# gvanhorn38/multibox

Measured on AMD Instinct MI355X. Metric: images/sec (299x299, 5-AR priors) train, higher is better.
Workload: dtype bf16; 1 GPU; full train step: Inception-ResNet-v2 + multibox heads fwd, on-device matching+loss, bwd, RMSProp+EMA; 299x299, k=5 (P=646), BATCH_SIZE=64/GPU, MAX_NUM_BBOXES=13; global_batch=64, parallelism=dp1, hip_graph=True

## Files before the change

### include/mbx.h

```cpp
#ifndef MBX_H
#define MBX_H

#include <stddef.h>
#include <stdint.h>

#ifdef __cplusplus
extern "C" {
#endif

typedef void* mbx_stream_t;

typedef enum {
  MBX_OK = 0,
  MBX_ERR_INVALID_ARG = -1,
  MBX_ERR_UNSUPPORTED = -2,
  MBX_ERR_LAUNCH = -3,
  MBX_ERR_WORKSPACE = -4
} mbx_status;

int mbx_version(void);
const char* mbx_status_string(int status);

int mbx_priors_count(int k, const int* grids, int n_grids);

uint32_t mbx_crc32c(const void* data, uint64_t n, uint32_t crc);
int mbx_generate_priors(const double* aspect_ratios, int k, double min_scale, double max_scale,
                        int restrict_to_image_bounds, const int* grids, int n_grids,
                        double* out );

int mbx_decode_conf(const float* raw_locs , const float* logits ,
                    const float* priors , int B, int P, float eps_add,
                    float* decoded , float* conf , mbx_stream_t stream);

size_t mbx_match_workspace_bytes(int B, int P, int G);
int mbx_match(const float* decoded , const float* conf ,
              const float* gt , const int32_t* n_gt , float alpha,
              int B, int P, int G, int32_t* match , int32_t* status ,
              void* workspace, size_t workspace_bytes, mbx_stream_t stream);

int mbx_match_extend(const float* priors , const float* gt ,
                     const int32_t* n_gt , const int32_t* status ,
                     float iou_threshold, int B, int P, int G,
                     int32_t* match ,
                     int32_t* n_extra , mbx_stream_t stream);

size_t mbx_loss_workspace_bytes(int B);
int mbx_loss_fwd_bwd(const float* decoded , const float* conf_in ,
                     int conf_is_logit, const float* gt ,
                     const int32_t* match , float alpha, float grad_scale, int B, int P,
                     int G, float* loss2 ,
                     float* d_raw_locs , float* d_logits ,
                     void* workspace, size_t workspace_bytes, mbx_stream_t stream);

size_t mbx_loss_mined_workspace_bytes(int B, int P);
int mbx_loss_fwd_bwd_mined(const float* decoded , const float* conf_in ,
                           int conf_is_logit, const float* gt ,
                           const int32_t* match , float alpha, float grad_scale, int B, int P,
                           int G, float* loss2 ,
                           float* d_raw_locs , float* d_logits ,
                           int neg_per_pos, int min_neg, int32_t* n_neg ,
                           void* workspace, size_t workspace_bytes, mbx_stream_t stream);

size_t mbx_loss_focal_workspace_bytes(int B, int P);
int mbx_loss_fwd_bwd_focal(const float* decoded , const float* conf_in ,
                           int conf_is_logit, const float* gt ,
                           const int32_t* match , float alpha, float grad_scale, int B, int P,
                           int G, float* loss2 ,
                           float* d_raw_locs , float* d_logits ,
                           float gamma, float w_pos, float w_neg,
                           int neg_per_pos , int min_neg, int32_t* n_neg ,
                           void* workspace, size_t workspace_bytes, mbx_stream_t stream);

typedef struct {
  int32_t offset_y, offset_x;
  int32_t patch_h, patch_w;
  int32_t image_h, image_w;
  int32_t is_flipped;
  int32_t max_to_keep;
  float restrictions[4];
} mbx_patch_meta;

int mbx_decode_filter_topk(const float* raw_locs , const float* conf ,
                           const float* priors , const mbx_patch_meta* meta ,
                           int B, int P, int k_max, double* out_boxes ,
                           float* out_scores , int32_t* out_index ,
                           int32_t* out_count , mbx_stream_t stream);

int mbx_nms(double* boxes , float* scores , int32_t* index ,
            int32_t* count , int B, int k_max, double iou_threshold, mbx_stream_t stream);

#define MBX_MERGE_MAX_CANDIDATES 16384
int mbx_merge_detections(const double* boxes , const float* scores ,
                         const int32_t* count , const int32_t* image_rows , int I, int k_max,
                         int max_det, double iou_threshold, double* out_boxes ,
                         float* out_scores , int32_t* out_src ,
                         int32_t* out_count , int32_t* out_status , mbx_stream_t stream);

int mbx_merge_detections_voted(const double* boxes , const float* scores ,
                               const int32_t* count , const int32_t* image_rows , int I,
                               int k_max, int max_det, double iou_threshold, double vote_iou_threshold,
                               double* out_boxes , float* out_scores ,
                               int32_t* out_src , int32_t* out_count ,
                               int32_t* out_status , int32_t* out_votes , mbx_stream_t stream);

#define MBX_SOFT_LINEAR 1
#define MBX_SOFT_GAUSSIAN 2
int mbx_merge_detections_soft(const double* boxes , const float* scores ,
                              const int32_t* count , const int32_t* image_rows , int I, int k_max,
                              int max_det, int method, double iou_threshold , double sigma ,
                              double min_score, double vote_iou_threshold ,
                              double* out_boxes , float* out_scores ,
                              int32_t* out_src , int32_t* out_count , int32_t* out_status ,
                              int32_t* out_votes , mbx_stream_t stream);

#define MBX_COCO_MAX_DET 100
#define MBX_COCO_MAX_GT 128
int mbx_coco_match(const double* dt , const int32_t* dt_rows ,
                   const double* gt , const int32_t* gt_rows , int I,
                   const double* iou_thrs , int T, const double* area_rng ,
                   int A, int16_t* match , uint8_t* ignore ,
                   int32_t* n_gt_counted , int32_t* status , mbx_stream_t stream);

#define MBX_COCO_ACC_MAX_R 128
#define MBX_COCO_ACC_MAX_M 4
#define MBX_COCO_ACC_MAX_ND 4194304
#define MBX_COCO_ACC_CHUNK 256
#define MBX_COCO_ACC_SORT_TILE 1024
size_t mbx_coco_accumulate_workspace(long long ND, int T, int A, int M);
int mbx_coco_accumulate(const double* dt , const int32_t* dt_rows , int I,
                        const int16_t* match , const uint8_t* ignore ,
                        const int32_t* n_gt_counted , int T, int A, const double* rec_thrs , int R,
                        const int32_t* max_dets , int M, double* precision ,
                        double* recall , void* workspace, size_t workspace_bytes, mbx_stream_t stream);

typedef enum {
  MBX_EPI_STORE = 0,
  MBX_EPI_AFFINE = 1,
  MBX_EPI_RESIDUAL = 2,
  MBX_EPI_STORE_F32 = 3
} mbx_epilogue;

typedef struct {
  int32_t n, rows_mod;
  int32_t c_begin[4];
  const void* y[4]; int32_t ld_y[4];
  const float* relu_thr[4];
  float* stats[4]; int32_t stats_ld[4];
} mbx_bn_bwd_stats;

#define MBX_GRID_BARRIER_BYTES 6400
typedef struct {
  void* barrier;
  void* a; int32_t ld_a;
  const float* beta;
  float* mean; float* rstd;
  float* moving_mean; float* moving_var;
  float* relu_thr;
  int32_t relu; float eps, decay;
  float* step_poison;
} mbx_bn_apply_desc;

#define MBX_BN_BWD_SLOTS 8
typedef struct {
  void* barrier;
  int32_t n;
  int32_t c_begin[4];
  const void* y[4]; int32_t ld_y[4];
  void* dy[4]; int32_t ld_dy[4];
  const float* mean[4]; const float* rstd[4]; const float* beta[4];
  float* dbeta[4];
  float* acc[4]; int32_t acc_ld[4];
  int32_t relu[4];
  float* step_poison;
} mbx_bn_bwd_fused;

typedef struct {
  const void* x; int64_t x_img_stride; int32_t ldx;
  int32_t N, H_in, W_in, C_in;
  const void* w; int32_t C_out, R, S;
  int32_t stride, transposed, pad_t, pad_l, H_out, W_out;
  void* y; int64_t y_img_stride; int32_t ldy;
  int32_t epilogue, relu, accumulate;
  const float* scale; const float* shift;
  const void* skip; int64_t skip_img_stride; int32_t ld_skip; float rscale;
  float* stats_partial;
  int32_t tile_config;
  const void* acc_src; int64_t acc_img_stride; int32_t ld_acc;
  int32_t* work_counter;
  int32_t max_workgroups;
  void* splitk_ws; int64_t splitk_ws_bytes;
  int32_t stats_rows_mod, stats_ld;
  const mbx_bn_bwd_stats* bn_bwd_stats;
  void* relu_bits; int32_t ld_bits;
  const mbx_bn_apply_desc* bn_apply;
  const mbx_bn_bwd_fused* bn_bwd;
} mbx_conv_desc;
#define MBX_CONV_TILE_CONFIGS 14
#define MBX_TILE_I5_BASE 32
#define MBX_TILE_I7 65
#define MBX_TILE_DIRECT3 96
#define MBX_TILE_DIRECTW 97
#define MBX_TILE_RESIDENT 98
#define MBX_TILE_PWRES 99
#define MBX_TILE_SPLITK_BASE 128
#define MBX_TILE_SPLITK_MAX 32

int mbx_conv_stats_rows(const mbx_conv_desc* desc );
int mbx_conv(const mbx_conv_desc* desc , mbx_stream_t stream);
int mbx_conv_supported(const mbx_conv_desc* desc );
int mbx_conv_pair(const mbx_conv_desc* a , const mbx_conv_desc* b , mbx_stream_t stream);
size_t mbx_conv_splitk_workspace_bytes(const mbx_conv_desc* desc );

int mbx_conv_wgrad(const mbx_conv_desc* desc , const void* dy,
                   int64_t dy_img_stride, int32_t ld_dy, float* dw, float* db, mbx_stream_t stream);

typedef struct {
  mbx_conv_desc desc;
  const void* dy; int64_t dy_img_stride; int32_t ld_dy;
  float scale;
  float* dw; float* db;
} mbx_wgrad_job;
typedef struct {
  int32_t n_layers, n_items;
  int64_t layers_off, items_off;
  int64_t queues_off, heads_off;
  double flops;
  int64_t tally_off;
} mbx_wgrad_plan_info;
#define MBX_WGRAD_DETERMINISTIC 1
#define MBX_WGRAD_SCATTER 2
size_t mbx_wgrad_plan_bytes(const mbx_wgrad_job* jobs , int n_jobs, int flags);
int mbx_wgrad_plan(const mbx_wgrad_job* jobs , int n_jobs, int flags, void* host_image, size_t bytes,
                   mbx_wgrad_plan_info* info );
int mbx_conv_wgrad_grouped(void* device_image , const mbx_wgrad_plan_info* info ,
                           mbx_stream_t stream);
int mbx_conv_wgrad_grouped_capped(void* device_image, const mbx_wgrad_plan_info* info , int max_workgroups,
                                  mbx_stream_t stream);

int mbx_conv_wgrad_scaled(const mbx_conv_desc* desc, const void* dy, int64_t dy_img_stride,
                          int32_t ld_dy, float scale, float* dw, float* db, mbx_stream_t stream);

int mbx_bn_finalize(const float* stats_partial , int rows, int C, int64_t count,
                    float eps, float decay, float* mean , float* rstd ,
                    float* moving_mean , float* moving_var ,
                    mbx_stream_t stream);
int mbx_bn_apply(const void* y, int64_t M, int C, const float* mean, const float* rstd,
                 const float* beta, int relu, void* a, int ld_a, mbx_stream_t stream);
int mbx_bn_apply_fused(const float* stats_partial, int rows, int64_t count, float eps, float decay,
                       const void* y, int64_t M, int C, const float* beta, int relu, void* a, int ld_a,
                       float* mean, float* rstd, float* moving_mean, float* moving_var,
                       mbx_stream_t stream);
int mbx_bn_apply_fused_mapped(const void* stats_fixed, int rows, int64_t count, float eps, float decay,
                              const void* y, int64_t M, int C, const float* beta, int relu, void* a, int ld_a,
                              const struct mbx_chan_map_s* a_map , float* mean, float* rstd, float* moving_mean,
                              float* moving_var, float* relu_thr, mbx_stream_t stream);
int mbx_bn_moving_update(float* moving_mean, float* moving_var, const float* batch_mean, const float* batch_var,
                         int64_t n, float decay, const float* skip_ctl, uint64_t* skipped_steps,
                         float* ema_mean, float* ema_var, float ema_decay, mbx_stream_t stream);
typedef struct mbx_chan_map_s { int32_t n; int32_t c_begin[4]; int32_t offset[4]; } mbx_chan_map;
int mbx_bn_finalize_parts(const float* const* parts , const int32_t* rows ,
                          const int32_t* Cs , int n_parts, int64_t count, float eps, float decay, float* mean,
                          float* rstd, float* moving_mean, float* moving_var, mbx_stream_t stream);
int mbx_bn_apply_mapped(const void* y, int64_t M, int C, const float* mean, const float* rstd, const float* beta,
                        int relu, void* a, int ld_a, const mbx_chan_map* a_map , mbx_stream_t stream);
int mbx_bn_apply_maxpool(const void* y, int N, int H, int W, int C, const float* mean, const float* rstd, const float* beta,
                         int relu, void* p, int64_t p_img_stride, int ld_p, int Ho, int Wo, uint8_t* argmax,
                         mbx_stream_t stream);
int mbx_bn_fold(const float* moving_mean, const float* moving_var, const float* beta, float eps,
                int C, float* scale, float* shift, mbx_stream_t stream);
int mbx_bn_bwd_rows(int64_t M, int C);
int mbx_bn_bwd_reduce(const void* da, int ld_da, const void* a, int ld_a, int relu, const void* y,
                      int64_t M, int C, const float* mean, const float* rstd, const float* beta,
                      float* partial , mbx_stream_t stream);
int mbx_bn_bwd_finalize(const float* partial, int rows, int C, int64_t M, float* dbeta ,
                        float* m12 , mbx_stream_t stream);
int mbx_bn_bwd_apply(const void* da, int ld_da, const void* a, int ld_a, int relu, const void* y,
                     int64_t M, int C, const float* mean, const float* rstd, const float* beta,
                     const float* m12, void* dy , mbx_stream_t stream);

int mbx_bn_bwd_reduce_mapped(const void* da, int ld_da, const void* a, int ld_a, int relu, const void* y, int64_t M, int C,
                             const float* mean, const float* rstd, const float* beta, float* partial,
                             const mbx_chan_map* da_map , mbx_stream_t stream);
int mbx_bn_bwd_apply_mapped(const void* da, int ld_da, const void* a, int ld_a, int relu, const void* y, int64_t M, int C,
                            const float* mean, const float* rstd, const float* beta, const float* m12, void* dy,
                            const mbx_chan_map* da_map , mbx_stream_t stream);

int mbx_bn_bwd_apply_rows(const float* stats, int rows, const void* da, int ld_da, const void* y, int64_t M, int C,
                          const float* mean, const float* rstd, const float* relu_thr, float* dbeta, void* dy,
                          const mbx_chan_map* da_map , mbx_stream_t stream);

size_t mbx_bn_bwd_onepass_workspace_bytes(int C);
int mbx_bn_bwd_onepass_supported(int64_t M, int C, int max_workgroups);
int mbx_bn_bwd_onepass(const void* da, int ld_da, int relu, const void* y, int64_t M, int C,
                       const float* mean, const float* rstd, const float* beta, float* dbeta ,
                       void* dy , void* ws, int max_workgroups, float* step_poison ,
                       mbx_stream_t stream);

int mbx_bn_bwd_rows_pooled(int N, int H, int W, int C);
int mbx_bn_bwd_reduce_pooled(const void* gy, int64_t gy_img_stride, int ld_gy, const uint8_t* argmax, int N, int H, int W,
                             int Ho, int Wo, int relu, const void* y, int C, const float* mean, const float* rstd,
                             const float* beta, float* partial , mbx_stream_t stream);
int mbx_bn_bwd_apply_pooled(const void* gy, int64_t gy_img_stride, int ld_gy, const uint8_t* argmax, int N, int H, int W,
                            int Ho, int Wo, int relu, const void* y, int C, const float* mean, const float* rstd,
                            const float* beta, const float* m12, void* dy, mbx_stream_t stream);
int mbx_bn_bwd_onepass_mapped(const void* da, int ld_da, int relu, const void* y, int64_t M, int C, const float* mean,
                              const float* rstd, const float* beta, float* dbeta, void* dy, void* ws, int max_workgroups,
                              float* step_poison, const mbx_chan_map* da_map , mbx_stream_t stream);

int mbx_maxpool_fwd(const void* x, int64_t x_img_stride, int ldx, int N, int H, int W, int C,
                    int k, int stride, void* y, int64_t y_img_stride, int ldy, int Ho, int Wo,
                    uint8_t* argmax , mbx_stream_t stream);
int mbx_maxpool_bwd(const void* dy, int64_t dy_img_stride, int ld_dy, const uint8_t* argmax,
                    int N, int H, int W, int C, int k, int stride, int Ho, int Wo, void* dx,
                    int64_t dx_img_stride, int ld_dx, int accumulate, mbx_stream_t stream);
int mbx_avgpool_fwd(const void* x, int64_t x_img_stride, int ldx, int N, int H, int W, int C,
                    int k, int pad, void* y, int64_t y_img_stride, int ldy, int Ho, int Wo,
                    mbx_stream_t stream);
int mbx_avgpool_bwd(const void* dy, int64_t dy_img_stride, int ld_dy, int N, int H, int W, int C,
                    int k, int pad, int Ho, int Wo, void* dx, int64_t dx_img_stride, int ld_dx,
                    int accumulate, mbx_stream_t stream);

int mbx_relu_mask(void* g, int ld_g, const void* a, int ld_a, int64_t M, int C, mbx_stream_t stream);
int mbx_pack_input(const float* img, int64_t pixels, void* out, mbx_stream_t stream);
int mbx_head_gather(const float* h, int ld_h, int N, int cells, int k, int P, int off,
                    float* locs, float* logits, mbx_stream_t stream);
int mbx_head_scatter(const float* d_locs, const float* d_logits, int N, int cells, int k, int P,
                     int off, void* g, int ld_g, mbx_stream_t stream);

typedef struct {
  const float* h; int32_t ld_h;
  void* g; int32_t ld_g;
  int32_t cells, k, off;
} mbx_head;
int mbx_head_gather_all(const mbx_head* heads , int n_heads, int N, int P, float* locs, float* logits,
                        mbx_stream_t stream);
int mbx_head_scatter_all(const float* d_locs, const float* d_logits, const mbx_head* heads , int n_heads, int N,
                         int P, mbx_stream_t stream);

int mbx_step_begin(float* grads, int64_t n_grads, float* bn_ws, int64_t n_ws, int64_t ctl_index, uint64_t* timeouts_total,
                   float* zero_scalar, mbx_stream_t stream);

typedef struct {
  int64_t src_off;
  int64_t dst_off;
  int32_t K, R, S, C, Kpad;
  int32_t first_block;
} mbx_filter_entry;
int mbx_filter_prepare(const void* w_bf16, void* w_dgrad, const mbx_filter_entry* table ,
                       int n_entries, int total_blocks, mbx_stream_t stream);

int mbx_rmsprop_ema_step(float* w, const float* g, float* ms, float* mom ,
                         float* ema , void* w_bf16 , int64_t n, float lr,
                         float decay, float momentum, float eps, float wd, float ema_decay,
                         int trainable, float* reg_loss, const float* skip_ctl, mbx_stream_t stream);
int mbx_ema_update(float* ema, const float* value, int64_t n, float ema_decay, const float* skip_ctl ,
                   mbx_stream_t stream);

typedef struct {
  uint64_t src_offset;
  int32_t src_h, src_w;
  int32_t method;
  int32_t flip;
  int32_t n_ops;
  int32_t op[4];
  int32_t pad_;
  double arg[4];
} mbx_augment_item;
size_t mbx_augment_workspace_bytes(int B, int S);
int mbx_augment_batch(const uint8_t* src , const mbx_augment_item* items , int B, int S,
                      int any_contrast, float* out , void* workspace, mbx_stream_t stream);

typedef struct {
  uint64_t src_offset;
  int32_t img_h, img_w;
  int32_t win_y, win_x, win_h, win_w;
  int32_t flip_source;
  int32_t pad_;
} mbx_patch_item;
int mbx_extract_patches(const uint8_t* src , const mbx_patch_item* items , int n, int S,
                        float* out , mbx_stream_t stream);

#ifdef __cplusplus
}
#endif
#endif
```

### multibox_amd/_lib.py

```python
from __future__ import annotations

import ctypes as C
import os

_HERE = os.path.dirname(os.path.abspath(__file__))
LIB_PATH = os.path.join(_HERE, "libmbx.so")

P = C.c_void_p
I = C.c_int
F = C.c_float
D = C.c_double
SZ = C.c_size_t


class PatchMeta(C.Structure):
    _fields_ = [("offset_y", C.c_int32), ("offset_x", C.c_int32), ("patch_h", C.c_int32), ("patch_w", C.c_int32),
                ("image_h", C.c_int32), ("image_w", C.c_int32), ("is_flipped", C.c_int32),
                ("max_to_keep", C.c_int32), ("restrictions", C.c_float * 4)]


_SIGS = {
    "mbx_version": (I, []),
    "mbx_status_string": (C.c_char_p, [I]),
    "mbx_priors_count": (I, [I, P, I]),
    "mbx_crc32c": (C.c_uint32, [P, C.c_uint64, C.c_uint32]),
    "mbx_generate_priors": (I, [P, I, D, D, I, P, I, P]),
    "mbx_decode_conf": (I, [P, P, P, I, I, F, P, P, P]),
    "mbx_match_workspace_bytes": (SZ, [I, I, I]),
    "mbx_match": (I, [P, P, P, P, F, I, I, I, P, P, P, SZ, P]),
    "mbx_match_extend": (I, [P, P, P, P, F, I, I, I, P, P, P]),
    "mbx_loss_workspace_bytes": (SZ, [I]),
    "mbx_loss_fwd_bwd": (I, [P, P, I, P, P, F, F, I, I, I, P, P, P, P, SZ, P]),
    "mbx_loss_mined_workspace_bytes": (SZ, [I, I]),
    "mbx_loss_fwd_bwd_mined": (I, [P, P, I, P, P, F, F, I, I, I, P, P, P, I, I, P, P, SZ, P]),
    "mbx_loss_focal_workspace_bytes": (SZ, [I, I]),
    "mbx_loss_fwd_bwd_focal": (I, [P, P, I, P, P, F, F, I, I, I, P, P, P, F, F, F, I, I, P, P, SZ, P]),
    "mbx_decode_filter_topk": (I, [P, P, P, P, I, I, I, P, P, P, P, P]),
    "mbx_nms": (I, [P, P, P, P, I, I, C.c_double, P]),
    "mbx_merge_detections": (I, [P, P, P, P, I, I, I, C.c_double, P, P, P, P, P, P]),
    "mbx_merge_detections_voted": (I, [P, P, P, P, I, I, I, C.c_double, C.c_double, P, P, P, P, P, P, P]),
    "mbx_merge_detections_soft": (I, [P, P, P, P, I, I, I, I, C.c_double, C.c_double, C.c_double, C.c_double, P, P, P, P, P, P, P]),
    "mbx_coco_match": (I, [P, P, P, P, I, P, I, P, I, P, P, P, P, P]),
    "mbx_coco_accumulate_workspace": (SZ, [C.c_longlong, I, I, I]),
    "mbx_coco_accumulate": (I, [P, P, I, P, P, P, I, I, P, I, P, I, P, P, P, SZ, P]),
    "mbx_augment_workspace_bytes": (SZ, [I, I]),
    "mbx_augment_batch": (I, [P, P, I, I, I, P, P, P]),
    "mbx_extract_patches": (I, [P, P, I, I, P, P]),
    "mbx_conv_stats_rows": (I, [P]),
    "mbx_conv": (I, [P, P]),
    "mbx_conv_supported": (I, [P]),
    "mbx_conv_pair": (I, [P, P, P]),
    "mbx_conv_splitk_workspace_bytes": (SZ, [P]),
    "mbx_conv_wgrad": (I, [P, P, C.c_int64, I, P, P, P]),
    "mbx_conv_wgrad_scaled": (I, [P, P, C.c_int64, I, F, P, P, P]),
    "mbx_wgrad_plan_bytes": (SZ, [P, I, I]),
    "mbx_wgrad_plan": (I, [P, I, I, P, SZ, P]),
    "mbx_conv_wgrad_grouped": (I, [P, P, P]),
    "mbx_conv_wgrad_grouped_capped": (I, [P, P, I, P]),
    "mbx_bn_finalize": (I, [P, I, I, C.c_int64, F, F, P, P, P, P, P]),
    "mbx_bn_apply": (I, [P, C.c_int64, I, P, P, P, I, P, I, P]),
    "mbx_bn_moving_update": (I, [P, P, P, P, C.c_int64, F, P, P, P, P, F, P]),
    "mbx_bn_finalize_parts": (I, [P, P, P, I, C.c_int64, F, F, P, P, P, P, P]),
    "mbx_bn_apply_mapped": (I, [P, C.c_int64, I, P, P, P, I, P, I, P, P]),
    "mbx_bn_bwd_reduce_mapped": (I, [P, I, P, I, I, P, C.c_int64, I, P, P, P, P, P, P]),
    "mbx_bn_bwd_apply_mapped": (I, [P, I, P, I, I, P, C.c_int64, I, P, P, P, P, P, P, P]),
    "mbx_bn_apply_maxpool": (I, [P, I, I, I, I, P, P, P, I, P, C.c_int64, I, I, I, P, P]),
    "mbx_bn_bwd_rows_pooled": (I, [I, I, I, I]),
    "mbx_bn_bwd_reduce_pooled": (I, [P, C.c_int64, I, P, I, I, I, I, I, I, P, I, P, P, P, P, P]),
    "mbx_bn_bwd_apply_pooled": (I, [P, C.c_int64, I, P, I, I, I, I, I, I, P, I, P, P, P, P, P, P]),
    "mbx_bn_bwd_onepass_mapped": (I, [P, I, I, P, C.c_int64, I, P, P, P, P, P, P, I, P, P, P]),
    "mbx_bn_fold": (I, [P, P, P, F, I, P, P, P]),
    "mbx_bn_apply_fused": (I, [P, I, C.c_int64, F, F, P, C.c_int64, I, P, I, P, I, P, P, P, P, P]),
    "mbx_bn_apply_fused_mapped": (I, [P, I, C.c_int64, F, F, P, C.c_int64, I, P, I, P, I, P, P, P, P, P, P, P]),
    "mbx_bn_bwd_apply_rows": (I, [P, I, P, I, P, C.c_int64, I, P, P, P, P, P, P, P]),
    "mbx_bn_bwd_rows": (I, [C.c_int64, I]),
    "mbx_bn_bwd_onepass_workspace_bytes": (C.c_size_t, [I]),
    "mbx_bn_bwd_onepass_supported": (I, [C.c_int64, I, I]),
    "mbx_bn_bwd_onepass": (I, [P, I, I, P, C.c_int64, I, P, P, P, P, P, P, I, P, P]),
    "mbx_bn_bwd_reduce": (I, [P, I, P, I, I, P, C.c_int64, I, P, P, P, P, P]),
    "mbx_bn_bwd_finalize": (I, [P, I, I, C.c_int64, P, P, P]),
    "mbx_bn_bwd_apply": (I, [P, I, P, I, I, P, C.c_int64, I, P, P, P, P, P, P]),
    "mbx_maxpool_fwd": (I, [P, C.c_int64, I, I, I, I, I, I, I, P, C.c_int64, I, I, I, P, P]),
    "mbx_maxpool_bwd": (I, [P, C.c_int64, I, P, I, I, I, I, I, I, I, I, P, C.c_int64, I, I, P]),
    "mbx_avgpool_fwd": (I, [P, C.c_int64, I, I, I, I, I, I, I, P, C.c_int64, I, I, I, P]),
    "mbx_avgpool_bwd": (I, [P, C.c_int64, I, I, I, I, I, I, I, I, I, P, C.c_int64, I, I, P]),
    "mbx_relu_mask": (I, [P, I, P, I, C.c_int64, I, P]),
    "mbx_pack_input": (I, [P, C.c_int64, P, P]),
    "mbx_head_gather": (I, [P, I, I, I, I, I, I, P, P, P]),
    "mbx_head_scatter": (I, [P, P, I, I, I, I, I, P, I, P]),
    "mbx_head_gather_all": (I, [P, I, I, I, P, P, P]),
    "mbx_head_scatter_all": (I, [P, P, P, I, I, I, P]),
    "mbx_step_begin": (I, [P, C.c_int64, P, C.c_int64, C.c_int64, P, P, P]),
    "mbx_filter_prepare": (I, [P, P, P, I, I, P]),
    "mbx_rmsprop_ema_step": (I, [P, P, P, P, P, P, C.c_int64, F, F, F, F, F, F, I, P, P, P]),
    "mbx_ema_update": (I, [P, P, C.c_int64, F, P, P]),
}

_lib = None


class MbxError(RuntimeError):
    pass


class ChanMap(C.Structure):
    _fields_ = [("n", C.c_int32), ("c_begin", C.c_int32 * 4), ("offset", C.c_int32 * 4)]


class BnBwdStats(C.Structure):
    _fields_ = [("n", C.c_int32), ("rows_mod", C.c_int32), ("c_begin", C.c_int32 * 4), ("y", C.c_void_p * 4), ("ld_y", C.c_int32 * 4),
                ("relu_thr", C.c_void_p * 4), ("stats", C.c_void_p * 4), ("stats_ld", C.c_int32 * 4)]


class Head(C.Structure):
    _fields_ = [("h", C.c_void_p), ("ld_h", C.c_int32), ("g", C.c_void_p), ("ld_g", C.c_int32), ("cells", C.c_int32),
                ("k", C.c_int32), ("off", C.c_int32)]


class FilterEntry(C.Structure):
    _fields_ = [("src_off", C.c_int64), ("dst_off", C.c_int64), ("K", C.c_int32), ("R", C.c_int32), ("S", C.c_int32),
                ("C", C.c_int32), ("Kpad", C.c_int32), ("first_block", C.c_int32)]


def lib():
    global _lib
    if _lib is None:
        if not os.path.exists(LIB_PATH):
            raise MbxError("libmbx.so not built at %s -- run `python -c 'import __graft_entry__ as g; g.build()'` "
                           "(needs hipcc); there is no CPU fallback" % LIB_PATH)
        import torch
        l = C.CDLL(LIB_PATH)
        for name, (res, args) in _SIGS.items():
            fn = getattr(l, name)
            fn.restype = res
            fn.argtypes = args
        _lib = l
    return _lib


def check(status, what=""):
    if status != 0:
        msg = lib().mbx_status_string(int(status))
        raise MbxError("%s failed: %s (%d)" % (what or "libmbx call", msg.decode() if msg else "?", status))


def declared_symbols():
    return sorted(_SIGS)
```

### multibox_amd/csrc/loss.hip

```cpp
#include "boxes.h"

namespace {

constexpr int kThreads = 256;
constexpr int kWaves = kThreads / 64;

__global__ void __launch_bounds__(kThreads)
decode_conf_kernel(const float4* __restrict__ raw, const float* __restrict__ logits,
                   const float4* __restrict__ priors, int total, int P, float eps_add,
                   float4* __restrict__ decoded, float* __restrict__ conf) {
  for (int i = blockIdx.x * blockDim.x + threadIdx.x; i < total; i += gridDim.x * blockDim.x) {
    if (decoded) {
      const float4 r = raw[i], p = priors[i % P];
      decoded[i] = make_float4(__fadd_rn(r.x, p.x), __fadd_rn(r.y, p.y), __fadd_rn(r.z, p.z), __fadd_rn(r.w, p.w));
    }
    if (conf) {
      const float s = 1.0f / (1.0f + expf(-logits[i]));
      conf[i] = __fadd_rn(s, eps_add);
    }
  }
}

__device__ __forceinline__ double match_cost(const float4 l, const float4 g, float half_alpha,
                                             float lc, float l1c) {
  const float d0 = __fsub_rn(l.x, g.x), d1 = __fsub_rn(l.y, g.y), d2 = __fsub_rn(l.z, g.z), d3 = __fsub_rn(l.w, g.w);
  const float ss = __fadd_rn(__fadd_rn(__fadd_rn(__fmul_rn(d0, d0), __fmul_rn(d1, d1)), __fmul_rn(d2, d2)), __fmul_rn(d3, d3));
  const float nrm = __fsqrt_rn(ss);
  float t = __fmul_rn(half_alpha, __fmul_rn(nrm, nrm));
  t = __fsub_rn(t, lc);
  t = __fadd_rn(t, l1c);
  return (double)t;
}

struct Cand {
  double val;
  int j;
  int free_;
};

__device__ __forceinline__ bool cand_better(const Cand& a, const Cand& b) {
  if (a.j < 0) return false;
  if (b.j < 0) return true;
  if (a.val < b.val) return true;
  if (a.val > b.val) return false;
  if (a.free_ != b.free_) return a.free_ > b.free_;
  return a.j < b.j;
}

__device__ __forceinline__ Cand cand_shfl_xor(const Cand& c, int o) {
  Cand r;
  r.val = __shfl_xor(c.val, o, 64);
  r.j = __shfl_xor(c.j, o, 64);
  r.free_ = __shfl_xor(c.free_, o, 64);
  return r;
}

__global__ void __launch_bounds__(1024)
match_kernel(const float4* __restrict__ decoded, const float* __restrict__ conf,
             const float4* __restrict__ gt, const int* __restrict__ n_gt, float alpha, int P, int G,
             int* __restrict__ match, int* __restrict__ status) {
  extern __shared__ __attribute__((aligned(16))) unsigned char smem[];
  double* v = reinterpret_cast<double*>(smem);
  double* spc = v + P;
  double* u = spc + P;
  float2* lcl = reinterpret_cast<float2*>(u + G);
  int* path = reinterpret_cast<int*>(lcl + P);
  int* row4col = path + P;
  int* SC = row4col + P;
  int* col4row = SC + P;
  int* SR = col4row + G;
  __shared__ Cand wave_best[16];
  __shared__ int sh_i, sh_sink, sh_bad;
  __shared__ double sh_min;

  const int b = blockIdx.x, tid = threadIdx.x;
  const int nt = (int)blockDim.x, nwaves = nt >> 6;
  const float4* loc = decoded + (size_t)b * P;
  const float* cf = conf + (size_t)b * P;
  const float4* g = gt + (size_t)b * G;
  int* mt = match + (size_t)b * P;
  const int n = n_gt[b];
  const float half_alpha = alpha / 2.0f;

  if (tid == 0) sh_bad = 0;
  __syncthreads();
  int bad = 0;
  for (int j = tid; j < P; j += nt) {
    mt[j] = -1;
    const float c = cf[j];
    const float lc = logf(c);
    float w = __fsub_rn(1.0f, c);
    if (w > 1.0f) w = 1.0f;
    if (w <= 0.0f) w = 1e-10f;
    const float l1c = logf(w);
    lcl[j] = make_float2(lc, l1c);
    v[j] = 0.0;
    row4col[j] = -1;
    const float4 l = loc[j];
    if (!(isfinite(lc) && isfinite(l1c) && isfinite(l.x) && isfinite(l.y) && isfinite(l.z) && isfinite(l.w))) bad = 1;
  }
  for (int i = tid; i < G; i += nt) {
    u[i] = 0.0;
    col4row[i] = -1;
    if (i < n) {
      const float4 q = g[i];
      if (!(isfinite(q.x) && isfinite(q.y) && isfinite(q.z) && isfinite(q.w))) bad = 1;
    }
  }
  if (bad) sh_bad = 1;
  __syncthreads();
  if (n <= 0) { if (tid == 0) status[b] = 0; return; }
  if (n > P || n > G) { if (tid == 0) status[b] = 1; return; }
  if (sh_bad) { if (tid == 0) status[b] = 2; return; }

  for (int cur = 0; cur < n; ++cur) {
    for (int j = tid; j < P; j += nt) { spc[j] = INFINITY; SC[j] = 0; }
    for (int i = tid; i < n; i += nt) SR[i] = 0;
    if (tid == 0) { sh_i = cur; sh_sink = -1; sh_min = 0.0; }
    __syncthreads();
    while (true) {
      const int i = sh_i;
      const double min_val = sh_min;
      const float4 gi = g[i];
      const double ui = u[i];
      Cand best; best.val = INFINITY; best.j = -1; best.free_ = 0;
      for (int j = tid; j < P; j += nt) {
        if (SC[j]) continue;
        const float2 ll = lcl[j];
        const double r = ((min_val + match_cost(loc[j], gi, half_alpha, ll.x, ll.y)) - ui) - v[j];
        double s = spc[j];
        if (r < s) { path[j] = i; spc[j] = r; s = r; }
        Cand c; c.val = s; c.j = j; c.free_ = row4col[j] < 0;
        if (cand_better(c, best)) best = c;
      }
#pragma unroll
      for (int o = 32; o > 0; o >>= 1) {
        const Cand other = cand_shfl_xor(best, o);
        if (cand_better(other, best)) best = other;
      }
      if ((tid & 63) == 0) wave_best[tid >> 6] = best;
      __syncthreads();
      if (tid == 0) {
        Cand bb = wave_best[0];
        for (int w = 1; w < nwaves; ++w) if (cand_better(wave_best[w], bb)) bb = wave_best[w];
        if (bb.j < 0 || !(bb.val < INFINITY)) {
          sh_sink = -2;
        } else {
          sh_min = bb.val;
          SC[bb.j] = 1;
          SR[i] = 1;
          const int r4c = row4col[bb.j];
          if (r4c < 0) sh_sink = bb.j; else sh_i = r4c;
        }
      }
      __syncthreads();
      if (sh_sink != -1) break;
    }
    const int sink = sh_sink;
    if (sink == -2) { if (tid == 0) status[b] = 2; return; }
    const double min_val = sh_min;
    for (int i = tid; i < n; i += nt) {
      if (i == cur) u[i] += min_val;
      else if (SR[i]) u[i] += min_val - spc[col4row[i]];
    }
    for (int j = tid; j < P; j += nt)
      if (SC[j]) v[j] -= min_val - spc[j];
    __syncthreads();
    if (tid == 0) {
      int j = sink;
      while (true) {
        const int i = path[j];
        row4col[j] = i;
        const int t = col4row[i];
        col4row[i] = j;
        j = t;
        if (i == cur) break;
      }
    }
    __syncthreads();
  }
  for (int i = tid; i < n; i += nt) mt[col4row[i]] = i;
  if (tid == 0) status[b] = 0;
}

struct StagedBox { Box box; double area; };

__global__ void __launch_bounds__(1024)
match_extend_kernel(const float4* __restrict__ priors, const float4* __restrict__ gt, const int* __restrict__ n_gt,
                    const int* __restrict__ status, double thr, int P, int G, int* __restrict__ match,
                    int* __restrict__ n_extra) {
  extern __shared__ __attribute__((aligned(16))) unsigned char smem[];
  StagedBox* boxes = reinterpret_cast<StagedBox*>(smem);
  __shared__ int added_waves[16];
  const int b = blockIdx.x, tid = threadIdx.x, nt = (int)blockDim.x;
  const int n = n_gt[b];
  if (status[b] != 0 || n <= 0 || n > G) {
    if (tid == 0 && n_extra) n_extra[b] = 0;
    return;
  }
  for (int j = tid; j < n; j += nt) {
    const float4 q = gt[(size_t)b * G + j];
    StagedBox s;
    s.box = {(double)q.x, (double)q.y, (double)q.z, (double)q.w};
    s.area = box_area(s.box);
    boxes[j] = s;
  }
  __syncthreads();
  int* mt = match + (size_t)b * P;
  int added = 0;
  for (int p = tid; p < P; p += nt) {
    if (mt[p] >= 0) continue;
    const float4 q = priors[p];
    const Box e = {(double)q.x, (double)q.y, (double)q.z, (double)q.w};
    const double area_e = box_area(e);
    double best = thr;
    int best_j = -1;
    for (int j = 0; j < n; ++j) {
      const Box g = boxes[j].box;
      const double iw = fmin(e.x2, g.x2) - fmax(e.x1, g.x1), ih = fmin(e.y2, g.y2) - fmax(e.y1, g.y1);
      if (iw > 0.0 && ih > 0.0) {
        const double inter = iw * ih;
        const double uni = area_e + boxes[j].area - inter;
        const double iou = uni > 0.0 ? inter / uni : 0.0;
        if (iou > best) { best = iou; best_j = j; }
      }
    }
    if (best_j >= 0) { mt[p] = best_j; ++added; }
  }
  if (!n_extra) return;
  added = wave_sum(added);
  if ((tid & 63) == 0) added_waves[tid >> 6] = added;
  __syncthreads();
  if (tid == 0) {
    int total = 0;
    for (int w = 0; w < (nt >> 6); ++w) total += added_waves[w];
    n_extra[b] = total;
  }
}

__global__ void loss_final_kernel(const double* __restrict__ partial, int B, float alpha, float* __restrict__ loss2) {
  if (threadIdx.x == 0 && blockIdx.x == 0) {
    double a = 0.0, c = 0.0;
    for (int b = 0; b < B; ++b) { a += partial[2 * b]; c += partial[2 * b + 1]; }
    loss2[0] = alpha * (float)(a * 0.5);
    loss2[1] = (float)c;
  }
}

__device__ __forceinline__ unsigned long long mined_key(float conf_in, int P, int p) {
  return ((unsigned long long)score_order_key(conf_in) << 32) | (unsigned)(P - 1 - p);
}

__device__ __forceinline__ unsigned long long mined_select_cut(const int* __restrict__ mt, const float* __restrict__ cf,
                                                               int P, int neg_per_pos, int min_neg, int b,
                                                               int* __restrict__ n_neg) {
  static_assert(kThreads == 256, "one thread per histogram bin, four bins per lane of the walking wave");
  __shared__ unsigned hist[256];
  __shared__ unsigned long long sh_cut;
  __shared__ int sh_need, sh_done;
  const int tid = threadIdx.x;
  unsigned long long cut = 0ull;
  int need = 0;
  for (int shift = 56; shift >= 0; shift -= 8) {
    if (shift < 32 && ((unsigned)(P - 1) >> shift) == 0) continue;
    const unsigned long long fixed = shift == 56 ? 0ull : ~0ull << (shift + 8);
    hist[tid] = 0u;
    __syncthreads();
    for (int p = tid; p < P; p += kThreads) {
      if (mt[p] >= 0) continue;
      const unsigned long long key = mined_key(cf[p], P, p);
      if (((key ^ cut) & fixed) == 0ull) atomicAdd(&hist[(unsigned)(key >> shift) & 255u], 1u);
    }
    __syncthreads();
    if (tid < 64) {
      const unsigned h0 = hist[4 * tid], h1 = hist[4 * tid + 1], h2 = hist[4 * tid + 2], h3 = hist[4 * tid + 3];
      const unsigned own = h0 + h1 + h2 + h3;
      unsigned incl = own;
#pragma unroll
      for (int o = 1; o < 64; o <<= 1) {
        const unsigned t = __shfl_down(incl, o, 64);
        if (tid + o < 64) incl += t;
      }
      bool whole = false;
      if (shift == 56) {
        const int n_negatives = (int)__shfl(incl, 0, 64), n_pos = P - n_negatives;
        long long K = (long long)neg_per_pos * (long long)n_pos;
        if (K < (long long)min_neg) K = min_neg;
        if (K > (long long)n_negatives) K = n_negatives;
        need = (int)K;
        whole = need == 0 || need == n_negatives;
        if (tid == 0) {
          if (n_neg) n_neg[b] = need;
          if (whole) { sh_cut = need == 0 ? ~0ull : 0ull; sh_need = 0; sh_done = 1; }
        }
      }
      const unsigned above = incl - own, k = (unsigned)need;
      if (!whole && above < k && k <= incl) {
        unsigned a = above, cnt = h3;
        int d = 3;
        if (k > a + h3) { a += h3; cnt = h2; d = 2;
          if (k > a + h2) { a += h2; cnt = h1; d = 1;
            if (k > a + h1) { a += h1; cnt = h0; d = 0; } } }
        sh_cut = cut | ((unsigned long long)(4 * tid + d) << shift);
        sh_need = (int)(k - a);
        sh_done = cnt == k - a;
      }
    }
    __syncthreads();
    cut = sh_cut;
    need = sh_need;
    if (sh_done) break;
  }
  return cut;
}

template <bool MINED, bool FOCAL>
__device__ __forceinline__ void loss_body(const float4* __restrict__ decoded, const float* __restrict__ logits, int is_logit,
                                          const float4* __restrict__ gt, const int* __restrict__ match, float alpha,
                                          float grad_scale, int P, int G, float gamma, float w_pos, float w_neg,
                                          int neg_per_pos, int min_neg, double* __restrict__ partial ,
                                          float4* __restrict__ d_locs, float* __restrict__ d_logits, int* __restrict__ n_neg) {
  constexpr bool kCountPositives = FOCAL && !MINED;
  const int b = blockIdx.x, tid = threadIdx.x;
  unsigned long long cut = 0ull;
  if (MINED) cut = mined_select_cut(match + (size_t)b * P, logits + (size_t)b * P, P, neg_per_pos, min_neg, b, n_neg);
  const bool modulated = FOCAL && gamma != 0.0f;

  double loc_acc = 0.0, conf_acc = 0.0;
  int n_pos = 0;
  for (int p = tid; p < P; p += kThreads) {
    const size_t i = (size_t)b * P + p;
    const int m = match[i];
    const float z = logits[i];
    float4 dl = make_float4(0.f, 0.f, 0.f, 0.f);
    float g;
    if (MINED && m < 0 && mined_key(z, P, p) < cut) {
      g = 0.f;
    } else {
      const float s = is_logit ? 1.0f / (1.0f + expf(-z)) : z;
      const float c = __fadd_rn(s, 1e-10f);
      const float w = __fadd_rn(__fsub_rn(1.0f, c), 1e-10f);
      const float ds = is_logit ? s * (1.0f - s) : 1.0f;
      const bool pos = m >= 0;
      if (pos) {
        const float4 l = decoded[i], q = gt[(size_t)b * G + m];
        const float d0 = __fsub_rn(l.x, q.x), d1 = __fsub_rn(l.y, q.y), d2 = __fsub_rn(l.z, q.z), d3 = __fsub_rn(l.w, q.w);
        loc_acc += (double)d0 * d0 + (double)d1 * d1 + (double)d2 * d2 + (double)d3 * d3;
        const float a = alpha * grad_scale;
        dl = make_float4(a * d0, a * d1, a * d2, a * d3);
        if (kCountPositives) ++n_pos;
      }
      const float arg = pos ? c : w, base = pos ? w : c, wt = FOCAL ? (pos ? w_pos : w_neg) : 1.0f;
      const float lg = logf(arg);
      const float pw = modulated ? powf(base, gamma) : 1.0f;
      conf_acc -= (double)wt * ((double)pw * (double)lg);
      float d = (ds * pw) / arg;
      if (modulated) d = d - gamma * (pw / base) * lg * ds;
      d = wt * d;
      g = (pos ? -d : d) * grad_scale;
    }
    if (d_locs) d_locs[i] = dl;
    if (d_logits) d_logits[i] = g;
  }
  loc_acc = wave_sum(loc_acc);
  conf_acc = wave_sum(conf_acc);
  __shared__ double red[kWaves][2];
  __shared__ int pos_waves[kWaves];
  if (kCountPositives) n_pos = wave_sum(n_pos);
  if ((tid & 63) == 0) {
    red[tid >> 6][0] = loc_acc; red[tid >> 6][1] = conf_acc;
    if (kCountPositives) pos_waves[tid >> 6] = n_pos;
  }
  __syncthreads();
  if (tid == 0) {
    double a = 0.0, c = 0.0;
    for (int w = 0; w < kWaves; ++w) { a += red[w][0]; c += red[w][1]; }
    partial[2 * b] = a;
    partial[2 * b + 1] = c;
    if (kCountPositives && n_neg) {
      int total = 0;
      for (int w = 0; w < kWaves; ++w) total += pos_waves[w];
      n_neg[b] = P - total;
    }
  }
}

__global__ void __launch_bounds__(kThreads)
loss_kernel(const float4* __restrict__ decoded, const float* __restrict__ logits, int is_logit,
            const float4* __restrict__ gt, const int* __restrict__ match, float alpha, float grad_scale,
            int P, int G, double* __restrict__ partial , float4* __restrict__ d_locs,
            float* __restrict__ d_logits) {
  loss_body<false, false>(decoded, logits, is_logit, gt, match, alpha, grad_scale, P, G, 0.0f, 1.0f, 1.0f, 0, 0, partial,
                          d_locs, d_logits, nullptr);
}

__global__ void __launch_bounds__(kThreads)
loss_mined_kernel(const float4* __restrict__ decoded, const float* __restrict__ logits, int is_logit,
                  const float4* __restrict__ gt, const int* __restrict__ match, float alpha, float grad_scale,
                  int P, int G, int neg_per_pos, int min_neg, double* __restrict__ partial ,
                  float4* __restrict__ d_locs, float* __restrict__ d_logits, int* __restrict__ n_neg) {
  loss_body<true, false>(decoded, logits, is_logit, gt, match, alpha, grad_scale, P, G, 0.0f, 1.0f, 1.0f, neg_per_pos,
                         min_neg, partial, d_locs, d_logits, n_neg);
}

template <bool MINED>
__global__ void __launch_bounds__(kThreads)
loss_focal_kernel(const float4* __restrict__ decoded, const float* __restrict__ logits, int is_logit,
                  const float4* __restrict__ gt, const int* __restrict__ match, float alpha, float grad_scale,
                  int P, int G, float gamma, float w_pos, float w_neg, int neg_per_pos, int min_neg,
                  double* __restrict__ partial , float4* __restrict__ d_locs, float* __restrict__ d_logits,
                  int* __restrict__ n_neg) {
  loss_body<MINED, true>(decoded, logits, is_logit, gt, match, alpha, grad_scale, P, G, gamma, w_pos, w_neg, neg_per_pos,
                         min_neg, partial, d_locs, d_logits, n_neg);
}

}

extern "C" int mbx_decode_conf(const float* raw_locs, const float* logits, const float* priors, int B,
                               int P, float eps_add, float* decoded, float* conf, mbx_stream_t stream) {
  if (B < 0 || P <= 0) return MBX_ERR_INVALID_ARG;
  if ((decoded && (!raw_locs || !priors)) || (conf && !logits)) return MBX_ERR_INVALID_ARG;
  if (B == 0 || (!decoded && !conf)) return MBX_OK;
  const int total = B * P;
  int blocks = (total + kThreads - 1) / kThreads;
  if (blocks > 2048) blocks = 2048;
  MBX_ENTER();
  hipLaunchKernelGGL(decode_conf_kernel, dim3(blocks), dim3(kThreads), 0, mbx_s(stream),
                     reinterpret_cast<const float4*>(raw_locs), logits, reinterpret_cast<const float4*>(priors),
                     total, P, eps_add, reinterpret_cast<float4*>(decoded), conf);
  MBX_LAUNCH_CHECK();
  return MBX_OK;
}

static size_t match_lds_bytes(int P, int G) { return (size_t)P * 36 + (size_t)G * 16 + 16; }

extern "C" size_t mbx_match_workspace_bytes(int, int, int) { return 0; }

extern "C" int mbx_match(const float* decoded, const float* conf, const float* gt, const int32_t* n_gt,
                         float alpha, int B, int P, int G, int32_t* match, int32_t* status, void*, size_t,
                         mbx_stream_t stream) {
  if (!decoded || !conf || !gt || !n_gt || !match || !status || B < 0 || P <= 0 || G <= 0) return MBX_ERR_INVALID_ARG;
  if (B == 0) return MBX_OK;
  const size_t lds = match_lds_bytes(P, G);
  if (lds > 150 * 1024) return MBX_ERR_UNSUPPORTED;
  static const int force_nt = mbx_env_int("MBX_MATCH_THREADS", 0);
  const int nthreads = force_nt ? force_nt : (P > 1536 ? 512 : kThreads);
  MBX_ENTER();
  if (lds > 64 * 1024) {
    if (hipFuncSetAttribute(reinterpret_cast<const void*>(match_kernel), hipFuncAttributeMaxDynamicSharedMemorySize,
                            (int)lds) != hipSuccess) return MBX_ERR_LAUNCH;
  }
  hipLaunchKernelGGL(match_kernel, dim3(B), dim3(nthreads), lds, mbx_s(stream),
                     reinterpret_cast<const float4*>(decoded), conf, reinterpret_cast<const float4*>(gt), n_gt,
                     alpha, P, G, match, status);
  MBX_LAUNCH_CHECK();
  return MBX_OK;
}

extern "C" int mbx_match_extend(const float* priors, const float* gt, const int32_t* n_gt, const int32_t* status,
                                float iou_threshold, int B, int P, int G, int32_t* match, int32_t* n_extra,
                                mbx_stream_t stream) {
  if (!priors || !gt || !n_gt || !status || !match || B < 0 || P <= 0 || G <= 0) return MBX_ERR_INVALID_ARG;
  if (!(iou_threshold > 0.0f && iou_threshold <= 1.0f)) return MBX_ERR_INVALID_ARG;
  const size_t lds = (size_t)G * sizeof(StagedBox);
  if (lds > 60 * 1024) return MBX_ERR_UNSUPPORTED;
  if (B == 0) return MBX_OK;
  const int nthreads = P >= 1024 ? 1024 : (P + 63) / 64 * 64;
  MBX_ENTER();
  hipLaunchKernelGGL(match_extend_kernel, dim3(B), dim3(nthreads), lds, mbx_s(stream),
                     reinterpret_cast<const float4*>(priors), reinterpret_cast<const float4*>(gt), n_gt, status,
                     (double)iou_threshold, P, G, match, n_extra);
  MBX_LAUNCH_CHECK();
  return MBX_OK;
}

extern "C" size_t mbx_loss_workspace_bytes(int B) { return (size_t)(B > 0 ? B : 1) * 2 * sizeof(double); }
extern "C" size_t mbx_loss_mined_workspace_bytes(int B, int) { return mbx_loss_workspace_bytes(B); }
extern "C" size_t mbx_loss_focal_workspace_bytes(int B, int) { return mbx_loss_workspace_bytes(B); }

enum class LossKind { kPlain, kMined, kFocal };

static int launch_loss(LossKind kind, const float* decoded, const float* logits, int conf_is_logit, const float* gt,
                       const int32_t* match, float alpha, float grad_scale, int B, int P, int G, float* loss2,
                       float* d_raw_locs, float* d_logits, float gamma, float w_pos, float w_neg, int neg_per_pos,
                       int min_neg, int32_t* n_neg, void* workspace, size_t workspace_bytes, mbx_stream_t stream) {
  if (!decoded || !logits || !gt || !match || !loss2 || B <= 0 || P <= 0 || G <= 0) return MBX_ERR_INVALID_ARG;
  if (!workspace || workspace_bytes < mbx_loss_workspace_bytes(B)) return MBX_ERR_WORKSPACE;
  double* partial = reinterpret_cast<double*>(workspace);
  const float4* dec4 = reinterpret_cast<const float4*>(decoded);
  const float4* gt4 = reinterpret_cast<const float4*>(gt);
  float4* dl4 = reinterpret_cast<float4*>(d_raw_locs);
  MBX_ENTER();
  switch (kind) {
    case LossKind::kPlain:
      hipLaunchKernelGGL(loss_kernel, dim3(B), dim3(kThreads), 0, mbx_s(stream), dec4, logits, conf_is_logit, gt4, match,
                         alpha, grad_scale, P, G, partial, dl4, d_logits);
      break;
    case LossKind::kMined:
      hipLaunchKernelGGL(loss_mined_kernel, dim3(B), dim3(kThreads), 0, mbx_s(stream), dec4, logits, conf_is_logit, gt4,
                         match, alpha, grad_scale, P, G, neg_per_pos, min_neg, partial, dl4, d_logits, n_neg);
      break;
    case LossKind::kFocal:
      hipLaunchKernelGGL(neg_per_pos ? loss_focal_kernel<true> : loss_focal_kernel<false>, dim3(B), dim3(kThreads), 0,
                         mbx_s(stream), dec4, logits, conf_is_logit, gt4, match, alpha, grad_scale, P, G, gamma, w_pos,
                         w_neg, neg_per_pos, min_neg, partial, dl4, d_logits, n_neg);
      break;
  }
  MBX_LAUNCH_CHECK();
  hipLaunchKernelGGL(loss_final_kernel, dim3(1), dim3(64), 0, mbx_s(stream), partial, B, alpha, loss2);
  MBX_LAUNCH_CHECK();
  return MBX_OK;
}

extern "C" int mbx_loss_fwd_bwd(const float* decoded, const float* logits, int conf_is_logit, const float* gt,
                                const int32_t* match, float alpha, float grad_scale, int B, int P, int G, float* loss2,
                                float* d_raw_locs, float* d_logits, void* workspace, size_t workspace_bytes,
                                mbx_stream_t stream) {
  return launch_loss(LossKind::kPlain, decoded, logits, conf_is_logit, gt, match, alpha, grad_scale, B, P, G, loss2,
                     d_raw_locs, d_logits, 0.0f, 1.0f, 1.0f, 0, 0, nullptr, workspace, workspace_bytes, stream);
}

extern "C" int mbx_loss_fwd_bwd_mined(const float* decoded, const float* logits, int conf_is_logit, const float* gt,
                                      const int32_t* match, float alpha, float grad_scale, int B, int P, int G, float* loss2,
                                      float* d_raw_locs, float* d_logits, int neg_per_pos, int min_neg, int32_t* n_neg,
                                      void* workspace, size_t workspace_bytes, mbx_stream_t stream) {
  if (neg_per_pos < 1 || min_neg < 0) return MBX_ERR_INVALID_ARG;
  return launch_loss(LossKind::kMined, decoded, logits, conf_is_logit, gt, match, alpha, grad_scale, B, P, G, loss2,
                     d_raw_locs, d_logits, 0.0f, 1.0f, 1.0f, neg_per_pos, min_neg, n_neg, workspace, workspace_bytes, stream);
}

extern "C" int mbx_loss_fwd_bwd_focal(const float* decoded, const float* logits, int conf_is_logit, const float* gt,
                                      const int32_t* match, float alpha, float grad_scale, int B, int P, int G, float* loss2,
                                      float* d_raw_locs, float* d_logits, float gamma, float w_pos, float w_neg,
                                      int neg_per_pos, int min_neg, int32_t* n_neg, void* workspace, size_t workspace_bytes,
                                      mbx_stream_t stream) {
  if (!(gamma >= 0.0f && gamma <= 10.0f)) return MBX_ERR_INVALID_ARG;
  if (!(w_pos >= 0.0f && w_neg >= 0.0f) || isinf(w_pos) || isinf(w_neg)) return MBX_ERR_INVALID_ARG;
  if (neg_per_pos < 0 || min_neg < 0 || (neg_per_pos == 0 && min_neg > 0)) return MBX_ERR_INVALID_ARG;
  return launch_loss(LossKind::kFocal, decoded, logits, conf_is_logit, gt, match, alpha, grad_scale, B, P, G, loss2,
                     d_raw_locs, d_logits, gamma, w_pos, w_neg, neg_per_pos, min_neg, n_neg, workspace, workspace_bytes, stream);
}
```

### multibox_amd/csrc/nnops.hip

```cpp
#include "vec8.h"

namespace {

template <int KK, int SS>
__global__ void __launch_bounds__(kT)
maxpool_fwd_kernel(const unsigned short* __restrict__ x, long long xs, int ldx, int N, int H, int W, int C, int k_,
                   int stride_, unsigned short* __restrict__ y, long long ys, int ldy, int Ho, int Wo,
                   unsigned char* __restrict__ argmax) {
  const int k = KK ? KK : k_, stride = SS ? SS : stride_;
  const int C8 = C >> 3;
  const unsigned total = (unsigned)N * Ho * Wo * C8;
  for (unsigned i = blockIdx.x * kT + threadIdx.x; i < total; i += gridDim.x * kT) {
    unsigned t = i / (unsigned)C8;
    const int c = (int)(i - t * C8) << 3;
    const unsigned t2 = t / (unsigned)Wo;
    const int ow = (int)(t - t2 * Wo);
    const int n = (int)(t2 / (unsigned)Ho);
    const int oh = (int)(t2 - (unsigned)n * Ho);
    float best[8];
    unsigned arg[8];
#pragma unroll
    for (int j = 0; j < 8; ++j) { best[j] = -INFINITY; arg[j] = 0; }
    if constexpr (KK > 0) {
      u32x4 v[KK * KK];
#pragma unroll
      for (int r = 0; r < KK; ++r)
#pragma unroll
        for (int s = 0; s < KK; ++s) {
          const int h = oh * stride + r, w = ow * stride + s;
          v[r * KK + s] = (h < H && w < W) ? ld8(x + n * xs + ((long long)h * W + w) * ldx + c) : u32x4{0u, 0u, 0u, 0u};
        }
#pragma unroll
      for (int r = 0; r < KK; ++r)
#pragma unroll
        for (int s = 0; s < KK; ++s) {
          const int h = oh * stride + r, w = ow * stride + s;
          if (h >= H || w >= W) continue;
          float f[8];
          unpack8(v[r * KK + s], f);
#pragma unroll
          for (int j = 0; j < 8; ++j)
            if (f[j] > best[j]) { best[j] = f[j]; arg[j] = r * KK + s; }
        }
    } else {
      for (int r = 0; r < k; ++r)
        for (int s = 0; s < k; ++s) {
          const int h = oh * stride + r, w = ow * stride + s;
          if (h >= H || w >= W) continue;
          float f[8];
          unpack8(ld8(x + n * xs + ((long long)h * W + w) * ldx + c), f);
#pragma unroll
          for (int j = 0; j < 8; ++j)
            if (f[j] > best[j]) { best[j] = f[j]; arg[j] = r * k + s; }
        }
    }
    st8(y + n * ys + ((long long)oh * Wo + ow) * ldy + c, pack8(best));
    if (argmax) {
      u32x2 av;
      av.x = arg[0] | (arg[1] << 8) | (arg[2] << 16) | (arg[3] << 24);
      av.y = arg[4] | (arg[5] << 8) | (arg[6] << 16) | (arg[7] << 24);
      *reinterpret_cast<u32x2*>(argmax + (((long long)n * Ho + oh) * Wo + ow) * C + c) = av;
    }
  }
}

template <int KK, int SS>
__global__ void __launch_bounds__(kT)
maxpool_bwd_kernel(const unsigned short* __restrict__ dy, long long dys, int ld_dy,
                   const unsigned char* __restrict__ argmax, int N, int H, int W, int C, int k_, int stride_, int Ho,
                   int Wo, unsigned short* __restrict__ dx, long long dxs, int ld_dx, int accumulate) {
  const int k = KK ? KK : k_, stride = SS ? SS : stride_;
  const int C8 = C >> 3;
  const unsigned total = (unsigned)N * H * W * C8;
  for (unsigned i = blockIdx.x * kT + threadIdx.x; i < total; i += gridDim.x * kT) {
    unsigned t = i / (unsigned)C8;
    const int c = (int)(i - t * C8) << 3;
    const unsigned t2 = t / (unsigned)W;
    const int w = (int)(t - t2 * W);
    const int n = (int)(t2 / (unsigned)H);
    const int h = (int)(t2 - (unsigned)n * H);
    float acc[8];
    unsigned short* dst = dx + n * dxs + ((long long)h * W + w) * ld_dx + c;
    if (accumulate) unpack8(ld8(dst), acc);
    else {
#pragma unroll
      for (int j = 0; j < 8; ++j) acc[j] = 0.f;
    }
    if constexpr (KK > 0) {
      constexpr int NW = (KK + SS - 1) / SS;
      const int ohb = h / SS, owb = w / SS;
      u32x4 gv[NW * NW];
      u32x2 av[NW * NW];
      bool ok[NW * NW];
#pragma unroll
      for (int a = 0; a < NW; ++a)
#pragma unroll
        for (int b = 0; b < NW; ++b) {
          const int oh = ohb - (NW - 1 - a), ow = owb - (NW - 1 - b);
          const bool v = oh >= 0 && oh < Ho && ow >= 0 && ow < Wo && h - oh * SS < KK && w - ow * SS < KK;
          ok[a * NW + b] = v;
          const long long o = ((long long)n * Ho + (v ? oh : 0)) * Wo + (v ? ow : 0);
          av[a * NW + b] = v ? *reinterpret_cast<const u32x2*>(argmax + o * C + c) : u32x2{0u, 0u};
          gv[a * NW + b] = v ? ld8(dy + n * dys + ((long long)oh * Wo + ow) * ld_dy + c) : u32x4{0u, 0u, 0u, 0u};
        }
#pragma unroll
      for (int a = 0; a < NW; ++a)
#pragma unroll
        for (int b = 0; b < NW; ++b) {
          if (!ok[a * NW + b]) continue;
          const int oh = ohb - (NW - 1 - a), ow = owb - (NW - 1 - b);
          const unsigned tap = (h - oh * SS) * KK + (w - ow * SS);
          float g[8];
          unpack8(gv[a * NW + b], g);
#pragma unroll
          for (int j = 0; j < 8; ++j) {
            const unsigned aj = ((j < 4 ? av[a * NW + b].x : av[a * NW + b].y) >> (8 * (j & 3))) & 0xffu;
            if (aj == tap) acc[j] += g[j];
          }
        }
    } else {
      int oh0 = (h - k + stride) / stride;
      if (h - k + 1 <= 0) oh0 = 0;
      int ow0 = (w - k + stride) / stride;
      if (w - k + 1 <= 0) ow0 = 0;
      const int oh1 = min(h / stride, Ho - 1), ow1 = min(w / stride, Wo - 1);
      for (int oh = oh0; oh <= oh1; ++oh)
        for (int ow = ow0; ow <= ow1; ++ow) {
          const unsigned tap = (h - oh * stride) * k + (w - ow * stride);
          const long long o = ((long long)n * Ho + oh) * Wo + ow;
          const u32x2 av = *reinterpret_cast<const u32x2*>(argmax + o * C + c);
          float g[8];
          unpack8(ld8(dy + n * dys + ((long long)oh * Wo + ow) * ld_dy + c), g);
#pragma unroll
          for (int j = 0; j < 8; ++j) {
            const unsigned aj = ((j < 4 ? av.x : av.y) >> (8 * (j & 3))) & 0xffu;
            if (aj == tap) acc[j] += g[j];
          }
        }
    }
    st8(dst, pack8(acc));
  }
}

__global__ void __launch_bounds__(kT)
avgpool_fwd_kernel(const unsigned short* __restrict__ x, long long xs, int ldx, int N, int H, int W, int C, int k,
                   int pad, unsigned short* __restrict__ y, long long ys, int ldy, int Ho, int Wo) {
  const int C8 = C >> 3;
  const unsigned total = (unsigned)N * Ho * Wo * C8;
  for (unsigned i = blockIdx.x * kT + threadIdx.x; i < total; i += gridDim.x * kT) {
    unsigned t = i / (unsigned)C8;
    const int c = (int)(i - t * C8) << 3;
    const unsigned t2 = t / (unsigned)Wo;
    const int ow = (int)(t - t2 * Wo);
    const int n = (int)(t2 / (unsigned)Ho);
    const int oh = (int)(t2 - (unsigned)n * Ho);
    float acc[8];
#pragma unroll
    for (int j = 0; j < 8; ++j) acc[j] = 0.f;
    int cnt = 0;
    if (k == 3) {
      u32x4 v[9];
      bool ok[9];
#pragma unroll
      for (int r = 0; r < 3; ++r)
#pragma unroll
        for (int q = 0; q < 3; ++q) {
          const int h = oh - pad + r, w = ow - pad + q;
          ok[r * 3 + q] = (unsigned)h < (unsigned)H && (unsigned)w < (unsigned)W;
          v[r * 3 + q] = ok[r * 3 + q] ? ld8(x + n * xs + ((long long)h * W + w) * ldx + c) : u32x4{0u, 0u, 0u, 0u};
        }
#pragma unroll
      for (int tq = 0; tq < 9; ++tq) {
        if (!ok[tq]) continue;
        float f[8];
        unpack8(v[tq], f);
#pragma unroll
        for (int j = 0; j < 8; ++j) acc[j] += f[j];
        ++cnt;
      }
    } else
    for (int r = 0; r < k; ++r) {
      const int h = oh - pad + r;
      if ((unsigned)h >= (unsigned)H) continue;
      const unsigned short* row = x + n * xs + (long long)h * W * ldx + c;
      for (int s0 = 0; s0 < k; s0 += 8) {
        u32x4 v[8];
        bool ok[8];
#pragma unroll
        for (int q = 0; q < 8; ++q) {
          const int w = ow - pad + s0 + q;
          ok[q] = s0 + q < k && (unsigned)w < (unsigned)W;
          v[q] = ok[q] ? ld8(row + (long long)w * ldx) : u32x4{0u, 0u, 0u, 0u};
        }
#pragma unroll
        for (int q = 0; q < 8; ++q) {
          if (!ok[q]) continue;
          float f[8];
          unpack8(v[q], f);
#pragma unroll
          for (int j = 0; j < 8; ++j) acc[j] += f[j];
          ++cnt;
        }
      }
    }
    const float inv = 1.0f / (float)cnt;
#pragma unroll
    for (int j = 0; j < 8; ++j) acc[j] *= inv;
    st8(y + n * ys + ((long long)oh * Wo + ow) * ldy + c, pack8(acc));
  }
}

__global__ void __launch_bounds__(kT)
avgpool_bwd_kernel(const unsigned short* __restrict__ dy, long long dys, int ld_dy, int N, int H, int W, int C, int k,
                   int pad, int Ho, int Wo, unsigned short* __restrict__ dx, long long dxs, int ld_dx,
                   int accumulate) {
  const int C8 = C >> 3;
  const unsigned total = (unsigned)N * H * W * C8;
  for (unsigned i = blockIdx.x * kT + threadIdx.x; i < total; i += gridDim.x * kT) {
    unsigned t = i / (unsigned)C8;
    const int c = (int)(i - t * C8) << 3;
    const unsigned t2 = t / (unsigned)W;
    const int w = (int)(t - t2 * W);
    const int n = (int)(t2 / (unsigned)H);
    const int h = (int)(t2 - (unsigned)n * H);
    float acc[8];
    unsigned short* dst = dx + n * dxs + ((long long)h * W + w) * ld_dx + c;
    if (accumulate) unpack8(ld8(dst), acc);
    else {
#pragma unroll
      for (int j = 0; j < 8; ++j) acc[j] = 0.f;
    }
    const int oh0 = max(h + pad - k + 1, 0), oh1 = min(h + pad, Ho - 1);
    const int ow0 = max(w + pad - k + 1, 0), ow1 = min(w + pad, Wo - 1);
    if (k == 3) {
      u32x4 v[9];
      float inv[9];
#pragma unroll
      for (int a = 0; a < 3; ++a)
#pragma unroll
        for (int b = 0; b < 3; ++b) {
          const int oh = oh0 + a, ow = ow0 + b;
          const bool ok = oh <= oh1 && ow <= ow1;
          const int nh = min(oh - pad + 3, H) - max(oh - pad, 0), nw = min(ow - pad + 3, W) - max(ow - pad, 0);
          inv[a * 3 + b] = ok ? 1.0f / (float)(nh * nw) : 0.f;
          v[a * 3 + b] = ok ? ld8(dy + n * dys + ((long long)oh * Wo + ow) * ld_dy + c) : u32x4{0u, 0u, 0u, 0u};
        }
#pragma unroll
      for (int tq = 0; tq < 9; ++tq) {
        if (inv[tq] == 0.f) continue;
        float g[8];
        unpack8(v[tq], g);
#pragma unroll
        for (int j = 0; j < 8; ++j) acc[j] += g[j] * inv[tq];
      }
    } else
    for (int oh = oh0; oh <= oh1; ++oh) {
      const int nh = min(oh - pad + k, H) - max(oh - pad, 0);
      for (int ow = ow0; ow <= ow1; ++ow) {
        const int nw = min(ow - pad + k, W) - max(ow - pad, 0);
        const float inv = 1.0f / (float)(nh * nw);
        float g[8];
        unpack8(ld8(dy + n * dys + ((long long)oh * Wo + ow) * ld_dy + c), g);
#pragma unroll
        for (int j = 0; j < 8; ++j) acc[j] += g[j] * inv;
      }
    }
    st8(dst, pack8(acc));
  }
}

__global__ void __launch_bounds__(kT)
relu_mask_kernel(unsigned short* __restrict__ g, int ld_g, const unsigned short* __restrict__ a, int ld_a,
                 long long M, int C) {
  const int C8 = C >> 3;
  const long long total = M * C8;
  for (long long i = (long long)blockIdx.x * kT + threadIdx.x; i < total; i += (long long)gridDim.x * kT) {
    const long long m = i / C8;
    const int c = (int)(i - m * C8) << 3;
    float gg[8], aa[8];
    unpack8(ld8(g + m * ld_g + c), gg);
    unpack8(ld8(a + m * ld_a + c), aa);
#pragma unroll
    for (int j = 0; j < 8; ++j)
      if (!(aa[j] > 0.f)) gg[j] = 0.f;
    st8(g + m * ld_g + c, pack8(gg));
  }
}

__global__ void __launch_bounds__(kT)
pack_input_kernel(const float* __restrict__ img, long long pixels, unsigned short* __restrict__ out) {
  for (long long i = (long long)blockIdx.x * kT + threadIdx.x; i < pixels; i += (long long)gridDim.x * kT) {
    float f[8] = {img[3 * i], img[3 * i + 1], img[3 * i + 2], 0.f, 0.f, 0.f, 0.f, 0.f};
    st8(out + 8 * i, pack8(f));
  }
}

__global__ void __launch_bounds__(kT)
head_gather_kernel(const float* __restrict__ h, int ld_h, int N, int cells, int k, int P, int off,
                   float* __restrict__ locs, float* __restrict__ logits) {
  const int total = N * cells * k;
  for (int i = blockIdx.x * kT + threadIdx.x; i < total; i += gridDim.x * kT) {
    const int a = i % k, t = i / k, cell = t % cells, n = t / cells;
    const float* row = h + (size_t)(n * cells + cell) * ld_h;
    const size_t p = (size_t)n * P + off + cell * k + a;
    *reinterpret_cast<float4*>(locs + p * 4) = make_float4(row[a * 4], row[a * 4 + 1], row[a * 4 + 2], row[a * 4 + 3]);
    logits[p] = row[4 * k + a];
  }
}

__global__ void __launch_bounds__(kT)
head_scatter_kernel(const float* __restrict__ d_locs, const float* __restrict__ d_logits, int N, int cells, int k,
                    int P, int off, unsigned short* __restrict__ g, int ld_g) {
  const int total = N * cells * ld_g;
  for (int i = blockIdx.x * kT + threadIdx.x; i < total; i += gridDim.x * kT) {
    const int ch = i % ld_g, t = i / ld_g, cell = t % cells, n = t / cells;
    const size_t p = (size_t)n * P + off + cell * k;
    float v = 0.f;
    if (ch < 4 * k) v = d_locs[(p + ch / 4) * 4 + (ch & 3)];
    else if (ch < 5 * k) v = d_logits[p + (ch - 4 * k)];
    g[i] = (unsigned short)f2bf(v);
  }
}

constexpr int kMaxHeads = 8;
struct HeadTable {
  const float* h[kMaxHeads]; unsigned short* g[kMaxHeads];
  int ld_h[kMaxHeads], ld_g[kMaxHeads], cells[kMaxHeads], k[kMaxHeads], off[kMaxHeads];
  int start[kMaxHeads + 1];
  int n;
};

__global__ void __launch_bounds__(kT)
head_gather_all_kernel(const HeadTable t, int P, float* __restrict__ locs, float* __restrict__ logits) {
  const int total = t.start[t.n];
  for (int i = blockIdx.x * kT + threadIdx.x; i < total; i += gridDim.x * kT) {
    int j = 0;
    while (j + 1 < t.n && i >= t.start[j + 1]) ++j;
    const int e = i - t.start[j], k = t.k[j], cells = t.cells[j];
    const int a = e % k, q = e / k, cell = q % cells, n = q / cells;
    const float* row = t.h[j] + (size_t)(n * cells + cell) * t.ld_h[j];
    const size_t p = (size_t)n * P + t.off[j] + cell * k + a;
    *reinterpret_cast<float4*>(locs + p * 4) = make_float4(row[a * 4], row[a * 4 + 1], row[a * 4 + 2], row[a * 4 + 3]);
    logits[p] = row[4 * k + a];
  }
}

__global__ void __launch_bounds__(kT)
head_scatter_all_kernel(const HeadTable t, int P, const float* __restrict__ d_locs, const float* __restrict__ d_logits) {
  const int total = t.start[t.n];
  for (int i = blockIdx.x * kT + threadIdx.x; i < total; i += gridDim.x * kT) {
    int j = 0;
    while (j + 1 < t.n && i >= t.start[j + 1]) ++j;
    const int e = i - t.start[j], k = t.k[j], cells = t.cells[j], ld = t.ld_g[j];
    const int ch = e % ld, q = e / ld, cell = q % cells, n = q / cells;
    const size_t p = (size_t)n * P + t.off[j] + cell * k;
    float v = 0.f;
    if (ch < 4 * k) v = d_locs[(p + ch / 4) * 4 + (ch & 3)];
    else if (ch < 5 * k) v = d_logits[p + (ch - 4 * k)];
    t.g[j][e] = (unsigned short)f2bf(v);
  }
}

__global__ void __launch_bounds__(kT)
step_begin_kernel(float* __restrict__ G, long long nG, float* __restrict__ ws, long long nws, long long ctl,
                  unsigned long long* __restrict__ timeouts_total, float* __restrict__ scalar) {
  if (scalar && blockIdx.x == 0 && threadIdx.x == 0) *scalar = 0.f;
  const long long n4 = nG >> 2, w4 = nws >> 2;
  const float4 z = make_float4(0.f, 0.f, 0.f, 0.f);
  for (long long i = (long long)blockIdx.x * kT + threadIdx.x; i < n4 + w4; i += (long long)gridDim.x * kT) {
    if (i < n4) {
      if (timeouts_total && i == (ctl >> 2)) {
        const float t = G[ctl];
        if (t > 0.f) *timeouts_total += (unsigned long long)t;
      }
      reinterpret_cast<float4*>(G)[i] = z;
    } else {
      reinterpret_cast<float4*>(ws)[i - n4] = z;
    }
  }
}

__global__ void __launch_bounds__(kT)
filter_prepare_kernel(const unsigned short* __restrict__ w, unsigned short* __restrict__ wd,
                      const mbx_filter_entry* __restrict__ table, int n_entries) {
  __shared__ __attribute__((aligned(16))) unsigned short tile[64][40];
  int lo = 0, hi = n_entries - 1;
  while (lo < hi) {
    const int mid = (lo + hi + 1) >> 1;
    if (table[mid].first_block <= (int)blockIdx.x) lo = mid; else hi = mid - 1;
  }
  const mbx_filter_entry e = table[lo];
  const int kt = (e.Kpad + 63) / 64, ct = (e.C + 31) / 32;
  int b = blockIdx.x - e.first_block;
  const int ck = b % kt; b /= kt;
  const int cc = b % ct; b /= ct;
  const int s = b % e.S, r = b / e.S;
  const unsigned short* src = w + e.src_off;
  unsigned short* dst = wd + e.dst_off;
  const int k0 = ck * 64, c0 = cc * 32;
  const long long tap_src = ((long long)(e.R - 1 - r) * e.S + (e.S - 1 - s)) * e.C;
  if (((e.C | e.Kpad) & 7) == 0 && ((e.src_off | e.dst_off) & 7) == 0) {
    static_assert(kT == 256, "one 16-byte chunk per thread");
    {
      const int kk = threadIdx.x >> 2, c = (threadIdx.x & 3) << 3;
      uint4 v = make_uint4(0u, 0u, 0u, 0u);
      if (k0 + kk < e.K && c0 + c < e.C)
        v = *reinterpret_cast<const uint4*>(src + (long long)(k0 + kk) * e.R * e.S * e.C + tap_src + c0 + c);
      *reinterpret_cast<uint4*>(&tile[kk][c]) = v;
    }
    __syncthreads();
    {
      const int c = threadIdx.x >> 3, kk = (threadIdx.x & 7) << 3;
      if (k0 + kk < e.Kpad && c0 + c < e.C) {
        unsigned q[4];
#pragma unroll
        for (int j = 0; j < 4; ++j) q[j] = (unsigned)tile[kk + 2 * j][c] | ((unsigned)tile[kk + 2 * j + 1][c] << 16);
        *reinterpret_cast<uint4*>(dst + (((long long)(c0 + c) * e.R + r) * e.S + s) * e.Kpad + k0 + kk) =
            make_uint4(q[0], q[1], q[2], q[3]);
      }
    }
    return;
  }
  for (int i = threadIdx.x; i < 64 * 32; i += kT) {
    const int kk = i >> 5, c = i & 31;
    unsigned short v = 0;
    if (k0 + kk < e.K && c0 + c < e.C) v = src[(long long)(k0 + kk) * e.R * e.S * e.C + tap_src + c0 + c];
    tile[kk][c] = v;
  }
  __syncthreads();
  for (int i = threadIdx.x; i < 64 * 32; i += kT) {
    const int c = i >> 6, kk = i & 63;
    if (k0 + kk < e.Kpad && c0 + c < e.C)
      dst[(((long long)(c0 + c) * e.R + r) * e.S + s) * e.Kpad + k0 + kk] = tile[kk][c];
  }
}

__global__ void __launch_bounds__(kT)
rmsprop_ema_kernel(float* __restrict__ w, const float* __restrict__ g, float* __restrict__ ms, float* __restrict__ mom,
                   float* __restrict__ ema, unsigned short* __restrict__ wb, long long n, float lr, float decay,
                   float momentum, float eps, float wd, float ema_decay, int trainable, float* __restrict__ reg_loss,
                   const float* __restrict__ skip_ctl) {
  if (skip_ctl && (skip_ctl[0] != 0.f || skip_ctl[1] != 0.f)) return;
  float sq = 0.f;
  auto one = [&](float wi, const float gi_, float& msi, float& momi, float& emai) -> float {
    sq += wi * wi;
    if (ema) emai = emai - (1.0f - ema_decay) * (emai - wi);
    if (trainable) {
      const float gi = gi_ + wd * wi;
      const float m = decay * msi + (1.0f - decay) * gi * gi;
      msi = m;
      float step = lr * gi / sqrtf(m + eps);
      if (mom) { step = momentum * momi + step; momi = step; }
      wi -= step;
    }
    return wi;
  };
  const bool vec = ((reinterpret_cast<uintptr_t>(w) | reinterpret_cast<uintptr_t>(g) | reinterpret_cast<uintptr_t>(ms) |
                     reinterpret_cast<uintptr_t>(mom) | reinterpret_cast<uintptr_t>(ema)) & 15) == 0 && (reinterpret_cast<uintptr_t>(wb) & 7) == 0;
  const long long n4 = vec ? n / 4 : 0;
  for (long long i = (long long)blockIdx.x * kT + threadIdx.x; i < n4; i += (long long)gridDim.x * kT) {
    float4 wv = reinterpret_cast<const float4*>(w)[i];
    float4 ev = ema ? reinterpret_cast<const float4*>(ema)[i] : make_float4(0.f, 0.f, 0.f, 0.f);
    float4 gv = make_float4(0.f, 0.f, 0.f, 0.f), mv = gv, ov = gv;
    if (trainable) { gv = reinterpret_cast<const float4*>(g)[i]; mv = reinterpret_cast<const float4*>(ms)[i]; if (mom) ov = reinterpret_cast<const float4*>(mom)[i]; }
    wv.x = one(wv.x, gv.x, mv.x, ov.x, ev.x); wv.y = one(wv.y, gv.y, mv.y, ov.y, ev.y);
    wv.z = one(wv.z, gv.z, mv.z, ov.z, ev.z); wv.w = one(wv.w, gv.w, mv.w, ov.w, ev.w);
    if (ema) reinterpret_cast<float4*>(ema)[i] = ev;
    if (trainable) { reinterpret_cast<float4*>(ms)[i] = mv; if (mom) reinterpret_cast<float4*>(mom)[i] = ov; reinterpret_cast<float4*>(w)[i] = wv; }
    if (wb) reinterpret_cast<uint2*>(wb)[i] = make_uint2(pack2bf(wv.x, wv.y), pack2bf(wv.z, wv.w));
  }
  for (long long i = 4 * n4 + (long long)blockIdx.x * kT + threadIdx.x; i < n; i += (long long)gridDim.x * kT) {
    float msi = trainable ? ms[i] : 0.f, momi = (trainable && mom) ? mom[i] : 0.f, emai = ema ? ema[i] : 0.f;
    const float wi = one(w[i], trainable ? g[i] : 0.f, msi, momi, emai);
    if (ema) ema[i] = emai;
    if (trainable) { ms[i] = msi; if (mom) mom[i] = momi; w[i] = wi; }
    if (wb) wb[i] = (unsigned short)f2bf(wi);
  }
  if (reg_loss && wd != 0.f) {
    sq = wave_sum(sq);
    __shared__ float red[kT / 64];
    if ((threadIdx.x & 63) == 0) red[threadIdx.x >> 6] = sq;
    __syncthreads();
    if (threadIdx.x == 0) {
      float t = 0.f;
      for (int i = 0; i < kT / 64; ++i) t += red[i];
      atomicAdd(reg_loss, 0.5f * wd * t);
    }
  }
}

__global__ void __launch_bounds__(kT)
ema_update_kernel(float* __restrict__ ema, const float* __restrict__ v, long long n, float d,
                  const float* __restrict__ skip_ctl) {
  if (skip_ctl && (skip_ctl[0] != 0.f || skip_ctl[1] != 0.f)) return;
  for (long long i = (long long)blockIdx.x * kT + threadIdx.x; i < n; i += (long long)gridDim.x * kT) {
    const float e = ema[i];
    ema[i] = e - (1.0f - d) * (e - v[i]);
  }
}

}

static int pool_args_ok(const void* x, int ldx, const void* y, int ldy, int N, int H, int W, int C, int k, int Ho, int Wo) {
  return x && y && N > 0 && H > 0 && W > 0 && C > 0 && C % 8 == 0 && ldx % 8 == 0 && ldy % 8 == 0 && k > 0 && k < 16 &&
         Ho > 0 && Wo > 0 && al16(x) && al16(y) && (long long)N * H * W * (C / 8) < (1LL << 31) &&
         (long long)N * Ho * Wo * (C / 8) < (1LL << 31);
}

extern "C" int mbx_maxpool_fwd(const void* x, int64_t xs, int ldx, int N, int H, int W, int C, int k, int stride, void* y,
                               int64_t ys, int ldy, int Ho, int Wo, uint8_t* argmax, mbx_stream_t stream) {
  if (!pool_args_ok(x, ldx, y, ldy, N, H, W, C, k, Ho, Wo) || stride < 1) return MBX_ERR_INVALID_ARG;
  if ((Ho - 1) * stride + k > H || (Wo - 1) * stride + k > W) return MBX_ERR_INVALID_ARG;
  MBX_ENTER();
  if (k == 3 && stride == 2)
    hipLaunchKernelGGL((maxpool_fwd_kernel<3, 2>), dim3(grid_for((long long)N * Ho * Wo * (C / 8))), dim3(kT), 0, mbx_s(stream),
                       (cus)x, (long long)xs, ldx, N, H, W, C, k, stride, (us)y, (long long)ys, ldy, Ho, Wo, argmax);
  else
    hipLaunchKernelGGL((maxpool_fwd_kernel<0, 0>), dim3(grid_for((long long)N * Ho * Wo * (C / 8))), dim3(kT), 0, mbx_s(stream),
                       (cus)x, (long long)xs, ldx, N, H, W, C, k, stride, (us)y, (long long)ys, ldy, Ho, Wo, argmax);
  MBX_LAUNCH_CHECK();
  return MBX_OK;
}

extern "C" int mbx_maxpool_bwd(const void* dy, int64_t dys, int ld_dy, const uint8_t* argmax, int N, int H, int W, int C,
                               int k, int stride, int Ho, int Wo, void* dx, int64_t dxs, int ld_dx, int accumulate,
                               mbx_stream_t stream) {
  if (!pool_args_ok(dy, ld_dy, dx, ld_dx, N, H, W, C, k, Ho, Wo) || !argmax || stride < 1) return MBX_ERR_INVALID_ARG;
  MBX_ENTER();
  if (k == 3 && stride == 2)
    hipLaunchKernelGGL((maxpool_bwd_kernel<3, 2>), dim3(grid_for((long long)N * H * W * (C / 8))), dim3(kT), 0, mbx_s(stream),
                       (cus)dy, (long long)dys, ld_dy, argmax, N, H, W, C, k, stride, Ho, Wo, (us)dx, (long long)dxs, ld_dx,
                       accumulate);
  else
    hipLaunchKernelGGL((maxpool_bwd_kernel<0, 0>), dim3(grid_for((long long)N * H * W * (C / 8))), dim3(kT), 0, mbx_s(stream),
                       (cus)dy, (long long)dys, ld_dy, argmax, N, H, W, C, k, stride, Ho, Wo, (us)dx, (long long)dxs, ld_dx,
                       accumulate);
  MBX_LAUNCH_CHECK();
  return MBX_OK;
}

extern "C" int mbx_avgpool_fwd(const void* x, int64_t xs, int ldx, int N, int H, int W, int C, int k, int pad, void* y,
                               int64_t ys, int ldy, int Ho, int Wo, mbx_stream_t stream) {
  if (!pool_args_ok(x, ldx, y, ldy, N, H, W, C, k, Ho, Wo) || pad < 0 || pad >= k) return MBX_ERR_INVALID_ARG;
  if (Ho != H + 2 * pad - k + 1 || Wo != W + 2 * pad - k + 1) return MBX_ERR_INVALID_ARG;
  MBX_ENTER();
  hipLaunchKernelGGL(avgpool_fwd_kernel, dim3(grid_for((long long)N * Ho * Wo * (C / 8))), dim3(kT), 0, mbx_s(stream),
                     (cus)x, (long long)xs, ldx, N, H, W, C, k, pad, (us)y, (long long)ys, ldy, Ho, Wo);
  MBX_LAUNCH_CHECK();
  return MBX_OK;
}

extern "C" int mbx_avgpool_bwd(const void* dy, int64_t dys, int ld_dy, int N, int H, int W, int C, int k, int pad, int Ho,
                               int Wo, void* dx, int64_t dxs, int ld_dx, int accumulate, mbx_stream_t stream) {
  if (!pool_args_ok(dy, ld_dy, dx, ld_dx, N, H, W, C, k, Ho, Wo) || pad < 0 || pad >= k) return MBX_ERR_INVALID_ARG;
  MBX_ENTER();
  hipLaunchKernelGGL(avgpool_bwd_kernel, dim3(grid_for((long long)N * H * W * (C / 8))), dim3(kT), 0, mbx_s(stream),
                     (cus)dy, (long long)dys, ld_dy, N, H, W, C, k, pad, Ho, Wo, (us)dx, (long long)dxs, ld_dx, accumulate);
  MBX_LAUNCH_CHECK();
  return MBX_OK;
}

extern "C" int mbx_relu_mask(void* g, int ld_g, const void* a, int ld_a, int64_t M, int C, mbx_stream_t stream) {
  if (!g || !a || M <= 0 || C <= 0 || C % 8 || ld_g % 8 || ld_a % 8 || !al16(g) || !al16(a)) return MBX_ERR_INVALID_ARG;
  MBX_ENTER();
  hipLaunchKernelGGL(relu_mask_kernel, dim3(grid_for(M * (C / 8))), dim3(kT), 0, mbx_s(stream), (us)g, ld_g, (cus)a, ld_a,
                     (long long)M, C);
  MBX_LAUNCH_CHECK();
  return MBX_OK;
}

extern "C" int mbx_pack_input(const float* img, int64_t pixels, void* out, mbx_stream_t stream) {
  if (!img || !out || pixels <= 0 || !al16(out)) return MBX_ERR_INVALID_ARG;
  MBX_ENTER();
  hipLaunchKernelGGL(pack_input_kernel, dim3(grid_for(pixels)), dim3(kT), 0, mbx_s(stream), img, (long long)pixels, (us)out);
  MBX_LAUNCH_CHECK();
  return MBX_OK;
}

extern "C" int mbx_head_gather(const float* h, int ld_h, int N, int cells, int k, int P, int off, float* locs,
                               float* logits, mbx_stream_t stream) {
  if (!h || !locs || !logits || N <= 0 || cells <= 0 || k <= 0 || ld_h < 5 * k || off < 0 || off + cells * k > P)
    return MBX_ERR_INVALID_ARG;
  MBX_ENTER();
  hipLaunchKernelGGL(head_gather_kernel, dim3(grid_for((long long)N * cells * k)), dim3(kT), 0, mbx_s(stream), h, ld_h, N,
                     cells, k, P, off, locs, logits);
  MBX_LAUNCH_CHECK();
  return MBX_OK;
}

extern "C" int mbx_head_scatter(const float* d_locs, const float* d_logits, int N, int cells, int k, int P, int off, void* g,
                                int ld_g, mbx_stream_t stream) {
  if (!d_locs || !d_logits || !g || N <= 0 || cells <= 0 || k <= 0 || ld_g < 5 * k || off < 0 || off + cells * k > P)
    return MBX_ERR_INVALID_ARG;
  MBX_ENTER();
  hipLaunchKernelGGL(head_scatter_kernel, dim3(grid_for((long long)N * cells * ld_g)), dim3(kT), 0, mbx_s(stream), d_locs,
                     d_logits, N, cells, k, P, off, (us)g, ld_g);
  MBX_LAUNCH_CHECK();
  return MBX_OK;
}

static int fill_head_table(const mbx_head* heads, int n_heads, int N, int P, bool scatter, HeadTable& t) {
  if (!heads || n_heads <= 0 || n_heads > kMaxHeads || N <= 0 || P <= 0) return MBX_ERR_INVALID_ARG;
  long long acc = 0;
  t.n = n_heads;
  for (int j = 0; j < n_heads; ++j) {
    const mbx_head& H = heads[j];
    if (H.cells <= 0 || H.k <= 0 || H.off < 0 || H.off + H.cells * H.k > P) return MBX_ERR_INVALID_ARG;
    if (scatter ? (!H.g || H.ld_g < 5 * H.k) : (!H.h || H.ld_h < 5 * H.k)) return MBX_ERR_INVALID_ARG;
    t.h[j] = H.h; t.g[j] = reinterpret_cast<unsigned short*>(H.g);
    t.ld_h[j] = H.ld_h; t.ld_g[j] = H.ld_g; t.cells[j] = H.cells; t.k[j] = H.k; t.off[j] = H.off;
    t.start[j] = (int)acc;
    acc += (long long)N * H.cells * (scatter ? H.ld_g : H.k);
    if (acc >= (1LL << 31)) return MBX_ERR_UNSUPPORTED;
  }
  for (int j = n_heads; j <= kMaxHeads; ++j) t.start[j] = (int)acc;
  return MBX_OK;
}

extern "C" int mbx_head_gather_all(const mbx_head* heads, int n_heads, int N, int P, float* locs, float* logits,
                                   mbx_stream_t stream) {
  if (!locs || !logits) return MBX_ERR_INVALID_ARG;
  HeadTable t;
  const int st = fill_head_table(heads, n_heads, N, P, false, t);
  if (st != MBX_OK) return st;
  MBX_ENTER();
  hipLaunchKernelGGL(head_gather_all_kernel, dim3(grid_for(t.start[t.n])), dim3(kT), 0, mbx_s(stream), t, P, locs, logits);
  MBX_LAUNCH_CHECK();
  return MBX_OK;
}

extern "C" int mbx_head_scatter_all(const float* d_locs, const float* d_logits, const mbx_head* heads, int n_heads, int N,
                                    int P, mbx_stream_t stream) {
  if (!d_locs || !d_logits) return MBX_ERR_INVALID_ARG;
  HeadTable t;
  const int st = fill_head_table(heads, n_heads, N, P, true, t);
  if (st != MBX_OK) return st;
  MBX_ENTER();
  hipLaunchKernelGGL(head_scatter_all_kernel, dim3(grid_for(t.start[t.n])), dim3(kT), 0, mbx_s(stream), t, P, d_locs, d_logits);
  MBX_LAUNCH_CHECK();
  return MBX_OK;
}

extern "C" int mbx_step_begin(float* grads, int64_t n_grads, float* bn_ws, int64_t n_ws, int64_t ctl_index,
                              uint64_t* timeouts_total, float* zero_scalar, mbx_stream_t stream) {
  if (!grads || n_grads <= 0 || n_grads % 4 || n_ws < 0 || n_ws % 4 || (n_ws && !bn_ws) || !al16(grads) || (bn_ws && !al16(bn_ws)) ||
      (timeouts_total && (ctl_index < 0 || ctl_index >= n_grads)))
    return MBX_ERR_INVALID_ARG;
  MBX_ENTER();
  hipLaunchKernelGGL(step_begin_kernel, dim3(grid_for((n_grads + n_ws) / 4)), dim3(kT), 0, mbx_s(stream), grads,
                     (long long)n_grads, bn_ws, (long long)n_ws, (long long)ctl_index,
                     reinterpret_cast<unsigned long long*>(timeouts_total), zero_scalar);
  MBX_LAUNCH_CHECK();
  return MBX_OK;
}

extern "C" int mbx_filter_prepare(const void* w_bf16, void* w_dgrad, const mbx_filter_entry* table, int n_entries,
                                  int total_blocks, mbx_stream_t stream) {
  if (!w_bf16 || !w_dgrad || !table || n_entries <= 0 || total_blocks <= 0) return MBX_ERR_INVALID_ARG;
  MBX_ENTER();
  hipLaunchKernelGGL(filter_prepare_kernel, dim3(total_blocks), dim3(kT), 0, mbx_s(stream), (cus)w_bf16, (us)w_dgrad, table,
                     n_entries);
  MBX_LAUNCH_CHECK();
  return MBX_OK;
}

extern "C" int mbx_rmsprop_ema_step(float* w, const float* g, float* ms, float* mom, float* ema, void* w_bf16, int64_t n,
                                    float lr, float decay, float momentum, float eps, float wd, float ema_decay,
                                    int trainable, float* reg_loss, const float* skip_ctl, mbx_stream_t stream) {
  if (!w || n <= 0 || (trainable && (!g || !ms))) return MBX_ERR_INVALID_ARG;
  if (trainable && momentum != 0.f && !mom) return MBX_ERR_INVALID_ARG;
  MBX_ENTER();
  hipLaunchKernelGGL(rmsprop_ema_kernel, dim3(grid_for(n)), dim3(kT), 0, mbx_s(stream), w, g, ms, momentum != 0.f ? mom : nullptr,
                     ema, (us)w_bf16, (long long)n, lr, decay, momentum, eps, wd, ema_decay, trainable, reg_loss, skip_ctl);
  MBX_LAUNCH_CHECK();
  return MBX_OK;
}

extern "C" int mbx_ema_update(float* ema, const float* value, int64_t n, float ema_decay, const float* skip_ctl,
                              mbx_stream_t stream) {
  if (!ema || !value || n <= 0) return MBX_ERR_INVALID_ARG;
  MBX_ENTER();
  hipLaunchKernelGGL(ema_update_kernel, dim3(grid_for(n)), dim3(kT), 0, mbx_s(stream), ema, value, (long long)n, ema_decay, skip_ctl);
  MBX_LAUNCH_CHECK();
  return MBX_OK;
}
```

### multibox_amd/engine.py

```python
from __future__ import annotations

import ctypes as C
import math
import os
import re

import numpy as np
import torch

from . import _lib, ops
from .ops import View

BN_EPS = 0.001
STATS_ROWS = int(os.environ.get("MBX_STATS_ROWS", "8"))
WEIGHT_DECAY = 0.00004


def _same_pad(n, k, s):
    out = -(-n // s)
    total = max((out - 1) * s + k - n, 0)
    return out, total // 2


def _valid(n, k, s):
# ... 549 lines not shown
        self._plan_fused_bwd()
        for op in self.convs:
            op.fb_acc_off = op.fb_bar_off = -1
        for op in self.convs:
            u = op.fb_unit
            if u is not None and op is u.lead:
                ws_floats = (ws_floats + 31) // 32 * 32
                op.fb_acc_off = ws_floats
                ws_floats += ops.BN_BWD_SLOTS * 2 * u.K
            if op.fb_segments is not None:
                ws_floats = (ws_floats + 31) // 32 * 32
                op.fb_bar_off = ws_floats
                ws_floats += ops.GRID_BARRIER_BYTES // 4
        ws_floats = (ws_floats + 31) // 32 * 32
        self.bn_ws = torch.zeros(max(ws_floats, 8), dtype=torch.float32, device=dev)
        assert self.bn_ws.data_ptr() % 128 == 0 or torch.device(dev).type != "cuda"
        n_ctr = self.i5_counters.numel()
        n_stats16 = (max(n_stats16, 4) + 31) // 32 * 32
        self._n_fwd_barriers = sum(1 for op in self.convs if op.kind == "bn") if self.fuse_apply else 0
        self._fwd_barriers_used = 0
        bar_words = ops.GRID_BARRIER_BYTES // 4
        self._fwd_clear = torch.zeros(n_ctr + n_stats16 + self._n_fwd_barriers * bar_words + 32, dtype=torch.int32, device=dev)
        self.i5_counters = self._fwd_clear[:n_ctr]
        self.stats16 = self._fwd_clear[n_ctr:n_ctr + n_stats16].view(torch.float32)
        b0 = n_ctr + n_stats16
        b0 += (-(self._fwd_clear.data_ptr() // 4 + b0)) % 32
        self._fwd_barrier_base = self._fwd_clear.data_ptr() + 4 * b0
        self.bn_thr = torch.zeros(max(self.nBt, 8), dtype=torch.float32, device=dev)
        self.bn_timeouts_total = torch.zeros((), dtype=torch.int64, device=dev)
        self.stats_scratch = torch.zeros(max(max_stats, 2), dtype=torch.float32, device=dev)
        self.bwd_scratch = torch.zeros(max(max_bwd, 2), dtype=torch.float32, device=dev)
        self.m12 = torch.zeros(2 * 2048, dtype=torch.float32, device=dev)
        self.reg_loss = torch.zeros(1, dtype=torch.float32, device=dev)

    def _plan_bw_stats(self):
        for op in self.convs:
            op.bw_unit, op.bw_segments = None, None
        if not self.bw_stats or torch.device(self.dev).type != "cuda":
            return

        def consumer_ok(X):
            dd = dgrad_probe(X)
            return not (ops.direct3_applies(dd) or ops.directw_applies(dd) or ops.resident_applies(dd))

        units, segs = plan_consumer_fusion(self.convs, self.fwd, lambda u: True, consumer_ok, align=32)
        for u in units:
            for m in u.members:
                m.bw_unit = u
        for X, sg in segs.items():
            X.bw_segments = sg

    def _plan_fused_bwd(self):
        for op in self.convs:
            op.fb_unit, op.fb_segments = None, None
        if not self.fuse_bwd:
            return
        pairs_ok = os.environ.get("MBX_FUSE_BWD_PAIRS", "1") != "0"
        only = re.compile(os.environ["MBX_FUSE_BWD_ONLY"]) if os.environ.get("MBX_FUSE_BWD_ONLY") else None
        max_rounds = int(os.environ.get("MBX_FUSE_BWD_MAX_ROUNDS", "1"))

        def consumer_ok(X):
            if X.x.img_stride != X.x.H * X.x.W * X.x.ld or X.Cin % 8 or (only is not None and not only.search(X.name)):
                return False
            if not pairs_ok and X.kind == "bn" and len(X.unit.members) == 2:
                return False
            dd = dgrad_probe(X)
            if ops.direct3_applies(dd):
                return False
            return ops.fused_tail_rounds(dd, self.n_cus) <= max_rounds

        units, segs = plan_consumer_fusion(self.convs, self.fwd, lambda u: all(m.fused_pool is None for m in u.members),
                                           consumer_ok, align=8)
        for u in units:
            for m in u.members:
                m.fb_unit = u
        for X, sg in segs.items():
            X.fb_segments = sg

    def _fb_table(self, X):
        t = ops.BnBwdFused()
        t.barrier = self.bn_ws.data_ptr() + 4 * X.fb_bar_off
        t.n = len(X.fb_segments)
        t.step_poison = self.step_ctl.data_ptr()
        for i, (c_rel, m, c_in, n) in enumerate(X.fb_segments):
            u = m.unit
            ko = m.y_view.ch_off
            assert m.y_view.ld == u.K and m.dy_view.ld == u.K and u.lead.fb_acc_off >= 0
            t.c_begin[i] = c_rel
            t.y[i], t.ld_y[i] = m.y_view.buf.data_ptr() + 2 * (ko + c_in), u.K
            t.dy[i], t.ld_dy[i] = m.dy_view.buf.data_ptr() + 2 * (ko + c_in), u.K
            t.mean[i] = self.bn_mean.data_ptr() + 4 * (m.beta_off + c_in)
            t.rstd[i] = self.bn_rstd.data_ptr() + 4 * (m.beta_off + c_in)
            t.beta[i] = self.Bt.data_ptr() + 4 * (m.beta_off + c_in)
            t.dbeta[i] = self.Btg.data_ptr() + 4 * (m.beta_off + c_in)
            t.acc[i], t.acc_ld[i] = self.bn_ws.data_ptr() + 4 * (u.lead.fb_acc_off + ko + c_in), u.K
            t.relu[i] = int(m.relu)
        self._keep.append(t)
        return t

    def _bw_table(self, X):
        t = _lib.BnBwdStats()
        t.n, t.rows_mod = len(X.bw_segments), STATS_ROWS
        for i, (c_rel, m, c_in, n) in enumerate(X.bw_segments):
            u = m.unit
            ko = m.y_view.ch_off
            t.c_begin[i] = c_rel
            t.y[i], t.ld_y[i] = m.y_view.buf.data_ptr() + 2 * (ko + c_in), u.K
            t.relu_thr[i] = self.bn_thr.data_ptr() + 4 * (m.beta_off + c_in)
            t.stats[i], t.stats_ld[i] = self.bn_ws.data_ptr() + 4 * (u.lead.bw_rows_off + 2 * (ko + c_in)), u.K
        self._keep.append(t)
        return t

    def _w(self, op):
        return self.Wb[op.w_off:]

    def _desc(self, op, y: View, **kw):
        return ops.make_desc(op.x, self._w(op), op.K, op.R, op.S, op.stride, op.pad_t, op.pad_l, y, **kw)

    def _sl(self, t, off, n):
        return t[off:off + n]

    def _tune(self, op, d, what):
        key = (what, op.x.N, op.x.H, op.x.W, op.x.C, op.K, op.R, op.S, op.stride, op.pad_t, op.pad_l, d.C_out, d.C_in,
               d.epilogue, bool(d.stats_partial), d.accumulate, bool(d.skip) or (bool(d.relu_bits) and d.epilogue == ops.EPI_STORE), d.relu)
        if d.relu_bits and d.epilogue == ops.EPI_RESIDUAL:
            key = key + ("bits",)
        self.tune_registry.append((repr(key), d, what))
        if self.autotune:
            ops.autotune(d, key)
            over = ops._TUNED.get(repr(key) + "#norule") if os.environ.get("MBX_NO_RULE_EXCEPTIONS") != "1" else None
            if over is not None:
                keep = d.tile_config
                d.tile_config = int(over)
                if _lib.lib().mbx_conv_supported(C.byref(d)) != 0:
                    d.tile_config, over = keep, None
            if os.environ.get("MBX_NO_I5") == "1" and d.tile_config > ops.I5_FLAG:
                d.tile_config = ops._TUNED.get(repr(key) + "#i3", 0)
            if d.tile_config > ops.I5_FLAG and os.environ.get("MBX_I5_STATIC") != "1":
                n = ops.I7_COUNTERS if d.tile_config == ops.I7_TILE_CONFIG else 1
                assert self._i5_used + n <= self.i5_counters.numel()
                d.work_counter = self.i5_counters.data_ptr() + 4 * self._i5_used
                self._i5_used += n
            if os.environ.get("MBX_NO_2STAGE") == "1":
                d.tile_config = {9: 7, 10: 2, 11: 5, 12: 2, 13: 8, 14: 1}.get(d.tile_config, d.tile_config)
            pair = (what == "fwd" and bool(d.stats_partial) and op.group is not None and len(op.group.members) == 2
                    and os.environ.get("MBX_CONV_PAIR", "1") != "0")
            rule = ops.launch_rule(d, pair) if over is None else None
            if rule is not None:
                d.tile_config, d.work_counter = rule[0], None
                _lib.check(_lib.lib().mbx_conv_supported(C.byref(d)), rule[1] + " " + op.name)
        return d

    def _build_forward_launches(self):
        L = []
        l = _lib.lib()
        st = lambda: torch.cuda.current_stream().cuda_stream
        for op in self.fwd:
            if isinstance(op, PoolOp):
                if not op.fused_fwd:
                    L.append(op.forward)
                continue
            if op.kind == "bn":
                L.append(self._bn_forward(op))
            elif op.kind == "frozen":
                d = self._tune(op, self._desc(op, op.out, epilogue=ops.EPI_AFFINE, relu=op.relu,
                                              scale=self._sl(self.bn_scale, op.beta_off, op.K),
                                              shift=self._sl(self.bn_shift, op.beta_off, op.K)), "fwd")
                L.append(lambda d=d, op=op: _lib.check(l.mbx_conv(C.byref(d), st()), op.name))
            elif op.kind == "residual":
                d = self._tune(op, self._desc(op, op.out, epilogue=ops.EPI_RESIDUAL, relu=op.relu,
                                              shift=self._sl(self.W, op.b_off, op.K), skip=op.skip, rscale=op.rscale,
                                              relu_bits=op.relu_bits), "fwd")
                L.append(lambda d=d, op=op: _lib.check(l.mbx_conv(C.byref(d), st()), op.name))
            elif op.kind == "head":
                d = self._desc(op, op.out, epilogue=ops.EPI_STORE_F32)
                L.append(lambda d=d, op=op: _lib.check(l.mbx_conv(C.byref(d), st()), op.name))
                if op is self.heads[-1]:
                    L.append(lambda: _lib.check(l.mbx_head_gather_all(self.head_table, len(self.heads), self.B, self.P,
                                                                      self.locs.data_ptr(), self.logits.data_ptr(), st()), "head_gather_all"))
        return L

    def _bn_forward(self, op):
        l = _lib.lib()
        st = lambda: torch.cuda.current_stream().cuda_stream
        cuda = torch.device(self.dev).type == "cuda"
        u = op.unit
        i, n, single = u.members.index(op), len(u.members), len(u.members) == 1
        fpool = op.fused_pool
        use16 = self.atomic_stats and fpool is None
        if use16:
            d = self._desc(op, op.y_view, stats=self.stats16[op.stats16_off:], stats_rows_mod=STATS_ROWS, stats_ld=0 if single else u.K)
        else:
            d = self._desc(op, op.y_view, stats=self.stats_scratch[op.stats_off:])
        d = self._tune(op, d, "fwd")
        S_ = ops.splitk_slices(d, self.n_cus) if single and cuda else 0
        if S_:
            d.tile_config = ops.SPLITK_FLAG + S_
            need = int(l.mbx_conv_splitk_workspace_bytes(C.byref(d)))
            ws = torch.empty(need // 4, dtype=torch.float32, device=self.dev)
            self._keep.append(ws)
            d.splitk_ws, d.splitk_ws_bytes = ws.data_ptr(), ws.numel() * 4
            _lib.check(l.mbx_conv_supported(C.byref(d)), "split-K " + op.name)
        rows = u.rows[i] = ops.conv_stats_rows(d)
        assert use16 or i + 1 == n or rows * op.K * 2 <= u.stats_off[i + 1] - u.stats_off[i]
        u.fwd_desc[i] = d
        if i + 1 < n:
            return lambda: None if u.pair_fwd else _lib.check(l.mbx_conv(C.byref(d), st()), op.name)
        if n == 2 and cuda and os.environ.get("MBX_CONV_PAIR", "1") != "0":
            u.pair_fwd = l.mbx_conv_pair(C.byref(u.fwd_desc[0]), C.byref(d), st()) == 0
        K, M, out = u.K, op.M, op.out
        mean, rstd, mm, mv, var, beta, thr = (self._sl(t, u.lead.beta_off, K) for t in
                                              (self.bn_mean, self.bn_rstd, self.MM, self.MV, self.bn_var, self.Bt, self.bn_thr))
        s16 = self.stats16[u.stats16_base:]
        a_ptr, a_ld, amap = u.target([m.out for m in u.members])
        amap = None if amap is None else C.byref(amap)
        parts = (C.c_void_p * n)(*[self.stats_scratch.data_ptr() + 4 * o for o in u.stats_off])
        rows_a, cs_a = (C.c_int32 * n)(*u.rows), (C.c_int32 * n)(*[m.K for m in u.members])
        if fpool is not None:
            fpool.fused_fwd = True
        fd = ba = None
        if single and use16 and self.fuse_apply and not S_ and cuda and out.img_stride == out.H * out.W * out.ld \
                and (not os.environ.get("MBX_FUSE_APPLY_ONLY") or re.search(os.environ["MBX_FUSE_APPLY_ONLY"], op.name)):
            ba = ops.BnApplyDesc()
            ba.barrier = self._fwd_barrier_base + ops.GRID_BARRIER_BYTES * self._fwd_barriers_used
            ba.a, ba.ld_a, ba.beta, ba.mean, ba.rstd = out.ptr, out.ld, beta.data_ptr(), mean.data_ptr(), rstd.data_ptr()
            ba.relu_thr, ba.relu, ba.eps, ba.step_poison = thr.data_ptr(), int(op.relu), BN_EPS, self.step_ctl.data_ptr()
            fd = ops.ConvDesc.from_buffer_copy(d)
            fd.bn_apply = C.addressof(ba)
            fd.work_counter = None
            if l.mbx_conv_supported(C.byref(fd)) == 0:
                assert self._fwd_barriers_used < self._n_fwd_barriers
                self._fwd_barriers_used += 1
                self.fused_apply_launches += 1
            else:
                fd = ba = None

        def run():
            s = st()
            mm_, mv_, decay = (None, var, -1.0) if self.defer_moving else (mm, mv, self.bn_decay)
            if fd is not None and not self.no_onepass:
                ba.moving_mean, ba.moving_var, ba.decay = ops._p(mm_), ops._p(mv_), decay
                fd.max_workgroups = self.cu_cap or self.bn_max_wg
                _lib.check(l.mbx_conv(C.byref(fd), s), op.name + " + bn apply")
                return
            if u.pair_fwd:
                _lib.check(l.mbx_conv_pair(C.byref(u.fwd_desc[0]), C.byref(d), s), "pair " + op.name)
            else:
                _lib.check(l.mbx_conv(C.byref(d), s), op.name)
            totals = (mean.data_ptr(), rstd.data_ptr(), ops._p(mm_), ops._p(mv_))
            if use16:
                _lib.check(l.mbx_bn_apply_fused_mapped(s16.data_ptr(), STATS_ROWS, M, BN_EPS, decay, u.y.data_ptr(), M, K,
                                                       beta.data_ptr(), int(op.relu), a_ptr, a_ld, amap, *totals,
                                                       thr.data_ptr(), s), "bn_apply_fused_mapped")
            elif not single:
                _lib.check(l.mbx_bn_finalize_parts(parts, rows_a, cs_a, n, M, BN_EPS, decay, *totals, s), "bn_finalize_parts")
                _lib.check(l.mbx_bn_apply_mapped(u.y.data_ptr(), M, K, mean.data_ptr(), rstd.data_ptr(), beta.data_ptr(),
                                                 int(op.relu), a_ptr, a_ld, amap, s), "bn_apply_mapped")
            elif fpool is not None:
                po = fpool.out
                _lib.check(l.mbx_bn_finalize(self.stats_scratch.data_ptr(), rows, K, M, BN_EPS, decay, *totals, s), "bn_finalize")
                _lib.check(l.mbx_bn_apply_maxpool(u.y.data_ptr(), out.N, out.H, out.W, K, mean.data_ptr(), rstd.data_ptr(),
                                                  beta.data_ptr(), int(op.relu), po.ptr, po.img_stride, po.ld, po.H, po.W,
                                                  fpool.argmax.data_ptr(), s), "bn_apply_maxpool")
            elif self._probe_skip_apply and ("/block" in op.name or "/Block8" in op.name):
                _lib.check(l.mbx_bn_finalize(self.stats_scratch.data_ptr(), rows, K, M, BN_EPS, decay, *totals, s), "fin")
            else:
                _lib.check(l.mbx_bn_apply_fused(self.stats_scratch.data_ptr(), rows, M, BN_EPS, decay, u.y.data_ptr(), M, K,
                                                beta.data_ptr(), int(op.relu), a_ptr, a_ld, *totals, s), "bn_apply_fused")
        return run

    def _gview(self, v: View) -> View:
        return self.grad_of(v)

    def _claim(self, g: View):
        key = (id(g.buf), g.ch_off, g.C)
        if key in self.written:
            return 1, None
        self.written.add(key)
        src = self.pending_acc.pop(key, None)
        return (1, src) if src is not None else (0, None)

    def _make_head_table(self):
        arr = (_lib.Head * len(self.heads))()
        for j, op in enumerate(self.heads):
            cells, kk, off = op.head
            if self.mode == "train":
                op.head_grad = View(torch.zeros((op.M, self.head_ld), dtype=torch.bfloat16, device=self.dev),
                                    op.out.N, op.out.H, op.out.W, self.head_ld)
                self._bufs.append(op.head_grad.buf)
            arr[j].h, arr[j].ld_h = op.out.buf.data_ptr(), self.head_ld
            arr[j].g, arr[j].ld_g = (op.head_grad.buf.data_ptr() if op.head_grad is not None else None), self.head_ld
            arr[j].cells, arr[j].k, arr[j].off = cells, kk, off
        self.head_table = arr

    def _build_backward(self):
        self._make_head_table()
        if self.mode != "train":
            self.fwd_launches = self._build_forward_launches()
            self.bwd_launches = []
            self.bwd_jobs = []
            return
        l = _lib.lib()
        st = lambda: torch.cuda.current_stream().cuda_stream
        entries, d_off, blocks = [], 0, 0
        for op in self.convs:
            if op.need_dx:
                kpad = (op.K + 7) // 8 * 8
                e = _lib.FilterEntry(op.w_off, d_off, op.K, op.R, op.S, op.Cin, kpad, blocks)
                op.dgrad_off, op.kpad = d_off, kpad
                n = op.Cin * op.R * op.S * kpad
                d_off += (n + 7) // 8 * 8
                blocks += op.R * op.S * ((op.Cin + 31) // 32) * ((kpad + 63) // 64)
                entries.append(e)
        self.Wd = torch.zeros(max(d_off, 8), dtype=torch.bfloat16, device=self.dev)
        arr = (_lib.FilterEntry * len(entries))(*entries)
        raw = np.frombuffer(C.string_at(C.addressof(arr), C.sizeof(arr)), dtype=np.uint8).copy()
        self.filter_table = torch.from_numpy(raw).to(self.dev)
        self.filter_blocks, self.filter_entries = blocks, len(entries)

        mask_of = {}
        fused_mask = set()
        for r in self.convs:
            if r.kind == "residual" and r.relu and r.trainable:
                for c in self.fwd:
                    if isinstance(c, ConvOp) and c.x.buf is r.out.buf:
                        if c.need_dx and c.x.ch_off == r.out.ch_off and c.x.C == r.out.C:
                            mask_of[id(c)] = r
                            fused_mask.add(id(r))
                        break
                    if isinstance(c, PoolOp) and c.x.buf is r.out.buf:
                        break
        self.pending_acc = {}
        L = []
        self.bwd_ops = []
        self.bwd_jobs = []
        for op in reversed(self.fwd):
            if isinstance(op, PoolOp):
                if op.needs_backward():
                    prod = self._pool_producer(op)
                    if prod is not None:
                        prod.fused_pool = op
                        continue
                    gx = self._gview(op.x)
                    acc, src = self._claim(gx)
                    assert src is None, "a pooling layer cannot be the first writer of a residual block's input gradient"
                    L.append(op.make_backward(self._gview(op.out), gx, acc))
                    self.bwd_ops.append(op)
                    self.bwd_jobs.append(None)
                continue
            if not op.trainable:
                continue
            K, M = op.K, op.M
            dw = self._sl(self.Wg, op.w_off, K * op.R * op.S * op.Cin)
            if op.kind == "head":
                cells, kk, off = op.head
                g = op.head_grad
                dyv, scale, db = g, 1.0, None
                pre = None
                if op is self.heads[-1]:
                    pre = lambda s: _lib.check(l.mbx_head_scatter_all(self.d_locs.data_ptr(), self.d_logits.data_ptr(), self.head_table,
                                                                      len(self.heads), self.B, self.P, s), "head_scatter_all")
            elif op.kind == "residual":
                gout = self._gview(op.out)
                gs = self._gview(op.skip)
                self.pending_acc[(id(gs.buf), gs.ch_off, gs.C)] = gout
                zb = id(self.grad_of(op.x).buf)
                self.written = {k for k in self.written if k[0] != zb}
                dyv, scale, db = gout, op.rscale, self._sl(self.Wg, op.b_off, K)
                if op.relu and id(op) not in fused_mask:
                    pre = lambda s, gout=gout, op=op: _lib.check(
                        l.mbx_relu_mask(gout.ptr, gout.ld, op.out.ptr, op.out.ld, op.M, op.K, s), "relu_mask")
                else:
                    pre = None
            else:
                dyv, scale, db = op.dy_view, 1.0, None
                pre = self._bn_backward(op)
            ddesc = fdesc = None
            if op.need_dx:
                gx = self._gview(op.x)
                acc, acc_src = self._claim(gx)
                dyin = View(dyv.buf, dyv.N, dyv.H, dyv.W, op.kpad, dyv.ld, dyv.ch_off, 2)
                mr = mask_of.get(id(op))
                ddesc = ops.make_desc(dyin, self.Wd[op.dgrad_off:], op.Cin, op.R, op.S, op.stride,
                                      op.R - 1 - op.pad_t, op.S - 1 - op.pad_l, gx, transposed=1, accumulate=acc,
                                      rscale=(scale if scale != 1.0 else 0.0), skip=(mr.out if mr is not None else None),
                                      acc_src=acc_src)
                if mr is not None and self.relu_bits and op.Cin % 8 == 0:
                    bits = torch.zeros((op.x.N * op.x.H * op.x.W, (op.Cin + 31) // 32 * 4), dtype=torch.uint8, device=self.dev)
                    alt = ops.make_desc(dyin, self.Wd[op.dgrad_off:], op.Cin, op.R, op.S, op.stride,
                                        op.R - 1 - op.pad_t, op.S - 1 - op.pad_l, gx, transposed=1, accumulate=acc,
                                        rscale=(scale if scale != 1.0 else 0.0), acc_src=acc_src, relu_bits=bits)
                    if torch.device(self.dev).type != "cuda" or l.mbx_conv_supported(C.byref(alt)) == 0:
                        ddesc, mr.relu_bits = alt, bits
                self._tune(op, ddesc, "dgrad")
                if op.fb_segments is not None:
                    assert acc == 0 and acc_src is None and mr is None, op.name
                    fdesc = ops.ConvDesc.from_buffer_copy(ddesc)
                    fdesc.bn_bwd = C.addressof(self._fb_table(op))
                    fdesc.work_counter = None
                    if not (ops.I5_FLAG < fdesc.tile_config <= ops.I5_FLAG + 7 or fdesc.tile_config in (ops.DIRECTW_TILE_CONFIG, ops.RESIDENT_TILE_CONFIG)):
                        fdesc.tile_config = ops.i5_tile_for(op.x.M, op.Cin, self.n_cus)
                    if l.mbx_conv_supported(C.byref(fdesc)) != 0:
                        fdesc.tile_config = ops.i5_tile_for(op.x.M, op.Cin, self.n_cus)
                    _lib.check(l.mbx_conv_supported(C.byref(fdesc)), "data gradient + BN backward " + op.name)
                    self.fused_bwd_launches += 1
                if op.bw_segments is not None:
                    assert acc == 0 and acc_src is None and mr is None, op.name
                    ddesc.bn_bwd_stats = C.addressof(self._bw_table(op))
                    if l.mbx_conv_supported(C.byref(ddesc)) != 0:
                        for alt in (ops.I5_TILE_CONFIGS[2], ops.I5_TILE_CONFIGS[1], 0):
                            ddesc.tile_config = alt
                            if alt == 0:
                                ddesc.work_counter = None
                            if l.mbx_conv_supported(C.byref(ddesc)) == 0:
                                break
                        _lib.check(l.mbx_conv_supported(C.byref(ddesc)), "statistics epilogue " + op.name)

            job = ops.WgradJob()
            job.desc = ops.make_desc(op.x, None, K, op.R, op.S, op.stride, op.pad_t, op.pad_l,
                                     View(dyv.buf, op.out.N, op.out.H, op.out.W, 8, dyv.ld, dyv.ch_off, 2))
            job.desc.C_out = K
            job.dy, job.dy_img_stride, job.ld_dy = dyv.ptr, dyv.img_stride, dyv.ld
            job.scale = float(scale)
            job.dw, job.db = dw.data_ptr(), (None if db is None else db.data_ptr())

            grp = op.group
            if grp is not None and ddesc is not None:
                grp.dgrad_desc[grp.members.index(op)] = ddesc

            op.fdesc = fdesc

            def run(op=op, pre=pre, ddesc=ddesc, grp=grp, fdesc=fdesc):
                s = st()
                if pre is not None and not (op.kind == "bn" and self._probe_skip_bn_bwd):
                    pre(s)
                if fdesc is not None and not self.no_onepass:
                    fdesc.max_workgroups = self.cu_cap or self.bn_max_wg
                    _lib.check(l.mbx_conv(C.byref(fdesc), s), "dgrad + bn backward " + op.name)
                    return
                if ddesc is not None:
                    if grp is not None and grp.pair_bwd:
                        if op is grp.members[-1]:
                            _lib.check(l.mbx_conv_pair(C.byref(ddesc), C.byref(grp.dgrad_desc[0]), s), "dgrad pair " + op.name)
                        return
                    ddesc.max_workgroups = self.cu_cap
                    _lib.check(l.mbx_conv(C.byref(ddesc), s), "dgrad " + op.name)
            L.append(run)
            self.bwd_ops.append(op)
            self.bwd_jobs.append(job)
        if torch.device(self.dev).type == "cuda" and os.environ.get("MBX_CONV_PAIR", "1") != "0":
            for grp in self.bn_groups:
                if len(grp.members) == 2 and len(grp.dgrad_desc) == 2 and not any(m.fdesc is not None for m in grp.members):
                    grp.pair_bwd = l.mbx_conv_pair(C.byref(grp.dgrad_desc[1]), C.byref(grp.dgrad_desc[0]), st()) == 0
        assert not self.pending_acc, "a residual block's input gradient was never written"
        self.bwd_launches = L
        self.fwd_launches = self._build_forward_launches()
        self._default_groups = None

    def _bn_backward(self, op):
        l = _lib.lib()
        u = op.unit
        if op is not u.members[-1]:
            return None
        K, M, relu, fpool = u.K, op.M, int(op.relu), op.fused_pool
        rows3 = l.mbx_bn_bwd_rows(M, K)
        y_ptr, dy_ptr, scratch, m12 = u.y.data_ptr(), u.dy.data_ptr(), self.bwd_scratch.data_ptr(), self.m12.data_ptr()
        mean, rstd, beta, dbeta, thr = (self._sl(t, u.lead.beta_off, K).data_ptr() for t in
                                        (self.bn_mean, self.bn_rstd, self.Bt, self.Btg, self.bn_thr))
        da_ptr = da_ld = dmap = None
        if fpool is None:
            da_ptr, da_ld, dmap = u.target([self._gview(m.out) for m in u.members])
            dmap = None if dmap is None else C.byref(dmap)

        def three(s):
            _lib.check(l.mbx_bn_bwd_reduce_mapped(da_ptr, da_ld, None, 0, relu, y_ptr, M, K, mean, rstd, beta, scratch, dmap, s),
                       "bn_bwd_reduce")
            _lib.check(l.mbx_bn_bwd_finalize(scratch, rows3, K, M, dbeta, m12, s), "bn_bwd_finalize")
            apply_only(s)

        def apply_only(s):
            _lib.check(l.mbx_bn_bwd_apply_mapped(da_ptr, da_ld, None, 0, relu, y_ptr, M, K, mean, rstd, beta, m12, dy_ptr, dmap, s),
                       "bn_bwd_apply")

        if fpool is not None:
            gy = self._gview(fpool.out)
            rows = l.mbx_bn_bwd_rows_pooled(fpool.x.N, fpool.x.H, fpool.x.W, K)
            assert 0 < rows * K * 2 <= self.bwd_scratch.numel()

            def form(s):
                geo = (gy.ptr, gy.img_stride, gy.ld, fpool.argmax.data_ptr(), fpool.x.N, fpool.x.H, fpool.x.W, fpool.out.H,
                       fpool.out.W, relu, y_ptr, K, mean, rstd, beta)
                _lib.check(l.mbx_bn_bwd_reduce_pooled(*geo, scratch, s), "bn_bwd_reduce_pooled")
                _lib.check(l.mbx_bn_bwd_finalize(scratch, rows, K, M, dbeta, m12, s), "bn_bwd_finalize")
                _lib.check(l.mbx_bn_bwd_apply_pooled(*geo, m12, dy_ptr, s), "bn_bwd_apply_pooled")
        elif op.bw_unit is not None:
            rows_ptr = self.bn_ws.data_ptr() + 4 * u.lead.bw_rows_off

            def form(s):
                _lib.check(l.mbx_bn_bwd_apply_rows(rows_ptr, STATS_ROWS, da_ptr, da_ld, y_ptr, M, K, mean, rstd, thr, dbeta,
                                                   dy_ptr, dmap, s), "bn_bwd_apply_rows")
        elif u.lead.bn_ws_off >= 0:
            ws_ptr = self.bn_ws.data_ptr() + 4 * u.lead.bn_ws_off

            def one(s):
                _lib.check(l.mbx_bn_bwd_onepass_mapped(da_ptr, da_ld, relu, y_ptr, M, K, mean, rstd, beta, dbeta, dy_ptr, ws_ptr,
                                                       self.cu_cap or self.bn_max_wg, self.step_ctl.data_ptr(), dmap, s),
                           "bn_bwd_onepass")

            def form(s):
                (three if self.no_onepass else one)(s)
            if os.environ.get("MBX_PROBE_BN_APPLY_ONLY") == "1":
                form = apply_only
        else:
            form = three
        if op.fb_unit is None:
            return form
        self.fused_bwd_layers += 1

        def unless_fused(s):
            if self.no_onepass:
                form(s)
        return unless_fused

    def _pool_producer(self, pool):
        if os.environ.get("MBX_POOL_FUSE", "1") == "0" or pool.kind != "max" or pool.k != 3 or pool.stride != 2 or pool.pad != 0 \
                or pool.argmax is None:
            return None
        readers = [o for o in self.fwd if o is not pool and o.x.buf is pool.x.buf]
        if readers:
            return None
        for c in self.convs:
            if c.out.buf is pool.x.buf and c.out.ch_off == pool.x.ch_off and c.out.C == pool.x.C and c.out.ld == pool.x.ld == pool.x.C:
                ok = c.kind == "bn" and c.trainable and c.group is None and (c.bn_ws_off < 0 or self.deterministic)
                return c if ok else None
        return None

    def make_wgrad_groups(self, job_lists):
        return [ops.WgradGroup(jobs, deterministic=self.deterministic, device=self.dev) for jobs in job_lists if jobs]

    def prepare_filters(self):
        if self.mode == "train" and self.filter_entries:
            _lib.check(_lib.lib().mbx_filter_prepare(self.Wb.data_ptr(), self.Wd.data_ptr(), self.filter_table.data_ptr(),
                                                     self.filter_entries, self.filter_blocks,
                                                     torch.cuda.current_stream().cuda_stream), "filter_prepare")

    def apply_moving_update(self, skip_ctl=None, skipped_steps=None, ema_mean=None, ema_var=None, ema_decay=0.0):
        lo = self.head_bt_start if self.fine_tune else 0
        n = self.nBt - lo
        if n > 0 and self.mode == "train":
            _lib.check(_lib.lib().mbx_bn_moving_update(self.MM.data_ptr() + 4 * lo, self.MV.data_ptr() + 4 * lo,
                                                       self.bn_mean.data_ptr() + 4 * lo, self.bn_var.data_ptr() + 4 * lo, n,
                                                       self.bn_decay, ops._p(skip_ctl), ops._p(skipped_steps),
                                                       None if ema_mean is None else ema_mean.data_ptr() + 4 * lo,
                                                       None if ema_var is None else ema_var.data_ptr() + 4 * lo, float(ema_decay),
                                                       torch.cuda.current_stream().cuda_stream), "bn_moving_update")

    def fold_bn(self):
        _lib.check(_lib.lib().mbx_bn_fold(self.MM.data_ptr(), self.MV.data_ptr(), self.Bt.data_ptr(), BN_EPS, self.nBt,
                                          self.bn_scale.data_ptr(), self.bn_shift.data_ptr(),
                                          torch.cuda.current_stream().cuda_stream), "bn_fold")

    def set_input(self, images_f32):
        assert images_f32.shape == (self.B, self.S, self.S, 3) and images_f32.dtype == torch.float32
        _lib.check(_lib.lib().mbx_pack_input(images_f32.contiguous().data_ptr(), self.B * self.S * self.S,
                                             self.images.buf.data_ptr(), torch.cuda.current_stream().cuda_stream), "pack_input")

    def forward(self):
        if self._i5_used or self.atomic_stats:
            self._fwd_clear.zero_()
        for f in self.fwd_launches:
            f()
        return self.locs, self.logits

    def layer_table(self):
        writers = {}

        def record(v: View, scope):
            lst = [w for w in writers.get(id(v.buf), []) if w[1] <= v.ch_off or w[0] >= v.ch_off + v.C]
            lst.append((v.ch_off, v.ch_off + v.C, scope))
            writers[id(v.buf)] = lst

        def producers(v: View):
            if v.buf is self.images.buf:
                return ["inputs"]
            inside = sorted(w for w in writers.get(id(v.buf), []) if w[0] >= v.ch_off and w[1] <= v.ch_off + v.C)
            assert inside and inside[0][0] == v.ch_off and inside[-1][1] == v.ch_off + v.C and \
                all(a[1] == b[0] for a, b in zip(inside, inside[1:])), "input view is not tiled by earlier outputs"
            return [w[2] for w in inside]

        table = []
        for op in self.fwd:
            if isinstance(op, PoolOp):
                table.append({"scope": op.scope, "op": op.kind + "_pool2d", "in_channels": op.x.C, "out_channels": op.out.C,
                              "kernel": [op.k, op.k], "stride": op.stride, "pad": [op.pad, op.pad],
                              "out_hw": [op.out.H, op.out.W], "inputs": producers(op.x)})
                record(op.out, op.scope)
                continue
            ins = producers(op.x)
            off = 0
            for m in op.members:
                e = {"scope": m.scope, "op": "conv2d", "in_channels": 3 if op.x.buf is self.images.buf else op.Cin,
                     "out_channels": m.K, "kernel": [op.R, op.S], "stride": op.stride, "pad": [op.pad_t, op.pad_l],
                     "out_hw": [op.out.H, op.out.W], "inputs": ins, "bn": op.kind in ("bn", "frozen"),
                     "bias": op.kind == "residual", "activation": "relu" if (op.relu and op.kind != "residual") else None}
                if op.kind == "residual":
                    e["residual"] = {"scale": op.rscale, "skip": producers(op.skip), "activation": "relu" if op.relu else None}
                table.append(e)
                if op.kind != "head":
                    record(op.out.slice(off, m.K), m.scope)
                off += m.K
        return table

    def flops_per_image(self, train=True):
        total = 0.0
        for op in self.convs:
            f = 2.0 * (op.M // self.B) * op.K * op.Cin * op.R * op.S
            total += f * (3.0 if (train and op.trainable) else 1.0)
        return total

    def barrier_timeouts(self):
        if self.mode != "train":
            return 0
        return int(self.bn_timeouts_total) + int(float(self.step_ctl[0]))

    def zero_grads(self):
        n_clear = self.G_off if self.fine_tune else self.G.numel()
        _lib.check(_lib.lib().mbx_step_begin(self.G.data_ptr(), n_clear, self.bn_ws.data_ptr(), self.bn_ws.numel(),
                                             self.nBt, self.bn_timeouts_total.data_ptr(), self.reg_loss.data_ptr(),
                                             torch.cuda.current_stream().cuda_stream), "step_begin")
        if self.fine_tune:
            self.Wg[self.head_w_start:].zero_()

    def backward(self):
        if self._i5_used:
            self.i5_counters.zero_()
        for f in self.bwd_launches:
            f()
        self.run_deferred_wgrad()

    def run_deferred_wgrad(self):
        if self._default_groups is None:
            jobs = [j for j in self.bwd_jobs if j is not None]
            n = max(1, (len(jobs) + 3) // 4)
            self._default_groups = self.make_wgrad_groups([jobs[i:i + n] for i in range(0, len(jobs), n)])
        for g in self._default_groups:
            g.launch()


class PoolOp:
    def __init__(self, net, kind, x: View, out: View, k, stride, pad):
        self.net, self.kind, self.x, self.out, self.k, self.stride, self.pad = net, kind, x, out, k, stride, pad
        self.argmax = None
        self.fused_fwd = False
        if kind == "max" and net.mode == "train" and not net.fine_tune:
            self.argmax = torch.zeros((out.N, out.H, out.W, out.C), dtype=torch.uint8, device=net.dev)

    def needs_backward(self):
        return self.net.mode == "train" and not self.net.fine_tune

    def forward(self):
        l, x, y = _lib.lib(), self.x, self.out
        s = torch.cuda.current_stream().cuda_stream
        if self.kind == "max":
            _lib.check(l.mbx_maxpool_fwd(x.ptr, x.img_stride, x.ld, x.N, x.H, x.W, x.C, self.k, self.stride, y.ptr,
                                         y.img_stride, y.ld, y.H, y.W, None if self.argmax is None else self.argmax.data_ptr(), s),
                       "maxpool_fwd")
        else:
            _lib.check(l.mbx_avgpool_fwd(x.ptr, x.img_stride, x.ld, x.N, x.H, x.W, x.C, self.k, self.pad, y.ptr,
                                         y.img_stride, y.ld, y.H, y.W, s), "avgpool_fwd")

    def make_backward(self, gy: View, gx: View, acc):
        l, x, y = _lib.lib(), self.x, self.out

        def run():
            s = torch.cuda.current_stream().cuda_stream
            if self.kind == "max":
                _lib.check(l.mbx_maxpool_bwd(gy.ptr, gy.img_stride, gy.ld, self.argmax.data_ptr(), x.N, x.H, x.W, x.C, self.k,
                                             self.stride, y.H, y.W, gx.ptr, gx.img_stride, gx.ld, acc, s), "maxpool_bwd")
            else:
                _lib.check(l.mbx_avgpool_bwd(gy.ptr, gy.img_stride, gy.ld, x.N, x.H, x.W, x.C, self.k, self.pad, y.H, y.W,
                                             gx.ptr, gx.img_stride, gx.ld, acc, s), "avgpool_bwd")
        return run
```

### multibox_amd/loss.py

```python
from __future__ import annotations

import torch

from . import _lib

SMALL_EPSILON = 1e-10


def _stream():
    return torch.cuda.current_stream().cuda_stream


def _f32(t):
    assert t.is_cuda and t.dtype == torch.float32 and t.is_contiguous(), "expected contiguous float32 CUDA tensor"
    return t


def _i32(t):
    assert t.is_cuda and t.dtype == torch.int32 and t.is_contiguous(), "expected contiguous int32 CUDA tensor"
    return t


def match_boxes(decoded, conf, gt_bboxes, num_gt_bboxes, alpha, match=None, status=None):
    B, P = decoded.shape[0], decoded.shape[1]
    G = gt_bboxes.shape[1]
    if match is None:
        match = torch.empty((B, P), dtype=torch.int32, device=decoded.device)
    if status is None:
        status = torch.empty((B,), dtype=torch.int32, device=decoded.device)
    _lib.check(_lib.lib().mbx_match(_f32(decoded).data_ptr(), _f32(conf).data_ptr(), _f32(gt_bboxes).data_ptr(),
                                    _i32(num_gt_bboxes).data_ptr(), float(alpha), B, P, G, match.data_ptr(),
                                    status.data_ptr(), None, 0, _stream()), "mbx_match")
    return match, status


def extend_matches(priors, gt_bboxes, num_gt_bboxes, status, match, iou_threshold, n_extra=None):
    B, P = match.shape
    G = gt_bboxes.shape[1]
    assert priors.shape == (P, 4) and gt_bboxes.shape == (B, G, 4)
    _lib.check(_lib.lib().mbx_match_extend(_f32(priors).data_ptr(), _f32(gt_bboxes).data_ptr(),
                                           _i32(num_gt_bboxes).data_ptr(), _i32(status).data_ptr(), float(iou_threshold),
                                           B, P, G, _i32(match).data_ptr(),
                                           None if n_extra is None else _i32(n_extra).data_ptr(), _stream()),
               "mbx_match_extend")
    return match, n_extra


def compute_assignments(locations, confidences, gt_bboxes, num_gt_bboxes, batch_size, alpha):
    B = int(batch_size)
    loc = locations.reshape(B, -1, 4).contiguous()
    P = loc.shape[1]
    conf = confidences.reshape(B, P).contiguous()
    match, status = match_boxes(loc, conf, gt_bboxes.contiguous(), num_gt_bboxes.to(torch.int32).contiguous(), alpha)
    st = status.cpu()
    if int(st.max()) != 0:
        raise ValueError("compute_assignments: infeasible or non-finite cost matrix (status %s)" % st.tolist())
    part = (match >= 0).to(torch.int32).reshape(-1)
    b_idx, p_idx = torch.nonzero(match >= 0, as_tuple=True)
    stacked = gt_bboxes[b_idx, match[b_idx, p_idx].long()].to(torch.float32)
    return [part, stacked]


def _focal_arguments(focal_gamma, focal_alpha):
    number = lambda v: isinstance(v, (int, float)) and not isinstance(v, bool)
    if focal_gamma is None:
        if focal_alpha is not None:
            raise ValueError("focal_alpha is given without focal_gamma")
        return None
    if not (number(focal_gamma) and 0.0 <= focal_gamma <= 10.0):
        raise ValueError("focal_gamma must be a number in [0, 10], got %r" % (focal_gamma,))
    if focal_alpha is None:
        return float(focal_gamma), 1.0, 1.0
    if not (number(focal_alpha) and 0.0 < focal_alpha < 1.0):
        raise ValueError("focal_alpha must be a number inside (0, 1), got %r" % (focal_alpha,))
    return float(focal_gamma), float(focal_alpha), 1.0 - float(focal_alpha)


class MultiboxLoss:

    def __init__(self, bbox_priors, batch_size, max_num_bboxes, location_loss_alpha, device="cuda", neg_per_pos=None,
                 min_neg=0, match_iou_threshold=None, focal_gamma=None, focal_alpha=None):
        self.focal = _focal_arguments(focal_gamma, focal_alpha)
        self.priors = torch.as_tensor(bbox_priors, dtype=torch.float32).to(device).contiguous()
        self.P = self.priors.shape[0]
        self.B, self.G, self.alpha = int(batch_size), int(max_num_bboxes), float(location_loss_alpha)
        f = dict(dtype=torch.float32, device=device)
        self.decoded = torch.empty((self.B, self.P, 4), **f)
        self.conf = torch.empty((self.B, self.P), **f)
        self.match = torch.empty((self.B, self.P), dtype=torch.int32, device=device)
        self.status = torch.zeros((self.B,), dtype=torch.int32, device=device)
        self.loss2 = torch.zeros((2,), **f)
        self.d_locs = torch.empty((self.B, self.P, 4), **f)
        self.d_logits = torch.empty((self.B, self.P), **f)
        self.neg_per_pos, self.min_neg, self.n_neg = neg_per_pos, min_neg, None
        mining = (0, 0, None)
        if neg_per_pos is not None:
            self.n_neg = torch.zeros((self.B,), dtype=torch.int32, device=device)
            mining = (neg_per_pos, min_neg, self.n_neg.data_ptr())
        l = _lib.lib()
        if self.focal is not None:
            self.entry, self.entry_args = "mbx_loss_fwd_bwd_focal", self.focal + mining
            ws_bytes = l.mbx_loss_focal_workspace_bytes(self.B, self.P)
        elif neg_per_pos is not None:
            self.entry, self.entry_args = "mbx_loss_fwd_bwd_mined", mining
            ws_bytes = l.mbx_loss_mined_workspace_bytes(self.B, self.P)
        else:
            self.entry, self.entry_args = "mbx_loss_fwd_bwd", ()
            ws_bytes = l.mbx_loss_workspace_bytes(self.B)
        self.ws = torch.empty((ws_bytes,), dtype=torch.uint8, device=device)
        self.match_iou_threshold, self.n_extra = match_iou_threshold, None
        if match_iou_threshold is not None:
            if not 0.0 < float(match_iou_threshold) <= 1.0:
                raise ValueError("match_iou_threshold must be in (0, 1], got %r" % (match_iou_threshold,))
            self.match_iou_threshold = float(match_iou_threshold)
            self.n_extra = torch.zeros((self.B,), dtype=torch.int32, device=device)

    def forward_backward(self, raw_locs, logits, gt_bboxes, num_gt_bboxes, grad_scale=1.0, conf_is_logit=True):
        l, s = _lib.lib(), _stream()
        B, P, G = self.B, self.P, self.G
        assert raw_locs.shape == (B, P, 4) and logits.numel() == B * P and gt_bboxes.shape == (B, G, 4)
        if conf_is_logit:
            _lib.check(l.mbx_decode_conf(_f32(raw_locs).data_ptr(), _f32(logits).data_ptr(), self.priors.data_ptr(),
                                         B, P, SMALL_EPSILON, self.decoded.data_ptr(), self.conf.data_ptr(), s),
                       "mbx_decode_conf")
        else:
            _lib.check(l.mbx_decode_conf(_f32(raw_locs).data_ptr(), None, self.priors.data_ptr(), B, P, 0.0,
                                         self.decoded.data_ptr(), None, s), "mbx_decode_conf")
            torch.add(logits.reshape(B, P), SMALL_EPSILON, out=self.conf)
        _lib.check(l.mbx_match(self.decoded.data_ptr(), self.conf.data_ptr(), _f32(gt_bboxes).data_ptr(),
                               _i32(num_gt_bboxes).data_ptr(), self.alpha, B, P, G, self.match.data_ptr(),
                               self.status.data_ptr(), None, 0, s), "mbx_match")
        if self.match_iou_threshold is not None:
            _lib.check(l.mbx_match_extend(self.priors.data_ptr(), gt_bboxes.data_ptr(), num_gt_bboxes.data_ptr(),
                                          self.status.data_ptr(), self.match_iou_threshold, B, P, G,
                                          self.match.data_ptr(), self.n_extra.data_ptr(), s), "mbx_match_extend")
        common = (self.decoded.data_ptr(), _f32(logits).data_ptr(), int(bool(conf_is_logit)), gt_bboxes.data_ptr(),
                  self.match.data_ptr(), self.alpha, float(grad_scale), B, P, G, self.loss2.data_ptr(), self.d_locs.data_ptr(),
                  self.d_logits.data_ptr())
        _lib.check(getattr(l, self.entry)(*common, *self.entry_args, self.ws.data_ptr(), self.ws.numel(), s), self.entry)
        return self.loss2, self.d_locs, self.d_logits


def add_loss(locations, confidences, batched_bboxes, batched_num_bboxes, bbox_priors, location_loss_alpha):
    B = locations.shape[0]
    m = MultiboxLoss(bbox_priors, B, batched_bboxes.shape[1], location_loss_alpha, device=locations.device)
    loss2, _, _ = m.forward_backward(locations.contiguous(), confidences.reshape(B, -1).contiguous(),
                                     batched_bboxes.to(torch.float32).contiguous(),
                                     batched_num_bboxes.to(torch.int32).contiguous(), conf_is_logit=False)
    st = m.status.cpu()
    if int(st.max()) != 0:
        raise ValueError("add_loss: matching failed (status %s)" % st.tolist())
    return loss2[0].clone(), loss2[1].clone()
```

### multibox_amd/trainer.py

```python
from __future__ import annotations

import math
import os
import re

import torch

from . import _lib
from .engine import Net, WEIGHT_DECAY
from .loss import MultiboxLoss
from .dist import BucketReducer


def decay_steps(num_train_examples, batch_size, num_epochs_per_decay):
    return int((int(num_train_examples) // int(batch_size)) * num_epochs_per_decay)


def learning_rate(step, lr0, dsteps, factor, staircase=True):
    p = step / float(dsteps)
    if staircase:
        p = math.floor(p)
    return float(lr0) * float(factor) ** p


class Trainer:
    def __init__(self, net: Net, bbox_priors, max_num_bboxes=13, location_loss_alpha=1000.0, initial_learning_rate=0.01,
                 decay_steps_=7116, learning_rate_decay_factor=0.94, staircase=True, rmsprop_decay=0.9,
                 rmsprop_momentum=0.0, rmsprop_epsilon=1.0, moving_average_decay=0.9999, use_graph=True,
                 n_segments=None, process_group=None, trainable_scopes=None, neg_per_pos=None, min_neg=0,
                 match_iou_threshold=None, focal_gamma=None, focal_alpha=None):
        assert net.mode == "train"
        self.net = net
        self.pg = process_group
        self.loss = MultiboxLoss(bbox_priors, net.B, max_num_bboxes, location_loss_alpha, device=net.dev,
                                 neg_per_pos=neg_per_pos, min_neg=min_neg, match_iou_threshold=match_iou_threshold,
                                 focal_gamma=focal_gamma, focal_alpha=focal_alpha)
        assert self.loss.P == net.P, "priors (%d) do not match the network's predictions (%d)" % (self.loss.P, net.P)
        self.loss.d_locs, self.loss.d_logits = net.d_locs, net.d_logits
        self.lr0, self.dsteps, self.lr_factor, self.staircase = initial_learning_rate, decay_steps_, learning_rate_decay_factor, staircase
        self.rms_decay, self.momentum, self.eps, self.ema_decay = rmsprop_decay, rmsprop_momentum, rmsprop_epsilon, moving_average_decay
        self.global_step = 0
        self.reducer = BucketReducer(process_group)
        f32 = dict(dtype=torch.float32, device=net.dev)
        self.w_lo = net.head_w_start if net.fine_tune else 0
        self.bt_lo = net.head_bt_start if net.fine_tune else 0
        self.Wms = torch.ones(net.nW, **f32)
        self.Btms = torch.ones(net.nBt, **f32)
        self.Wmom = torch.zeros(net.nW, **f32) if self.momentum != 0.0 else None
        self.Btmom = torch.zeros(net.nBt, **f32) if self.momentum != 0.0 else None
        self.Wema, self.Btema = net.W.clone(), net.Bt.clone()
        self.MMema, self.MVema = net.MM.clone(), net.MV.clone()
        self.frozen_reg = 0.0
        self.refresh_frozen_reg()
        self.opt_ranges = self._optimizer_ranges(trainable_scopes)
        self.gt = torch.zeros((net.B, max_num_bboxes, 4), **f32)
        self.n_gt = torch.zeros((net.B,), dtype=torch.int32, device=net.dev)
        self.images = torch.zeros((net.B, net.S, net.S, 3), **f32)
        net.prepare_filters()
        if net.fine_tune:
            net.fold_bn()
        self.use_graph = use_graph
        self.graphs = None
        self.events = []
        self._timeouts_seen = 0
        self._stop_flag = torch.zeros((), **f32)
        net.defer_moving = True
        self.skipped_steps = torch.zeros((), dtype=torch.int64, device=net.dev)
        self._skipped_seen = 0
        tail = 0
        self.overlap_cus = net.wgrad_overlap_cus if (use_graph and torch.device(net.dev).type == "cuda") else 0
        by_work = False
        if n_segments is None:
            n_segments = int(os.environ.get("MBX_DP_SEGMENTS", "2")) if self.reducer.enabled else int(os.environ.get("MBX_SEGMENTS", "1"))
            tail = int(os.environ.get("MBX_DP_TAIL_PARAMS", "2000000")) if self.reducer.enabled else 0
            if self.overlap_cus and not self.reducer.enabled:
                n_segments, by_work = int(os.environ.get("MBX_WG_GROUPS", "8")), True
        self._side = None
        self.exposed_events = None
        self._segments = self._make_segments(n_segments, tail_params=tail, by_work=by_work)

    def refresh_frozen_reg(self):
        self.frozen_reg = 0.0
        if self.w_lo > 0:
            self.frozen_reg = float(0.5 * WEIGHT_DECAY * (self.net.W[:self.w_lo].double() ** 2).sum())

    def _optimizer_ranges(self, scopes):
        net = self.net
        if scopes is None:
            return [("W", self.w_lo, net.nW, 1), ("Bt", self.bt_lo, net.nBt, 1)]
        pats = [re.compile(s.strip()) for s in scopes]
        marks = {"W": [], "Bt": []}
        self.trainable_names = []
        for name, (buf, off, shape, cpad) in net.param_index.items():
            if buf not in marks:
                continue
            n = 1
            for d in (shape[:-1] + (cpad,) if cpad is not None else shape):
                n *= d
            lo_buf = self.w_lo if buf == "W" else self.bt_lo
            if off < lo_buf:
                continue
            on = int(any(p.match(name) for p in pats))
            if on:
                self.trainable_names.append(name)
            marks[buf].append((off, off + n, on))
        out = []
        for buf, lo_buf, hi_buf in (("W", self.w_lo, net.nW), ("Bt", self.bt_lo, net.nBt)):
            cur_lo, cur_on = lo_buf, None
            pos = lo_buf
            for lo, hi, on in sorted(marks[buf]):
                if cur_on is None:
                    cur_on = on
                elif on != cur_on:
                    out.append((buf, cur_lo, lo, cur_on))
                    cur_lo, cur_on = lo, on
                pos = hi
            if cur_on is not None:
                out.append((buf, cur_lo, hi_buf, cur_on))
        return out

    def broadcast_parameters(self, src=0):
        if self.pg is None:
            return
        import torch.distributed as dist
        net = self.net
        for t in (net.W, net.Bt, net.MM, net.MV, self.Wms, self.Btms, self.Wmom, self.Btmom, self.Wema, self.Btema,
                  self.MMema, self.MVema):
            if t is not None:
                dist.broadcast(t, src=src, group=self.pg)
        step = torch.tensor([self.global_step], dtype=torch.int64, device=net.W.device)
        dist.broadcast(step, src=src, group=self.pg)
        self.global_step = int(step)
        if net.W.is_cuda:
            net.refresh_bf16()
            if net.fine_tune:
                net.fold_bn()
        self.refresh_frozen_reg()

    def request_stop(self):
        self._stop_flag.fill_(1.0)

    def fold_skipped(self, **note):
        sk = getattr(self, "skipped_steps", None)
        skipped = (int(sk) - self._skipped_seen) if sk is not None else 0
        if skipped:
            self._skipped_seen += skipped
            ev = {"event": "skipped_steps", "count": skipped, "global_step_before": self.global_step,
                  "global_step": self.global_step - skipped}
            ev.update(note)
            self.events.append(ev)
            self.global_step -= skipped
        return skipped

    def applied_global_step(self):
        sk = getattr(self, "skipped_steps", None)
        return self.global_step - ((int(sk) - self._skipped_seen) if sk is not None else 0)

    def check_health(self):
        net = self.net
        wg_bad = sum(0 if g.completed_ok() else 1 for g in getattr(self, "wgrad_groups", []))
        bad = torch.tensor([net.barrier_timeouts() - self._timeouts_seen, int(self.match_status().max() != 0), wg_bad,
                            int(float(net.step_ctl[1]) != 0.0 or float(self._stop_flag) != 0.0)], dtype=torch.int32, device=net.W.device)
        if self.pg is not None:
            import torch.distributed as dist
            if dist.get_world_size(self.pg) > 1:
                dist.all_reduce(bad, op=dist.ReduceOp.SUM, group=self.pg)
        t, m, w, stop = (int(v) for v in bad.tolist())
        self.fold_skipped(stop_requested=bool(stop), barrier_timeouts=t)
        if stop:
            return {"stop": True, "fallback": False}
        out = {"stop": bool(stop), "fallback": False}
        if t:
            self._timeouts_seen = net.barrier_timeouts()
            if net.no_onepass:
                raise RuntimeError("batch-norm backward: %d grid-barrier timeout(s) AFTER the fall-back to the three-launch form" % t)
            import sys
            net.no_onepass = True
            self.graphs = None
            self.events.append({"event": "bn_backward_fallback", "global_step": self.global_step, "barrier_timeouts": t})
            print("[multibox_amd] step %d: %d grid-barrier timeout(s) in the one-launch BN backward (workgroups not co-resident); "
                  "the affected steps were NOT applied; continuing with the three-launch BN backward" % (self.global_step, t),
                  file=sys.stderr)
            out["fallback"] = True
            return out
        if m:
            raise RuntimeError("bipartite matching failed on %d rank(s) (non-finite predictions or n_gt > P)" % m)
        if w:
            for g in self.wgrad_groups:
                g.reset()
            raise RuntimeError("grouped weight gradient: %d launch group(s) did not process all their work items "
                               "(queue heads re-uploaded)" % w)
        return out

    def _make_segments(self, n, tail_params=0, by_work=False):
        net = self.net
        tagged = list(zip(net.bwd_launches, net.bwd_ops, net.bwd_jobs))
        from .engine import PoolOp
        total = net.nW - self.w_lo
        target = max(total // max(n, 1), 1)

        def work(job):
            d = job.desc
            return float(d.N) * d.H_out * d.W_out * d.C_out * d.R * d.S * d.C_in
        wtarget = max(sum(work(j) for j in net.bwd_jobs if j is not None) / max(n, 1), 1.0)
        wacc = 0.0
        segs, cur, jobs, hi = [], [], [], net.nW
        lo = hi
        for fn, op, job in tagged:
            cur.append(fn)
            if job is not None:
                jobs.append(job)
                wacc += work(job)
            if not isinstance(op, PoolOp):
                lo = min(lo, op.w_off)
                full = (wacc >= wtarget * (len(segs) + 1)) if by_work else (hi - lo >= target)
                if full and hi > lo and len(segs) < n - 1:
                    segs.append((cur, lo, hi, jobs))
                    cur, jobs, hi = [], [], lo
                elif tail_params > 0 and len(segs) == n - 1 and hi > lo and 0 < lo - self.w_lo <= tail_params:
                    segs.append((cur, lo, hi, jobs))
                    cur, jobs, hi = [], [], lo
                    tail_params = 0
        if cur:
            segs.append((cur, self.w_lo, hi, jobs))
        on_gpu = torch.device(net.dev).type == "cuda"
        groups = net.make_wgrad_groups([j for _, _, _, j in segs]) if on_gpu else []
        self.wgrad_groups = groups
        self._seg_groups, gi = [], 0
        for _, _, _, jobs in segs:
            if jobs and on_gpu:
                self._seg_groups.append(groups[gi])
                gi += 1
            else:
                self._seg_groups.append(None)
        return [(fns, lo, hi) for fns, lo, hi, _ in segs]

    def _run_segment(self, i):
        for f in self._segments[i][0]:
            f()
        if self._seg_groups[i] is not None:
            self._seg_groups[i].launch()

    def _front(self):
        net = self.net
        first = net.fuse_apply
        if first:
            net.zero_grads()
        net.set_input(self.images)
        net.forward()
        self.loss.forward_backward(net.locs, net.logits, self.gt, self.n_gt)
        if not first:
            net.zero_grads()

    def _capture(self):
        net = self.net
        self._front_merged = False
        mm, mv = net.MM.clone(), net.MV.clone()
        self._front()
        for i in range(len(self._segments)):
            self._run_segment(i)
        net.MM.copy_(mm)
        net.MV.copy_(mv)
        torch.cuda.synchronize()
        graphs = []
        nseg, K = len(self._segments), self.overlap_cus
        mode = dict(capture_error_mode="thread_local")
        if K and self._side is None:
            self._side = torch.cuda.Stream()

        def chain(i, capped):
            net.cu_cap = net.chain_cap if capped else 0
            try:
                for f in self._segments[i][0]:
                    f()
            finally:
                net.cu_cap = 0

        def beside(fn):
            self._side.wait_stream(torch.cuda.current_stream())
            with torch.cuda.stream(self._side):
                fn()
            forked[0] = True

        def join():
            if forked[0]:
                torch.cuda.current_stream().wait_stream(self._side)
                forked[0] = False
        forked = [False]
        if K and not self.reducer.enabled:
            g = torch.cuda.CUDAGraph()
            with torch.cuda.graph(g, **mode):
                self._front()
                for i in range(nseg):
                    chain(i, capped=i > 0)
                    grp = self._seg_groups[i]
                    if grp is None:
                        continue
                    if i == nseg - 1:
                        join()
                        grp.launch()
                    else:
                        beside(lambda grp=grp: grp.launch(K))
                join()
            self.graphs = [g]
            return
        if not K and not self.reducer.enabled and nseg == 1 and os.environ.get("MBX_ONE_GRAPH", "1") != "0":
            g = torch.cuda.CUDAGraph()
            with torch.cuda.graph(g, **mode):
                self._front()
                self._run_segment(0)
            self.graphs = [g]
            return
        self._front_merged = not K
        g = torch.cuda.CUDAGraph()
        with torch.cuda.graph(g, **mode):
            self._front()
            if self._front_merged:
                self._run_segment(0)
        graphs.append(g)
        if K:
            for i in range(nseg + 1):
                g = torch.cuda.CUDAGraph()
                with torch.cuda.graph(g, **mode):
                    prev = self._seg_groups[i - 1] if i > 0 else None
                    if i == nseg:
                        if prev is not None:
                            prev.launch()
                    else:
                        if prev is not None:
                            beside(lambda prev=prev: prev.launch(K))
                        chain(i, capped=prev is not None)
                        join()
                graphs.append(g)
        else:
            for i in range(1, nseg):
                g = torch.cuda.CUDAGraph()
                with torch.cuda.graph(g, **mode):
                    self._run_segment(i)
                graphs.append(g)
        self.graphs = graphs

    def set_batch(self, images, gt_bboxes, num_gt_bboxes):
        self.images.copy_(images)
        self.gt.copy_(gt_bboxes)
        self.n_gt.copy_(num_gt_bboxes)

    def step(self):
        net, red = self.net, self.reducer
        reduce = self._reduce_bucket
        if self.use_graph:
            if self.graphs is None:
                self._capture()
            self.graphs[0].replay()
            if self.overlap_cus and red.enabled:
                for i, g in enumerate(self.graphs[1:]):
                    g.replay()
                    if i > 0:
                        reduce(i - 1, *self._segments[i - 1][1:])
            elif getattr(self, "_front_merged", False) and len(self.graphs) == len(self._segments):
                reduce(0, *self._segments[0][1:])
                for i, (g, (_, lo, hi)) in enumerate(zip(self.graphs[1:], self._segments[1:]), start=1):
                    g.replay()
                    reduce(i, lo, hi)
            else:
                for i, (g, (_, lo, hi)) in enumerate(zip(self.graphs[1:], self._segments)):
                    g.replay()
                    reduce(i, lo, hi)
        else:
            self._front()
            for i, (_, lo, hi) in enumerate(self._segments):
                self._run_segment(i)
                reduce(i, lo, hi)
        if self.exposed_events is not None and red.enabled:
            e0, e1 = torch.cuda.Event(enable_timing=True), torch.cuda.Event(enable_timing=True)
            e0.record()
            red.wait()
            e1.record()
            self.exposed_events.append((e0, e1))
        else:
            red.wait()
        self._optimizer()
        self.global_step += 1

    def _reduce_bucket(self, i, lo, hi):
        net, red = self.net, self.reducer
        if not red.enabled:
            return
        if i < len(self._segments) - 1:
            red.reduce_async(net.Wg, lo, hi)
            return
        net.step_ctl[1:2].copy_(self._stop_flag)
        if lo == 0:
            red.reduce_async(net.G, self.bt_lo, net.G_off + hi)
        else:
            red.reduce_async(net.Wg, lo, hi)
            red.reduce_async(net.Btg, self.bt_lo, net.nBt + 8)

    def run_eager_once(self):
        self._front()
        for i in range(len(self._segments)):
            self._run_segment(i)

    def _optimizer(self):
        net, l = self.net, _lib.lib()
        s = torch.cuda.current_stream().cuda_stream
        t = self.global_step
        lr = learning_rate(t, self.lr0, self.dsteps, self.lr_factor, self.staircase)
        d = min(self.ema_decay, (1.0 + t) / (10.0 + t))
        self.lr = lr
        P = lambda t_, off=0: None if t_ is None else t_.data_ptr() + 4 * off
        ctl = net.step_ctl.data_ptr()
        for buf, lo, hi, on in self.opt_ranges:
            n = hi - lo
            if n <= 0:
                continue
            if buf == "W":
                _lib.check(l.mbx_rmsprop_ema_step(P(net.W, lo), P(net.Wg, lo), P(self.Wms, lo), P(self.Wmom, lo), P(self.Wema, lo),
                                                  net.Wb.data_ptr() + 2 * lo, n, lr, self.rms_decay, self.momentum, self.eps,
                                                  WEIGHT_DECAY, d, on, net.reg_loss.data_ptr(), ctl, s), "rmsprop W")
            else:
                _lib.check(l.mbx_rmsprop_ema_step(P(net.Bt, lo), P(net.Btg, lo), P(self.Btms, lo), P(self.Btmom, lo), P(self.Btema, lo),
                                                  None, n, lr, self.rms_decay, self.momentum, self.eps, 0.0, d, on, None, ctl, s), "rmsprop beta")
        assert self.bt_lo == (net.head_bt_start if net.fine_tune else 0)
        net.apply_moving_update(net.step_ctl, self.skipped_steps, self.MMema, self.MVema, d)
        net.prepare_filters()

    def losses(self):
        l2 = self.loss.loss2.tolist()
        reg = float(self.net.reg_loss) + self.frozen_reg
        return l2[0], l2[1], reg, l2[0] + l2[1] + reg

    def match_status(self):
        return self.loss.status

    def mined_negatives_per_image(self):
        return None if self.loss.n_neg is None else float(self.loss.n_neg.float().mean())

    def extra_matches_per_image(self):
        return None if self.loss.n_extra is None else float(self.loss.n_extra.float().mean())
```

Baseline: 4384 images/sec.

## Fuse decode, match, grad clearing and filter prep into one mid-step kernel

Adds a single step_mid kernel whose blocks split three jobs: some decode and match one image, some zero the gradient and BN workspace, and the rest transpose the dgrad filter patches. This lets the filter preparation move from the end of the optimizer into the middle of the step. The forward-clear buffer is now zeroed inside the input pack kernel. RMSProp+EMA launches for all parameter ranges are batched into one call. The aim is fewer kernel launches and to let the small, low-occupancy matching work overlap with bandwidth-bound clearing and filter copies, at the cost of a heterogeneous kernel that takes the larger of the LDS needs.

```diff
diff --git a/include/mbx.h b/include/mbx.h
--- a/include/mbx.h
+++ b/include/mbx.h
@@ -322,6 +322,7 @@
 
 int mbx_relu_mask(void* g, int ld_g, const void* a, int ld_a, int64_t M, int C, mbx_stream_t stream);
 int mbx_pack_input(const float* img, int64_t pixels, void* out, mbx_stream_t stream);
+int mbx_pack_input_clear(const float* img, int64_t pixels, void* out, int32_t* clear, int64_t n_clear, mbx_stream_t stream);
 int mbx_head_gather(const float* h, int ld_h, int N, int cells, int k, int P, int off,
                     float* locs, float* logits, mbx_stream_t stream);
 int mbx_head_scatter(const float* d_locs, const float* d_logits, int N, int cells, int k, int P,
@@ -349,12 +350,27 @@
 int mbx_filter_prepare(const void* w_bf16, void* w_dgrad, const mbx_filter_entry* table ,
                        int n_entries, int total_blocks, mbx_stream_t stream);
 
+int mbx_step_mid(const float* raw_locs, const float* logits, const float* priors, float eps_add, float* decoded, float* conf,
+                 const float* gt, const int32_t* n_gt, float alpha, int B, int P, int G, int32_t* match, int32_t* status,
+                 float* grads, int64_t n_grads, float* bn_ws, int64_t n_ws, int64_t ctl_index, uint64_t* timeouts_total,
+                 float* zero_scalar, const void* w_bf16, void* w_dgrad, const mbx_filter_entry* table_mid ,
+                 int n_entries, int total_patches, mbx_stream_t stream);
+
 int mbx_rmsprop_ema_step(float* w, const float* g, float* ms, float* mom ,
                          float* ema , void* w_bf16 , int64_t n, float lr,
                          float decay, float momentum, float eps, float wd, float ema_decay,
                          int trainable, float* reg_loss, const float* skip_ctl, mbx_stream_t stream);
 int mbx_ema_update(float* ema, const float* value, int64_t n, float ema_decay, const float* skip_ctl ,
                    mbx_stream_t stream);
+#define MBX_MAX_PARAM_RANGES 4
+typedef struct {
+  float* w; const float* g; float* ms; float* mom; float* ema; void* w_bf16;
+  int64_t n;
+  float wd; int32_t trainable;
+  float* reg_loss;
+} mbx_param_range;
+int mbx_rmsprop_ema_ranges(const mbx_param_range* ranges , int n_ranges, float lr, float decay, float momentum,
+                           float eps, float ema_decay, const float* skip_ctl, mbx_stream_t stream);
 
 typedef struct {
   uint64_t src_offset;
diff --git a/multibox_amd/_lib.py b/multibox_amd/_lib.py
--- a/multibox_amd/_lib.py
+++ b/multibox_amd/_lib.py
@@ -86,6 +86,7 @@
     "mbx_avgpool_bwd": (I, [P, C.c_int64, I, I, I, I, I, I, I, I, I, P, C.c_int64, I, I, P]),
     "mbx_relu_mask": (I, [P, I, P, I, C.c_int64, I, P]),
     "mbx_pack_input": (I, [P, C.c_int64, P, P]),
+    "mbx_pack_input_clear": (I, [P, C.c_int64, P, P, C.c_int64, P]),
     "mbx_head_gather": (I, [P, I, I, I, I, I, I, P, P, P]),
     "mbx_head_scatter": (I, [P, P, I, I, I, I, I, P, I, P]),
     "mbx_head_gather_all": (I, [P, I, I, I, P, P, P]),
@@ -94,6 +95,8 @@
     "mbx_filter_prepare": (I, [P, P, P, I, I, P]),
     "mbx_rmsprop_ema_step": (I, [P, P, P, P, P, P, C.c_int64, F, F, F, F, F, F, I, P, P, P]),
     "mbx_ema_update": (I, [P, P, C.c_int64, F, P, P]),
+    "mbx_rmsprop_ema_ranges": (I, [P, I, F, F, F, F, F, P, P]),
+    "mbx_step_mid": (I, [P, P, P, F, P, P, P, P, F, I, I, I, P, P, P, C.c_int64, P, C.c_int64, C.c_int64, P, P, P, P, P, I, I, P]),
 }
 
 _lib = None
@@ -122,6 +125,14 @@
                 ("C", C.c_int32), ("Kpad", C.c_int32), ("first_block", C.c_int32)]
 
 
+class ParamRange(C.Structure):
+    _fields_ = [("w", C.c_void_p), ("g", C.c_void_p), ("ms", C.c_void_p), ("mom", C.c_void_p), ("ema", C.c_void_p),
+                ("w_bf16", C.c_void_p), ("n", C.c_int64), ("wd", C.c_float), ("trainable", C.c_int32), ("reg_loss", C.c_void_p)]
+
+
+MAX_PARAM_RANGES = 4
+
+
 def lib():
     global _lib
     if _lib is None:
diff --git a/multibox_amd/csrc/loss.hip b/multibox_amd/csrc/loss.hip
--- a/multibox_amd/csrc/loss.hip
+++ b/multibox_amd/csrc/loss.hip
@@ -1,24 +1,30 @@
 #include "boxes.h"
+#include "step_bodies.h"
 
 namespace {
 
 constexpr int kThreads = 256;
 constexpr int kWaves = kThreads / 64;
+
+__device__ __forceinline__ void decode_conf_one(const float4* __restrict__ raw, const float* __restrict__ logits,
+                                                const float4* __restrict__ priors, size_t i, int p, float eps_add,
+                                                float4* decoded, float* conf) {
+  if (decoded) {
+    const float4 r = raw[i], q = priors[p];
+    decoded[i] = make_float4(__fadd_rn(r.x, q.x), __fadd_rn(r.y, q.y), __fadd_rn(r.z, q.z), __fadd_rn(r.w, q.w));
+  }
+  if (conf) {
+    const float s = 1.0f / (1.0f + expf(-logits[i]));
+    conf[i] = __fadd_rn(s, eps_add);
+  }
+}
 
 __global__ void __launch_bounds__(kThreads)
 decode_conf_kernel(const float4* __restrict__ raw, const float* __restrict__ logits,
                    const float4* __restrict__ priors, int total, int P, float eps_add,
                    float4* __restrict__ decoded, float* __restrict__ conf) {
-  for (int i = blockIdx.x * blockDim.x + threadIdx.x; i < total; i += gridDim.x * blockDim.x) {
-    if (decoded) {
-      const float4 r = raw[i], p = priors[i % P];
-      decoded[i] = make_float4(__fadd_rn(r.x, p.x), __fadd_rn(r.y, p.y), __fadd_rn(r.z, p.z), __fadd_rn(r.w, p.w));
-    }
-    if (conf) {
-      const float s = 1.0f / (1.0f + expf(-logits[i]));
-      conf[i] = __fadd_rn(s, eps_add);
-    }
-  }
+  for (int i = blockIdx.x * blockDim.x + threadIdx.x; i < total; i += gridDim.x * blockDim.x)
+    decode_conf_one(raw, logits, priors, (size_t)i, i % P, eps_add, decoded, conf);
 }
 
 __device__ __forceinline__ double match_cost(const float4 l, const float4 g, float half_alpha,
@@ -55,11 +61,9 @@
   return r;
 }
 
-__global__ void __launch_bounds__(1024)
-match_kernel(const float4* __restrict__ decoded, const float* __restrict__ conf,
-             const float4* __restrict__ gt, const int* __restrict__ n_gt, float alpha, int P, int G,
-             int* __restrict__ match, int* __restrict__ status) {
-  extern __shared__ __attribute__((aligned(16))) unsigned char smem[];
+__device__ __forceinline__ void match_body(unsigned char* smem, const float4* decoded, const float* conf,
+                                           const float4* __restrict__ gt, const int* __restrict__ n_gt, float alpha, int P, int G,
+                                           int b, int* __restrict__ match, int* __restrict__ status) {
   double* v = reinterpret_cast<double*>(smem);
   double* spc = v + P;
   double* u = spc + P;
@@ -73,7 +77,7 @@
   __shared__ int sh_i, sh_sink, sh_bad;
   __shared__ double sh_min;
 
-  const int b = blockIdx.x, tid = threadIdx.x;
+  const int tid = threadIdx.x;
   const int nt = (int)blockDim.x, nwaves = nt >> 6;
   const float4* loc = decoded + (size_t)b * P;
   const float* cf = conf + (size_t)b * P;
@@ -181,6 +185,42 @@
   }
   for (int i = tid; i < n; i += nt) mt[col4row[i]] = i;
   if (tid == 0) status[b] = 0;
+}
+
+__global__ void __launch_bounds__(1024)
+match_kernel(const float4* __restrict__ decoded, const float* __restrict__ conf,
+             const float4* __restrict__ gt, const int* __restrict__ n_gt, float alpha, int P, int G,
+             int* __restrict__ match, int* __restrict__ status) {
+  extern __shared__ __attribute__((aligned(16))) unsigned char smem[];
+  match_body(smem, decoded, conf, gt, n_gt, alpha, P, G, (int)blockIdx.x, match, status);
+}
+
+__global__ void __launch_bounds__(kThreads)
+step_mid_kernel(const float4* __restrict__ raw, const float* __restrict__ logits, const float4* __restrict__ priors,
+                float eps_add, float4* decoded, float* conf, const float4* __restrict__ gt, const int* __restrict__ n_gt,
+                float alpha, int B, int P, int G, int* __restrict__ match, int* __restrict__ status,
+                float* __restrict__ grads, long long n_grads, float* __restrict__ bn_ws, long long n_ws, long long ctl,
+                unsigned long long* __restrict__ timeouts_total, float* __restrict__ scalar, int clear_blocks,
+                const unsigned short* __restrict__ w, unsigned short* __restrict__ wd,
+                const mbx_filter_entry* __restrict__ table, int n_entries) {
+  static_assert(kThreads == kBodyThreads, "the bodies of step_bodies.h are written for this workgroup");
+  extern __shared__ __attribute__((aligned(16))) unsigned char smem[];
+  int blk = (int)blockIdx.x;
+  if (blk < B) {
+    for (int p = threadIdx.x; p < P; p += kThreads)
+      decode_conf_one(raw, logits, priors, (size_t)blk * P + p, p, eps_add, decoded, conf);
+    __syncthreads();
+    match_body(smem, decoded, conf, gt, n_gt, alpha, P, G, blk, match, status);
+    return;
+  }
+  blk -= B;
+  if (blk < clear_blocks) {
+    step_clear_body(grads, n_grads, bn_ws, n_ws, ctl, timeouts_total, scalar, blk, clear_blocks);
+    return;
+  }
+  blk -= clear_blocks;
+  const mbx_filter_entry e = filter_find_entry(table, n_entries, blk);
+  filter_patch_copy<64>(w, wd, e, blk, reinterpret_cast<unsigned short*>(smem));
 }
 
 struct StagedBox { Box box; double area; };
@@ -433,7 +473,6 @@
 }
 
 static size_t match_lds_bytes(int P, int G) { return (size_t)P * 36 + (size_t)G * 16 + 16; }
-
 extern "C" size_t mbx_match_workspace_bytes(int, int, int) { return 0; }
 
 extern "C" int mbx_match(const float* decoded, const float* conf, const float* gt, const int32_t* n_gt,
@@ -453,6 +492,49 @@
   hipLaunchKernelGGL(match_kernel, dim3(B), dim3(nthreads), lds, mbx_s(stream),
                      reinterpret_cast<const float4*>(decoded), conf, reinterpret_cast<const float4*>(gt), n_gt,
                      alpha, P, G, match, status);
+  MBX_LAUNCH_CHECK();
+  return MBX_OK;
+}
+
+extern "C" int mbx_step_mid(const float* raw_locs, const float* logits, const float* priors, float eps_add, float* decoded,
+                            float* conf, const float* gt, const int32_t* n_gt, float alpha, int B, int P, int G,
+                            int32_t* match, int32_t* status, float* grads, int64_t n_grads, float* bn_ws, int64_t n_ws,
+                            int64_t ctl_index, uint64_t* timeouts_total, float* zero_scalar, const void* w_bf16, void* w_dgrad,
+                            const mbx_filter_entry* table_mid, int n_entries, int total_patches, mbx_stream_t stream) {
+  if (B < 0 || n_entries < 0 || n_grads < 0 || n_ws < 0) return MBX_ERR_INVALID_ARG;
+  if (B > 0 && (!raw_locs || !logits || !priors || !decoded || !conf || !gt || !n_gt || !match || !status || P <= 0 || G <= 0))
+    return MBX_ERR_INVALID_ARG;
+  const uintptr_t a16 = reinterpret_cast<uintptr_t>(grads) | reinterpret_cast<uintptr_t>(bn_ws);
+  if (n_grads % 4 || n_ws % 4 || (n_grads && !grads) || (n_ws && !bn_ws) || ((n_grads || n_ws) && (a16 & 15)) ||
+      (timeouts_total && (ctl_index < 0 || ctl_index >= n_grads)))
+    return MBX_ERR_INVALID_ARG;
+  if (n_entries > 0 && (!w_bf16 || !w_dgrad || !table_mid || total_patches <= 0)) return MBX_ERR_INVALID_ARG;
+  size_t lds = 0;
+  if (B > 0) {
+    if (match_lds_bytes(P, G) > 150 * 1024) return MBX_ERR_UNSUPPORTED;
+    lds = match_lds_bytes(P, G);
+  }
+  if (n_entries > 0 && lds < (size_t)filter_tile_bytes(64)) lds = filter_tile_bytes(64);
+  int clear_blocks = 0;
+  if (n_grads + n_ws > 0 || zero_scalar) {
+    long long c = ((n_grads + n_ws) / 4 + kThreads - 1) / kThreads;
+    clear_blocks = (int)(c > 2048 ? 2048 : (c < 1 ? 1 : c));
+  }
+  const long long blocks = (long long)B + clear_blocks + (n_entries > 0 ? total_patches : 0);
+  if (blocks == 0) return MBX_OK;
+  if (blocks >= (1LL << 31)) return MBX_ERR_UNSUPPORTED;
+  MBX_ENTER();
+  if (lds > 64 * 1024) {
+    if (hipFuncSetAttribute(reinterpret_cast<const void*>(step_mid_kernel), hipFuncAttributeMaxDynamicSharedMemorySize,
+                            (int)lds) != hipSuccess) return MBX_ERR_LAUNCH;
+  }
+  hipLaunchKernelGGL(step_mid_kernel, dim3((unsigned)blocks), dim3(kThreads), lds, mbx_s(stream),
+                     reinterpret_cast<const float4*>(raw_locs), logits, reinterpret_cast<const float4*>(priors), eps_add,
+                     reinterpret_cast<float4*>(decoded), conf, reinterpret_cast<const float4*>(gt), n_gt, alpha, B, P, G,
+                     match, status, grads, (long long)n_grads, bn_ws, (long long)n_ws,
+                     (long long)ctl_index, reinterpret_cast<unsigned long long*>(timeouts_total), zero_scalar, clear_blocks,
+                     reinterpret_cast<const unsigned short*>(w_bf16), reinterpret_cast<unsigned short*>(w_dgrad), table_mid,
+                     n_entries);
   MBX_LAUNCH_CHECK();
   return MBX_OK;
 }
diff --git a/multibox_amd/csrc/nnops.hip b/multibox_amd/csrc/nnops.hip
--- a/multibox_amd/csrc/nnops.hip
+++ b/multibox_amd/csrc/nnops.hip
@@ -1,4 +1,5 @@
 #include "vec8.h"
+#include "step_bodies.h"
 
 namespace {
 
@@ -288,11 +289,13 @@
 }
 
 __global__ void __launch_bounds__(kT)
-pack_input_kernel(const float* __restrict__ img, long long pixels, unsigned short* __restrict__ out) {
+pack_input_kernel(const float* __restrict__ img, long long pixels, unsigned short* __restrict__ out,
+                  int* __restrict__ clear, long long n_clear) {
   for (long long i = (long long)blockIdx.x * kT + threadIdx.x; i < pixels; i += (long long)gridDim.x * kT) {
     float f[8] = {img[3 * i], img[3 * i + 1], img[3 * i + 2], 0.f, 0.f, 0.f, 0.f, 0.f};
     st8(out + 8 * i, pack8(f));
   }
+  for (long long i = (long long)blockIdx.x * kT + threadIdx.x; i < n_clear; i += (long long)gridDim.x * kT) clear[i] = 0;
 }
 
 __global__ void __launch_bounds__(kT)
@@ -364,82 +367,24 @@
 __global__ void __launch_bounds__(kT)
 step_begin_kernel(float* __restrict__ G, long long nG, float* __restrict__ ws, long long nws, long long ctl,
                   unsigned long long* __restrict__ timeouts_total, float* __restrict__ scalar) {
-  if (scalar && blockIdx.x == 0 && threadIdx.x == 0) *scalar = 0.f;
-  const long long n4 = nG >> 2, w4 = nws >> 2;
-  const float4 z = make_float4(0.f, 0.f, 0.f, 0.f);
-  for (long long i = (long long)blockIdx.x * kT + threadIdx.x; i < n4 + w4; i += (long long)gridDim.x * kT) {
-    if (i < n4) {
-      if (timeouts_total && i == (ctl >> 2)) {
-        const float t = G[ctl];
-        if (t > 0.f) *timeouts_total += (unsigned long long)t;
-      }
-      reinterpret_cast<float4*>(G)[i] = z;
-    } else {
-      reinterpret_cast<float4*>(ws)[i - n4] = z;
-    }
-  }
+  step_clear_body(G, nG, ws, nws, ctl, timeouts_total, scalar, (int)blockIdx.x, (int)gridDim.x);
 }
 
 __global__ void __launch_bounds__(kT)
 filter_prepare_kernel(const unsigned short* __restrict__ w, unsigned short* __restrict__ wd,
                       const mbx_filter_entry* __restrict__ table, int n_entries) {
-  __shared__ __attribute__((aligned(16))) unsigned short tile[64][40];
-  int lo = 0, hi = n_entries - 1;
-  while (lo < hi) {
-    const int mid = (lo + hi + 1) >> 1;
-    if (table[mid].first_block <= (int)blockIdx.x) lo = mid; else hi = mid - 1;
-  }
-  const mbx_filter_entry e = table[lo];
-  const int kt = (e.Kpad + 63) / 64, ct = (e.C + 31) / 32;
-  int b = blockIdx.x - e.first_block;
-  const int ck = b % kt; b /= kt;
-  const int cc = b % ct; b /= ct;
-  const int s = b % e.S, r = b / e.S;
-  const unsigned short* src = w + e.src_off;
-  unsigned short* dst = wd + e.dst_off;
-  const int k0 = ck * 64, c0 = cc * 32;
-  const long long tap_src = ((long long)(e.R - 1 - r) * e.S + (e.S - 1 - s)) * e.C;
-  if (((e.C | e.Kpad) & 7) == 0 && ((e.src_off | e.dst_off) & 7) == 0) {
-    static_assert(kT == 256, "one 16-byte chunk per thread");
-    {
-      const int kk = threadIdx.x >> 2, c = (threadIdx.x & 3) << 3;
-      uint4 v = make_uint4(0u, 0u, 0u, 0u);
-      if (k0 + kk < e.K && c0 + c < e.C)
-        v = *reinterpret_cast<const uint4*>(src + (long long)(k0 + kk) * e.R * e.S * e.C + tap_src + c0 + c);
-      *reinterpret_cast<uint4*>(&tile[kk][c]) = v;
-    }
-    __syncthreads();
-    {
-      const int c = threadIdx.x >> 3, kk = (threadIdx.x & 7) << 3;
-      if (k0 + kk < e.Kpad && c0 + c < e.C) {
-        unsigned q[4];
-#pragma unroll
-        for (int j = 0; j < 4; ++j) q[j] = (unsigned)tile[kk + 2 * j][c] | ((unsigned)tile[kk + 2 * j + 1][c] << 16);
-        *reinterpret_cast<uint4*>(dst + (((long long)(c0 + c) * e.R + r) * e.S + s) * e.Kpad + k0 + kk) =
-            make_uint4(q[0], q[1], q[2], q[3]);
-      }
-    }
-    return;
-  }
-  for (int i = threadIdx.x; i < 64 * 32; i += kT) {
-    const int kk = i >> 5, c = i & 31;
-    unsigned short v = 0;
-    if (k0 + kk < e.K && c0 + c < e.C) v = src[(long long)(k0 + kk) * e.R * e.S * e.C + tap_src + c0 + c];
-    tile[kk][c] = v;
-  }
-  __syncthreads();
-  for (int i = threadIdx.x; i < 64 * 32; i += kT) {
-    const int c = i >> 6, kk = i & 63;
-    if (k0 + kk < e.Kpad && c0 + c < e.C)
-      dst[(((long long)(c0 + c) * e.R + r) * e.S + s) * e.Kpad + k0 + kk] = tile[kk][c];
-  }
-}
-
-__global__ void __launch_bounds__(kT)
-rmsprop_ema_kernel(float* __restrict__ w, const float* __restrict__ g, float* __restrict__ ms, float* __restrict__ mom,
-                   float* __restrict__ ema, unsigned short* __restrict__ wb, long long n, float lr, float decay,
-                   float momentum, float eps, float wd, float ema_decay, int trainable, float* __restrict__ reg_loss,
-                   const float* __restrict__ skip_ctl) {
+  static_assert(kT == kBodyThreads, "the bodies of step_bodies.h are written for this workgroup");
+  __shared__ __attribute__((aligned(16))) unsigned short tile[64 * 40];
+  const mbx_filter_entry e = filter_find_entry(table, n_entries, (int)blockIdx.x);
+  filter_patch_copy<32>(w, wd, e, (int)blockIdx.x, tile);
+}
+
+__device__ __forceinline__ void rmsprop_ema_range(float* __restrict__ w, const float* __restrict__ g, float* __restrict__ ms,
+                                                  float* __restrict__ mom, float* __restrict__ ema,
+                                                  unsigned short* __restrict__ wb, long long n, float lr, float decay,
+                                                  float momentum, float eps, float wd, float ema_decay, int trainable,
+                                                  float* __restrict__ reg_loss, const float* __restrict__ skip_ctl, int block,
+                                                  int nblocks) {
   if (skip_ctl && (skip_ctl[0] != 0.f || skip_ctl[1] != 0.f)) return;
   float sq = 0.f;
   auto one = [&](float wi, const float gi_, float& msi, float& momi, float& emai) -> float {
@@ -458,7 +403,7 @@
   const bool vec = ((reinterpret_cast<uintptr_t>(w) | reinterpret_cast<uintptr_t>(g) | reinterpret_cast<uintptr_t>(ms) |
                      reinterpret_cast<uintptr_t>(mom) | reinterpret_cast<uintptr_t>(ema)) & 15) == 0 && (reinterpret_cast<uintptr_t>(wb) & 7) == 0;
   const long long n4 = vec ? n / 4 : 0;
-  for (long long i = (long long)blockIdx.x * kT + threadIdx.x; i < n4; i += (long long)gridDim.x * kT) {
+  for (long long i = (long long)block * kT + threadIdx.x; i < n4; i += (long long)nblocks * kT) {
     float4 wv = reinterpret_cast<const float4*>(w)[i];
     float4 ev = ema ? reinterpret_cast<const float4*>(ema)[i] : make_float4(0.f, 0.f, 0.f, 0.f);
     float4 gv = make_float4(0.f, 0.f, 0.f, 0.f), mv = gv, ov = gv;
@@ -469,7 +414,7 @@
     if (trainable) { reinterpret_cast<float4*>(ms)[i] = mv; if (mom) reinterpret_cast<float4*>(mom)[i] = ov; reinterpret_cast<float4*>(w)[i] = wv; }
     if (wb) reinterpret_cast<uint2*>(wb)[i] = make_uint2(pack2bf(wv.x, wv.y), pack2bf(wv.z, wv.w));
   }
-  for (long long i = 4 * n4 + (long long)blockIdx.x * kT + threadIdx.x; i < n; i += (long long)gridDim.x * kT) {
+  for (long long i = 4 * n4 + (long long)block * kT + threadIdx.x; i < n; i += (long long)nblocks * kT) {
     float msi = trainable ? ms[i] : 0.f, momi = (trainable && mom) ? mom[i] : 0.f, emai = ema ? ema[i] : 0.f;
     const float wi = one(w[i], trainable ? g[i] : 0.f, msi, momi, emai);
     if (ema) ema[i] = emai;
@@ -490,6 +435,32 @@
 }
 
 __global__ void __launch_bounds__(kT)
+rmsprop_ema_kernel(float* __restrict__ w, const float* __restrict__ g, float* __restrict__ ms, float* __restrict__ mom,
+                   float* __restrict__ ema, unsigned short* __restrict__ wb, long long n, float lr, float decay,
+                   float momentum, float eps, float wd, float ema_decay, int trainable, float* __restrict__ reg_loss,
+                   const float* __restrict__ skip_ctl) {
+  rmsprop_ema_range(w, g, ms, mom, ema, wb, n, lr, decay, momentum, eps, wd, ema_decay, trainable, reg_loss, skip_ctl,
+                    (int)blockIdx.x, (int)gridDim.x);
+}
+
+struct RangeTable {
+  mbx_param_range r[MBX_MAX_PARAM_RANGES];
+  int first[MBX_MAX_PARAM_RANGES + 1];
+  int n;
+};
+
+__global__ void __launch_bounds__(kT)
+rmsprop_ema_ranges_kernel(const RangeTable t, float lr, float decay, float momentum, float eps, float ema_decay,
+                          const float* __restrict__ skip_ctl) {
+  int i = 0;
+  while (i + 1 < t.n && (int)blockIdx.x >= t.first[i + 1]) ++i;
+  const mbx_param_range& q = t.r[i];
+  rmsprop_ema_range(q.w, q.g, q.ms, momentum != 0.f ? q.mom : nullptr, q.ema, reinterpret_cast<unsigned short*>(q.w_bf16), q.n,
+                    lr, decay, momentum, eps, q.wd, ema_decay, q.trainable, q.reg_loss, skip_ctl,
+                    (int)blockIdx.x - t.first[i], t.first[i + 1] - t.first[i]);
+}
+
+__global__ void __launch_bounds__(kT)
 ema_update_kernel(float* __restrict__ ema, const float* __restrict__ v, long long n, float d,
                   const float* __restrict__ skip_ctl) {
   if (skip_ctl && (skip_ctl[0] != 0.f || skip_ctl[1] != 0.f)) return;
@@ -569,12 +540,18 @@
   return MBX_OK;
 }
 
+extern "C" int mbx_pack_input_clear(const float* img, int64_t pixels, void* out, int32_t* clear, int64_t n_clear,
+                                    mbx_stream_t stream) {
+  if (!img || !out || pixels <= 0 || !al16(out) || n_clear < 0 || (n_clear && !clear)) return MBX_ERR_INVALID_ARG;
+  MBX_ENTER();
+  hipLaunchKernelGGL(pack_input_kernel, dim3(grid_for(pixels > n_clear ? pixels : n_clear)), dim3(kT), 0, mbx_s(stream), img,
+                     (long long)pixels, (us)out, clear, (long long)n_clear);
+  MBX_LAUNCH_CHECK();
+  return MBX_OK;
+}
+
 extern "C" int mbx_pack_input(const float* img, int64_t pixels, void* out, mbx_stream_t stream) {
-  if (!img || !out || pixels <= 0 || !al16(out)) return MBX_ERR_INVALID_ARG;
-  MBX_ENTER();
-  hipLaunchKernelGGL(pack_input_kernel, dim3(grid_for(pixels)), dim3(kT), 0, mbx_s(stream), img, (long long)pixels, (us)out);
-  MBX_LAUNCH_CHECK();
-  return MBX_OK;
+  return mbx_pack_input_clear(img, pixels, out, nullptr, 0, stream);
 }
 
 extern "C" int mbx_head_gather(const float* h, int ld_h, int N, int cells, int k, int P, int off, float* locs,
@@ -676,6 +653,28 @@
   return MBX_OK;
 }
 
+extern "C" int mbx_rmsprop_ema_ranges(const mbx_param_range* ranges, int n_ranges, float lr, float decay, float momentum,
+                                      float eps, float ema_decay, const float* skip_ctl, mbx_stream_t stream) {
+  if (!ranges || n_ranges <= 0 || n_ranges > MBX_MAX_PARAM_RANGES) return MBX_ERR_INVALID_ARG;
+  RangeTable t;
+  t.n = n_ranges;
+  int blocks = 0;
+  for (int i = 0; i < n_ranges; ++i) {
+    const mbx_param_range& q = ranges[i];
+    if (!q.w || q.n <= 0 || (q.trainable && (!q.g || !q.ms))) return MBX_ERR_INVALID_ARG;
+    if (q.trainable && momentum != 0.f && !q.mom) return MBX_ERR_INVALID_ARG;
+    t.r[i] = q;
+    t.first[i] = blocks;
+    blocks += grid_for(q.n);
+  }
+  for (int i = n_ranges; i <= MBX_MAX_PARAM_RANGES; ++i) t.first[i] = blocks;
+  MBX_ENTER();
+  hipLaunchKernelGGL(rmsprop_ema_ranges_kernel, dim3(blocks), dim3(kT), 0, mbx_s(stream), t, lr, decay, momentum, eps,
+                     ema_decay, skip_ctl);
+  MBX_LAUNCH_CHECK();
+  return MBX_OK;
+}
+
 extern "C" int mbx_ema_update(float* ema, const float* value, int64_t n, float ema_decay, const float* skip_ctl,
                               mbx_stream_t stream) {
   if (!ema || !value || n <= 0) return MBX_ERR_INVALID_ARG;
diff --git a/multibox_amd/csrc/step_bodies.h b/multibox_amd/csrc/step_bodies.h
--- /dev/null
+++ b/multibox_amd/csrc/step_bodies.h
@@ -0,0 +1,102 @@
+#pragma once
+#include "common.h"
+
+namespace {
+
+constexpr int kBodyThreads = 256;
+
+__device__ __forceinline__ void step_clear_body(float* __restrict__ G, long long nG, float* __restrict__ ws, long long nws,
+                                                long long ctl, unsigned long long* __restrict__ timeouts_total,
+                                                float* __restrict__ scalar, int block, int nblocks) {
+  if (scalar && block == 0 && threadIdx.x == 0) *scalar = 0.f;
+  const long long n4 = nG >> 2, w4 = nws >> 2;
+  const float4 z = make_float4(0.f, 0.f, 0.f, 0.f);
+  const long long stride = (long long)nblocks * kBodyThreads;
+  long long i = (long long)block * kBodyThreads + threadIdx.x;
+  const long long c4 = timeouts_total ? (ctl >> 2) : -1;
+  for (; i + 3 * stride < n4; i += 4 * stride) {
+    if (c4 >= i && c4 <= i + 3 * stride && (c4 - i) % stride == 0) break;
+    float4* p = reinterpret_cast<float4*>(G) + i;
+    p[0] = z; p[stride] = z; p[2 * stride] = z; p[3 * stride] = z;
+  }
+  for (; i < n4 + w4; i += stride) {
+    if (i < n4) {
+      if (i == c4) {
+        const float t = G[ctl];
+        if (t > 0.f) *timeouts_total += (unsigned long long)t;
+      }
+      reinterpret_cast<float4*>(G)[i] = z;
+    } else {
+      reinterpret_cast<float4*>(ws)[i - n4] = z;
+    }
+  }
+}
+
+__device__ __forceinline__ mbx_filter_entry filter_find_entry(const mbx_filter_entry* __restrict__ table, int n_entries, int block) {
+  int lo = 0, hi = n_entries - 1;
+  while (lo < hi) {
+    const int mid = (lo + hi + 1) >> 1;
+    if (table[mid].first_block <= block) lo = mid; else hi = mid - 1;
+  }
+  return table[lo];
+}
+
+template <int CW>
+__device__ __forceinline__ void filter_patch_copy(const unsigned short* __restrict__ w, unsigned short* __restrict__ wd,
+                                                  const mbx_filter_entry& e, int block,
+                                                  unsigned short* __restrict__ tile ) {
+  static_assert(CW == 32 || CW == 64, "a patch row is one or two 64-byte runs");
+  constexpr int LD = CW + 8;
+  constexpr int CQ = CW / 8;
+  constexpr int PER = 64 * CQ / kBodyThreads;
+  const int tid = threadIdx.x;
+  const int kt = (e.Kpad + 63) / 64, ct = (e.C + CW - 1) / CW;
+  int b = block - e.first_block;
+  const int ck = b % kt; b /= kt;
+  const int cc = b % ct; b /= ct;
+  const int s = b % e.S, r = b / e.S;
+  if (r >= e.R) return;
+  const unsigned short* src = w + e.src_off;
+  unsigned short* dst = wd + e.dst_off;
+  const int k0 = ck * 64, c0 = cc * CW;
+  const long long tap_src = ((long long)(e.R - 1 - r) * e.S + (e.S - 1 - s)) * e.C;
+  if (((e.C | e.Kpad) & 7) == 0 && ((e.src_off | e.dst_off) & 7) == 0) {
+#pragma unroll
+    for (int p = 0; p < PER; ++p) {
+      const int q = tid + p * kBodyThreads, kk = q / CQ, c = (q % CQ) << 3;
+      uint4 v = make_uint4(0u, 0u, 0u, 0u);
+      if (k0 + kk < e.K && c0 + c < e.C)
+        v = *reinterpret_cast<const uint4*>(src + (long long)(k0 + kk) * e.R * e.S * e.C + tap_src + c0 + c);
+      *reinterpret_cast<uint4*>(&tile[kk * LD + c]) = v;
+    }
+    __syncthreads();
+#pragma unroll
+    for (int p = 0; p < PER; ++p) {
+      const int q = tid + p * kBodyThreads, c = q >> 3, kk = (q & 7) << 3;
+      if (k0 + kk < e.Kpad && c0 + c < e.C) {
+        unsigned u[4];
+#pragma unroll
+        for (int j = 0; j < 4; ++j) u[j] = (unsigned)tile[(kk + 2 * j) * LD + c] | ((unsigned)tile[(kk + 2 * j + 1) * LD + c] << 16);
+        *reinterpret_cast<uint4*>(dst + (((long long)(c0 + c) * e.R + r) * e.S + s) * e.Kpad + k0 + kk) =
+            make_uint4(u[0], u[1], u[2], u[3]);
+      }
+    }
+  } else {
+    for (int i = tid; i < 64 * CW; i += kBodyThreads) {
+      const int kk = i / CW, c = i % CW;
+      unsigned short v = 0;
+      if (k0 + kk < e.K && c0 + c < e.C) v = src[(long long)(k0 + kk) * e.R * e.S * e.C + tap_src + c0 + c];
+      tile[kk * LD + c] = v;
+    }
+    __syncthreads();
+    for (int i = tid; i < 64 * CW; i += kBodyThreads) {
+      const int c = i >> 6, kk = i & 63;
+      if (k0 + kk < e.Kpad && c0 + c < e.C)
+        dst[(((long long)(c0 + c) * e.R + r) * e.S + s) * e.Kpad + k0 + kk] = tile[kk * LD + c];
+    }
+  }
+}
+
+constexpr int filter_tile_bytes(int cw) { return 64 * (cw + 8) * 2; }
+
+}
diff --git a/multibox_amd/engine.py b/multibox_amd/engine.py
--- a/multibox_amd/engine.py
+++ b/multibox_amd/engine.py
@@ -875,21 +875,25 @@
             return
         l = _lib.lib()
         st = lambda: torch.cuda.current_stream().cuda_stream
-        entries, d_off, blocks = [], 0, 0
+        entries, entries_mid, d_off, blocks, patches = [], [], 0, 0, 0
         for op in self.convs:
             if op.need_dx:
                 kpad = (op.K + 7) // 8 * 8
-                e = _lib.FilterEntry(op.w_off, d_off, op.K, op.R, op.S, op.Cin, kpad, blocks)
+                entries.append(_lib.FilterEntry(op.w_off, d_off, op.K, op.R, op.S, op.Cin, kpad, blocks))
+                entries_mid.append(_lib.FilterEntry(op.w_off, d_off, op.K, op.R, op.S, op.Cin, kpad, patches))
                 op.dgrad_off, op.kpad = d_off, kpad
                 n = op.Cin * op.R * op.S * kpad
                 d_off += (n + 7) // 8 * 8
                 blocks += op.R * op.S * ((op.Cin + 31) // 32) * ((kpad + 63) // 64)
-                entries.append(e)
+                patches += op.R * op.S * ((op.Cin + 63) // 64) * ((kpad + 63) // 64)
         self.Wd = torch.zeros(max(d_off, 8), dtype=torch.bfloat16, device=self.dev)
-        arr = (_lib.FilterEntry * len(entries))(*entries)
-        raw = np.frombuffer(C.string_at(C.addressof(arr), C.sizeof(arr)), dtype=np.uint8).copy()
-        self.filter_table = torch.from_numpy(raw).to(self.dev)
-        self.filter_blocks, self.filter_entries = blocks, len(entries)
+
+        def upload(es):
+            arr = (_lib.FilterEntry * len(es))(*es)
+            return torch.from_numpy(np.frombuffer(C.string_at(C.addressof(arr), C.sizeof(arr)), dtype=np.uint8).copy()).to(self.dev)
+        self.filter_table, self.filter_table_mid = upload(entries), upload(entries_mid)
+        self.filter_blocks, self.filter_patches, self.filter_entries = blocks, patches, len(entries)
+        self.filters_stale = False
 
         mask_of = {}
         fused_mask = set()
@@ -1116,6 +1120,7 @@
             _lib.check(_lib.lib().mbx_filter_prepare(self.Wb.data_ptr(), self.Wd.data_ptr(), self.filter_table.data_ptr(),
                                                      self.filter_entries, self.filter_blocks,
                                                      torch.cuda.current_stream().cuda_stream), "filter_prepare")
+        self.filters_stale = False
 
     def apply_moving_update(self, skip_ctl=None, skipped_steps=None, ema_mean=None, ema_var=None, ema_decay=0.0):
         lo = self.head_bt_start if self.fine_tune else 0
@@ -1135,12 +1140,17 @@
 
     def set_input(self, images_f32):
         assert images_f32.shape == (self.B, self.S, self.S, 3) and images_f32.dtype == torch.float32
-        _lib.check(_lib.lib().mbx_pack_input(images_f32.contiguous().data_ptr(), self.B * self.S * self.S,
-                                             self.images.buf.data_ptr(), torch.cuda.current_stream().cuda_stream), "pack_input")
+        clear = self._fwd_clear if (self.mode == "train" and (self._i5_used or self.atomic_stats)) else None
+        _lib.check(_lib.lib().mbx_pack_input_clear(images_f32.contiguous().data_ptr(), self.B * self.S * self.S,
+                                                   self.images.buf.data_ptr(), None if clear is None else clear.data_ptr(),
+                                                   0 if clear is None else clear.numel(),
+                                                   torch.cuda.current_stream().cuda_stream), "pack_input")
+        self._fwd_cleared = clear is not None
 
     def forward(self):
-        if self._i5_used or self.atomic_stats:
+        if (self._i5_used or self.atomic_stats) and not getattr(self, "_fwd_cleared", False):
             self._fwd_clear.zero_()
+        self._fwd_cleared = False
         for f in self.fwd_launches:
             f()
         return self.locs, self.logits
@@ -1197,14 +1207,22 @@
         return int(self.bn_timeouts_total) + int(float(self.step_ctl[0]))
 
     def zero_grads(self):
-        n_clear = self.G_off if self.fine_tune else self.G.numel()
-        _lib.check(_lib.lib().mbx_step_begin(self.G.data_ptr(), n_clear, self.bn_ws.data_ptr(), self.bn_ws.numel(),
-                                             self.nBt, self.bn_timeouts_total.data_ptr(), self.reg_loss.data_ptr(),
-                                             torch.cuda.current_stream().cuda_stream), "step_begin")
+        _lib.check(_lib.lib().mbx_step_begin(*self.clear_args(), torch.cuda.current_stream().cuda_stream), "step_begin")
         if self.fine_tune:
             self.Wg[self.head_w_start:].zero_()
 
+    def clear_args(self):
+        n_clear = self.G_off if self.fine_tune else self.G.numel()
+        return (self.G.data_ptr(), n_clear, self.bn_ws.data_ptr(), self.bn_ws.numel(), self.nBt,
+                self.bn_timeouts_total.data_ptr(), self.reg_loss.data_ptr())
+
+    def step_mid_args(self):
+        return self.clear_args() + (self.Wb.data_ptr(), self.Wd.data_ptr(), self.filter_table_mid.data_ptr(),
+                                    self.filter_entries, self.filter_patches)
+
     def backward(self):
+        if self.filters_stale:
+            self.prepare_filters()
         if self._i5_used:
             self.i5_counters.zero_()
         for f in self.bwd_launches:
diff --git a/multibox_amd/loss.py b/multibox_amd/loss.py
--- a/multibox_amd/loss.py
+++ b/multibox_amd/loss.py
@@ -115,11 +115,17 @@
             self.match_iou_threshold = float(match_iou_threshold)
             self.n_extra = torch.zeros((self.B,), dtype=torch.int32, device=device)
 
-    def forward_backward(self, raw_locs, logits, gt_bboxes, num_gt_bboxes, grad_scale=1.0, conf_is_logit=True):
+    def forward_backward(self, raw_locs, logits, gt_bboxes, num_gt_bboxes, grad_scale=1.0, conf_is_logit=True, mid=None):
         l, s = _lib.lib(), _stream()
         B, P, G = self.B, self.P, self.G
         assert raw_locs.shape == (B, P, 4) and logits.numel() == B * P and gt_bboxes.shape == (B, G, 4)
-        if conf_is_logit:
+        if mid is not None:
+            assert conf_is_logit
+            _lib.check(l.mbx_step_mid(_f32(raw_locs).data_ptr(), _f32(logits).data_ptr(), self.priors.data_ptr(), SMALL_EPSILON,
+                                      self.decoded.data_ptr(), self.conf.data_ptr(), _f32(gt_bboxes).data_ptr(),
+                                      _i32(num_gt_bboxes).data_ptr(), self.alpha, B, P, G, self.match.data_ptr(),
+                                      self.status.data_ptr(), *mid, s), "mbx_step_mid")
+        elif conf_is_logit:
             _lib.check(l.mbx_decode_conf(_f32(raw_locs).data_ptr(), _f32(logits).data_ptr(), self.priors.data_ptr(),
                                          B, P, SMALL_EPSILON, self.decoded.data_ptr(), self.conf.data_ptr(), s),
                        "mbx_decode_conf")
@@ -127,9 +133,10 @@
             _lib.check(l.mbx_decode_conf(_f32(raw_locs).data_ptr(), None, self.priors.data_ptr(), B, P, 0.0,
                                          self.decoded.data_ptr(), None, s), "mbx_decode_conf")
             torch.add(logits.reshape(B, P), SMALL_EPSILON, out=self.conf)
-        _lib.check(l.mbx_match(self.decoded.data_ptr(), self.conf.data_ptr(), _f32(gt_bboxes).data_ptr(),
-                               _i32(num_gt_bboxes).data_ptr(), self.alpha, B, P, G, self.match.data_ptr(),
-                               self.status.data_ptr(), None, 0, s), "mbx_match")
+        if mid is None:
+            _lib.check(l.mbx_match(self.decoded.data_ptr(), self.conf.data_ptr(), _f32(gt_bboxes).data_ptr(),
+                                   _i32(num_gt_bboxes).data_ptr(), self.alpha, B, P, G, self.match.data_ptr(),
+                                   self.status.data_ptr(), None, 0, s), "mbx_match")
         if self.match_iou_threshold is not None:
             _lib.check(l.mbx_match_extend(self.priors.data_ptr(), gt_bboxes.data_ptr(), num_gt_bboxes.data_ptr(),
                                           self.status.data_ptr(), self.match_iou_threshold, B, P, G,
diff --git a/multibox_amd/trainer.py b/multibox_amd/trainer.py
--- a/multibox_amd/trainer.py
+++ b/multibox_amd/trainer.py
@@ -28,7 +28,7 @@
                  decay_steps_=7116, learning_rate_decay_factor=0.94, staircase=True, rmsprop_decay=0.9,
                  rmsprop_momentum=0.0, rmsprop_epsilon=1.0, moving_average_decay=0.9999, use_graph=True,
                  n_segments=None, process_group=None, trainable_scopes=None, neg_per_pos=None, min_neg=0,
-                 match_iou_threshold=None, focal_gamma=None, focal_alpha=None):
+                 match_iou_threshold=None, focal_gamma=None, focal_alpha=None, fused_mid=True):
         assert net.mode == "train"
         self.net = net
         self.pg = process_group
@@ -59,6 +59,7 @@
         net.prepare_filters()
         if net.fine_tune:
             net.fold_bn()
+        self.fused_mid = bool(fused_mid) and self.loss.P <= 1536 and not net.fuse_apply and net.filter_entries > 0
         self.use_graph = use_graph
         self.graphs = None
         self.events = []
@@ -248,6 +249,12 @@
             net.zero_grads()
         net.set_input(self.images)
         net.forward()
+        if self.fused_mid:
+            self.loss.forward_backward(net.locs, net.logits, self.gt, self.n_gt, mid=net.step_mid_args())
+            net.filters_stale = False
+            if net.fine_tune:
+                net.Wg[net.head_w_start:].zero_()
+            return
         self.loss.forward_backward(net.locs, net.logits, self.gt, self.n_gt)
         if not first:
             net.zero_grads()
@@ -410,20 +417,26 @@
         self.lr = lr
         P = lambda t_, off=0: None if t_ is None else t_.data_ptr() + 4 * off
         ctl = net.step_ctl.data_ptr()
+        table = []
         for buf, lo, hi, on in self.opt_ranges:
-            n = hi - lo
-            if n <= 0:
+            if hi - lo <= 0:
                 continue
             if buf == "W":
-                _lib.check(l.mbx_rmsprop_ema_step(P(net.W, lo), P(net.Wg, lo), P(self.Wms, lo), P(self.Wmom, lo), P(self.Wema, lo),
-                                                  net.Wb.data_ptr() + 2 * lo, n, lr, self.rms_decay, self.momentum, self.eps,
-                                                  WEIGHT_DECAY, d, on, net.reg_loss.data_ptr(), ctl, s), "rmsprop W")
+                table.append(_lib.ParamRange(P(net.W, lo), P(net.Wg, lo), P(self.Wms, lo), P(self.Wmom, lo), P(self.Wema, lo),
+                                             net.Wb.data_ptr() + 2 * lo, hi - lo, WEIGHT_DECAY, on, net.reg_loss.data_ptr()))
             else:
-                _lib.check(l.mbx_rmsprop_ema_step(P(net.Bt, lo), P(net.Btg, lo), P(self.Btms, lo), P(self.Btmom, lo), P(self.Btema, lo),
-                                                  None, n, lr, self.rms_decay, self.momentum, self.eps, 0.0, d, on, None, ctl, s), "rmsprop beta")
+                table.append(_lib.ParamRange(P(net.Bt, lo), P(net.Btg, lo), P(self.Btms, lo), P(self.Btmom, lo), P(self.Btema, lo),
+                                             None, hi - lo, 0.0, on, None))
+        for i in range(0, len(table), _lib.MAX_PARAM_RANGES):
+            part = table[i:i + _lib.MAX_PARAM_RANGES]
+            _lib.check(l.mbx_rmsprop_ema_ranges((_lib.ParamRange * len(part))(*part), len(part), lr, self.rms_decay,
+                                                self.momentum, self.eps, d, ctl, s), "rmsprop")
         assert self.bt_lo == (net.head_bt_start if net.fine_tune else 0)
         net.apply_moving_update(net.step_ctl, self.skipped_steps, self.MMema, self.MVema, d)
-        net.prepare_filters()
+        if self.fused_mid:
+            net.filters_stale = True
+        else:
+            net.prepare_filters()
 
     def losses(self):
         l2 = self.loss.loss2.tolist()
```

Result: no change. 4399 images/sec, median of 5 (+0.3%).
